# peteroh23/ModulationDetectionCNN

Measured on AMD Instinct MI355X. Metric: I/Q frames/sec (2x128, VT-CNN2, batch=2^20), higher is better.
Workload: dtype bf16; 1 GPU; vtcnn2-c11-bf16-n2^20; topology=vtcnn2, classes=11, frames_per_gpu=1048576, global_batch=1048576, parallelism=batch-shard x1 (no collective), outputs=softmax probabilities f32 + argmax int32, frames_per_forward_call=1048576, full=False

## Files before the change

### modulationdetectioncnn_amd/csrc/mdc_api.hip

```cpp
#include "mdc_internal.h"

#include <cstdlib>
#include <cstring>
#include <exception>
#include <mutex>
#include <new>

namespace mdc {

static thread_local char g_err[512] = "";

void set_error(const char* fmt, ...) {
    va_list ap;
    va_start(ap, fmt);
    vsnprintf(g_err, sizeof(g_err), fmt, ap);
    va_end(ap);
}

int upload(mdc_model* m, int idx, const void* host, size_t bytes) {
    if (m->d_pack[idx]) {
        (void)hipFree(m->d_pack[idx]);
        m->d_pack[idx] = nullptr;
    }
    MDC_HIP(hipMalloc(&m->d_pack[idx], bytes));
    MDC_HIP(hipMemcpy(m->d_pack[idx], host, bytes, hipMemcpyHostToDevice));
    m->pack_bytes[idx] = bytes;
    return MDC_OK;
}

ProfScope::ProfScope(const mdc_model* mm, int slot_, hipStream_t s_) : m(const_cast<mdc_model*>(mm)), slot(slot_), s(s_) {
    if (!m->profiling) return;
    if (hipEventCreate(&start) != hipSuccess) { start = nullptr; return; }
    (void)hipEventRecord(start, s);
}
ProfScope::~ProfScope() {
    if (!start) return;
    hipEvent_t stop = nullptr;
    if (hipEventCreate(&stop) != hipSuccess) { (void)hipEventDestroy(start); return; }
    (void)hipEventRecord(stop, s);
    try {
        std::lock_guard<std::mutex> g(m->prof_mu);
        std::vector<hipEvent_t>& ev = m->slots[slot].ev;
        ev.reserve(ev.size() + 2);
        ev.push_back(start);
        ev.push_back(stop);
    } catch (...) {
        (void)hipEventDestroy(start);
        (void)hipEventDestroy(stop);
    }
}

int iq_norm_check(const char* who, int64_t hop, float level, int flags) {
    if (hop < 1 || hop > (int64_t)1 << 24) { set_error("%s: hop must be in 1..2^24 sample pairs (got %lld)", who, (long long)hop); return MDC_EINVAL; }
    if (!(level > 0.f) || !(level <= 3.402823466e38f)) { set_error("%s: level must be finite and > 0", who); return MDC_EINVAL; }
    if ((flags & ~MDC_IQ_REMOVE_DC) != 0) { set_error("%s: unknown flag bits 0x%x", who, flags & ~MDC_IQ_REMOVE_DC); return MDC_EINVAL; }
    return MDC_OK;
}

}

using namespace mdc;

static int layer_layout(mdc_model* m) {
    const mdc_topology& t = m->topo;
    switch (t.kind) {
        case MDC_KIND_DEPLOYED:
            if (t.filters != 3 && t.filters != 10) { set_error("deployed: filters must be 3 or 10 (got %d)", t.filters); return MDC_ENOTSUP; }
            if (t.classes != 3) { set_error("deployed: classes must be 3 (got %d)", t.classes); return MDC_ENOTSUP; }
            m->nlayers = 2;
            m->nk[0] = 2 * (size_t)t.filters;            m->nb[0] = t.filters;
            m->nk[1] = 258 * (size_t)t.filters * t.classes; m->nb[1] = t.classes;
            m->slots = {{"mdc_deployed_fwd"}};
            return MDC_OK;
        case MDC_KIND_VTCNN2:
            if (t.classes < 2 || t.classes > 16) { set_error("vtcnn2: classes must be in 2..16 (got %d)", t.classes); return MDC_ENOTSUP; }
            m->nlayers = 4;
            m->nk[0] = (size_t)kC1 * 3;               m->nb[0] = kC1;
            m->nk[1] = (size_t)kC2 * kC1 * 2 * 3;     m->nb[1] = kC2;
            m->nk[2] = (size_t)kFeat * kHid;          m->nb[2] = kHid;
            m->nk[3] = (size_t)kHid * t.classes;      m->nb[3] = t.classes;
            m->slots = {{"mdc_vt_conv"}, {"mdc_vt_dense1"}, {"mdc_vt_head"}};
            return MDC_OK;
        case MDC_KIND_CNNPY:
            if (t.filters < 1 || t.filters > 10 || t.hidden < 1 || t.hidden > 16 || t.classes < 1 || t.classes > 16) {
                set_error("cnnpy: need filters 1..10, hidden 1..16, classes 1..16 (got %d,%d,%d)", t.filters, t.hidden, t.classes);
                return MDC_ENOTSUP;
            }
            m->nlayers = 3;
            m->nk[0] = 2 * 128 * (size_t)t.filters;        m->nb[0] = t.filters;
            m->nk[1] = 3 * (size_t)t.filters * t.hidden;    m->nb[1] = t.hidden;
            m->nk[2] = (size_t)t.hidden * t.classes;        m->nb[2] = t.classes;
            m->slots = {{"mdc_dense_chain"}};
            return MDC_OK;
        default:
            set_error("unknown topology kind %d", t.kind);
            return MDC_EINVAL;
    }
}

extern "C" {

int mdc_abi_version(void) { return MDC_ABI_VERSION; }

const char* mdc_last_error(void) { return g_err; }

int mdc_create(const mdc_topology* topo, int device, mdc_model** out) {
    return guarded("mdc_create", [&]() -> int {
        if (!topo || !out) { set_error("mdc_create: null argument"); return MDC_EINVAL; }
        *out = nullptr;
        if ((topo->reserved[0] & ~MDC_OPT_ALL) != 0) { set_error("mdc_create: unknown option bits 0x%x in reserved[0]", topo->reserved[0]); return MDC_EINVAL; }
        for (int i = 1; i < 4; ++i) if (topo->reserved[i] != 0) { set_error("mdc_create: reserved[1..3] must be 0"); return MDC_EINVAL; }
        if ((topo->reserved[0] & MDC_OPT_FP8_BF16_FEATURES) && topo->kind != MDC_KIND_VTCNN2) {
            set_error("mdc_create: MDC_OPT_FP8_BF16_FEATURES applies to MDC_KIND_VTCNN2 only");
            return MDC_EINVAL;
        }
        int ndev = 0;
        if (hipGetDeviceCount(&ndev) != hipSuccess || ndev == 0) { set_error("no HIP device available"); return MDC_ENODEV; }
        if (device < 0 || device >= ndev) { set_error("device %d out of range (have %d)", device, ndev); return MDC_ENODEV; }
        hipDeviceProp_t prop;
        MDC_HIP(hipGetDeviceProperties(&prop, device));
        if (std::strncmp(prop.gcnArchName, "gfx950", 6) != 0) {
            set_error("device %d is %s; libmdc.so carries gfx950 (MI355X) code only", device, prop.gcnArchName);
            return MDC_ENODEV;
        }
        mdc_model* m = new (std::nothrow) mdc_model();
        if (!m) { set_error("out of host memory"); return MDC_ENOMEM; }
        m->topo = *topo;
        m->device = device;
#ifdef MDC_ALTERNATES
        {
            auto flag = [](const char* name, int when) { const char* e = getenv(name); return e && atoi(e) == when; };
            if (flag("MDC_CONV_SCHED", 0)) m->alt |= kAltConvHipcc;
            if (flag("MDC_DENSE1_PHASED", 0)) m->alt |= kAltDense1Simple;
            if (flag("MDC_DEP_F32_MFMA", 1)) m->alt |= kAltDepF32Mfma;
            if (flag("MDC_D1_FUSED_HEAD", 0)) m->alt |= kAltSeparateHead;
            if (const char* e = getenv("MDC_DEP_RING")) m->alt_ring = atoi(e);
        }
#endif
        int rc = MDC_ENOMEM;
        try { rc = layer_layout(m); } catch (...) { delete m; throw; }
        if (rc != MDC_OK) { delete m; return rc; }
        *out = m;
        return MDC_OK;
    });
}

int mdc_num_layers(const mdc_model* m) {
    if (!m) { set_error("null model"); return MDC_EINVAL; }
    return m->nlayers;
}

int mdc_layer_sizes(const mdc_model* m, int layer, size_t* kernel_elems, size_t* bias_elems) {
    if (!m || layer < 0 || layer >= m->nlayers) { set_error("mdc_layer_sizes: bad layer %d", layer); return MDC_EINVAL; }
    if (kernel_elems) *kernel_elems = m->nk[layer];
    if (bias_elems) *bias_elems = m->nb[layer];
    return MDC_OK;
}

int mdc_set_weights(mdc_model* m, int layer, const float* kernel_host, size_t kernel_elems,
                    const float* bias_host, size_t bias_elems) {
    return guarded("mdc_set_weights", [&]() -> int {
        if (!m || !kernel_host || !bias_host) { set_error("mdc_set_weights: null argument"); return MDC_EINVAL; }
        if (m->finalized) { set_error("mdc_set_weights: model is finalized (immutable)"); return MDC_ESTATE; }
        if (layer < 0 || layer >= m->nlayers) { set_error("mdc_set_weights: layer %d out of range 0..%d", layer, m->nlayers - 1); return MDC_EINVAL; }
        if (kernel_elems != m->nk[layer] || bias_elems != m->nb[layer]) {
            set_error("mdc_set_weights: layer %d expects kernel %zu / bias %zu elements, got %zu / %zu",
                      layer, m->nk[layer], m->nb[layer], kernel_elems, bias_elems);
            return MDC_EINVAL;
        }
        m->have[layer] = false;
        m->hk[layer].assign(kernel_host, kernel_host + kernel_elems);
        m->hb[layer].assign(bias_host, bias_host + bias_elems);
        m->have[layer] = true;
        return MDC_OK;
    });
}

int mdc_finalize(mdc_model* m, int dtype) {
    return guarded("mdc_finalize", [&]() -> int {
        if (!m) { set_error("null model"); return MDC_EINVAL; }
        if (m->finalized) { set_error("mdc_finalize: already finalized"); return MDC_ESTATE; }
        for (int l = 0; l < m->nlayers; ++l)
            if (!m->have[l]) { set_error("mdc_finalize: layer %d has no weights", l); return MDC_ESTATE; }
        if (dtype != MDC_F32 && dtype != MDC_BF16 && dtype != MDC_FP8 && dtype != MDC_F16) { set_error("unknown dtype %d", dtype); return MDC_EINVAL; }
        if (dtype == MDC_F16 && m->topo.kind != MDC_KIND_DEPLOYED) { set_error("f16 is implemented for the deployed nets only"); return MDC_ENOTSUP; }
        if (dtype == MDC_FP8 && m->topo.kind == MDC_KIND_CNNPY) { set_error("fp8 is implemented for the vtcnn2 and deployed families only"); return MDC_ENOTSUP; }
        if ((m->topo.reserved[0] & MDC_OPT_FP8_BF16_FEATURES) && dtype != MDC_FP8) { set_error("mdc_finalize: MDC_OPT_FP8_BF16_FEATURES is an option of the MDC_FP8 mode"); return MDC_EINVAL; }
        if (dtype == MDC_BF16 && m->topo.kind == MDC_KIND_CNNPY) { set_error("bf16 is implemented for the vtcnn2 and deployed families only"); return MDC_ENOTSUP; }
        m->dtype = dtype;
        DeviceScope dev(m->device);
        if (!dev.ok) { set_error("mdc_finalize: cannot select device %d", m->device); return MDC_EIO; }
        int rc;
        switch (m->topo.kind) {
            case MDC_KIND_DEPLOYED:
                rc = deployed_pack(m);
                if (rc == MDC_OK) rc = deployed_q612_pack(m);
                if (rc == MDC_OK && dtype != MDC_F32) rc = deployed_bf16_pack(m);
                break;
            case MDC_KIND_VTCNN2:   rc = vtcnn2_pack(m); break;
            case MDC_KIND_CNNPY:    rc = cnnpy_pack(m); break;
            default: rc = MDC_EINVAL;
        }
        if (rc != MDC_OK) return rc;
        for (int l = 0; l < m->nlayers; ++l) {
            std::vector<float>().swap(m->hk[l]);
            std::vector<float>().swap(m->hb[l]);
        }
        m->finalized = true;
        return MDC_OK;
    });
}

size_t mdc_workspace_bytes(const mdc_model* m, int64_t n) {
    if (!m || n <= 0) return 0;
    if (m->topo.kind == MDC_KIND_VTCNN2) return vtcnn2_workspace_bytes(m, n);
    return 0;
}

int mdc_forward(const mdc_model* m, const void* x_dev, int64_t n, float* probs_dev, int32_t* labels_dev,
                float* tap_dev, int tap, void* workspace_dev, size_t workspace_bytes, void* hip_stream) {
    return guarded("mdc_forward", [&]() -> int {
        if (!m) { set_error("null model"); return MDC_EINVAL; }
        if (!m->finalized) { set_error("mdc_forward: model not finalized"); return MDC_ESTATE; }
        if (n < 0) { set_error("mdc_forward: negative frame count"); return MDC_EINVAL; }
        if (n == 0) return MDC_OK;
        if (!x_dev) { set_error("mdc_forward: null input"); return MDC_EINVAL; }
        if ((reinterpret_cast<uintptr_t>(x_dev) & 15) != 0) { set_error("mdc_forward: input must be 16-byte aligned"); return MDC_EINVAL; }
        if (tap < MDC_TAP_NONE || tap > MDC_TAP_HIDDEN) { set_error("mdc_forward: bad tap %d", tap); return MDC_EINVAL; }
        if ((tap != MDC_TAP_NONE) != (tap_dev != nullptr)) { set_error("mdc_forward: tap and tap_dev must be given together"); return MDC_EINVAL; }
        DeviceScope dev(m->device);
        if (!dev.ok) { set_error("mdc_forward: cannot select device %d", m->device); return MDC_EIO; }
        hipStream_t s = static_cast<hipStream_t>(hip_stream);
        const float* x = static_cast<const float*>(x_dev);
        switch (m->topo.kind) {
            case MDC_KIND_DEPLOYED: return deployed_forward(m, x, n, probs_dev, labels_dev, tap_dev, tap, s);
            case MDC_KIND_VTCNN2:   return vtcnn2_forward(m, x, n, probs_dev, labels_dev, tap_dev, tap, workspace_dev, workspace_bytes, s);
            case MDC_KIND_CNNPY:    return cnnpy_forward(m, x, n, probs_dev, labels_dev, tap_dev, tap, s);
            default: return MDC_EINVAL;
        }
    });
}

int mdc_forward_checked(const mdc_model* m, const void* x_dev, int64_t n, float* probs_dev, int32_t* labels_dev, void* workspace_dev,
                        size_t workspace_bytes, uint8_t* nonfinite_dev, int64_t* nonfinite_count_dev, int policy, void* hip_stream) {
    return guarded("mdc_forward_checked", [&]() -> int {
        if (policy != MDC_NONFINITE_REPORT && policy != MDC_NONFINITE_PROPAGATE) { set_error("mdc_forward_checked: unknown policy %d", policy); return MDC_EINVAL; }
        if (n < 0) { set_error("mdc_forward_checked: negative frame count"); return MDC_EINVAL; }
        if (n > 0 && !nonfinite_dev) { set_error("mdc_forward_checked: null nonfinite_dev (the per-frame flags are required)"); return MDC_EINVAL; }
        if (n > 0 && !x_dev) { set_error("mdc_forward_checked: null input"); return MDC_EINVAL; }
        if ((reinterpret_cast<uintptr_t>(x_dev) & 15) != 0) { set_error("mdc_forward_checked: input must be 16-byte aligned"); return MDC_EINVAL; }
        if (!m) { set_error("mdc_forward_checked: null model"); return MDC_EINVAL; }
        if (!m->finalized) { set_error("mdc_forward_checked: model not finalized"); return MDC_ESTATE; }
        if (n == 0) return MDC_OK;
        const bool poison = policy == MDC_NONFINITE_PROPAGATE;
        if (m->topo.kind == MDC_KIND_DEPLOYED) {
            DeviceScope dev(m->device);
            if (!dev.ok) { set_error("mdc_forward_checked: cannot select device %d", m->device); return MDC_EIO; }
            return deployed_forward_checked(m, static_cast<const float*>(x_dev), n, probs_dev, labels_dev, nonfinite_dev, nonfinite_count_dev,
                                            poison, static_cast<hipStream_t>(hip_stream));
        }
        int rc = mdc_forward(m, x_dev, n, probs_dev, labels_dev, nullptr, MDC_TAP_NONE, workspace_dev, workspace_bytes, hip_stream);
        if (rc != MDC_OK) return rc;
        DeviceScope dev(m->device);
        if (!dev.ok) { set_error("mdc_forward_checked: cannot select device %d", m->device); return MDC_EIO; }
        return nonfinite_launch(static_cast<const float*>(x_dev), n, nonfinite_dev, nonfinite_count_dev, probs_dev, labels_dev, m->topo.classes,
                                poison, static_cast<hipStream_t>(hip_stream));
    });
}

int mdc_forward_iq_u8(const mdc_model* m, const uint8_t* iq_dev, int64_t n, int64_t hop, float scale,
                      float* probs_dev, int32_t* labels_dev, void* workspace_dev, size_t workspace_bytes, void* hip_stream) {
    return guarded("mdc_forward_iq_u8", [&]() -> int {
        if (!m) { set_error("null model"); return MDC_EINVAL; }
        if (!m->finalized) { set_error("mdc_forward_iq_u8: model not finalized"); return MDC_ESTATE; }
        if (m->topo.kind == MDC_KIND_CNNPY) {
            set_error("mdc_forward_iq_u8: raw-IQ input exists for the deployed and vtcnn2 families; use mdc_iq_u8_to_frames + mdc_forward");
            return MDC_ENOTSUP;
        }
        if (n < 0) { set_error("mdc_forward_iq_u8: negative window count"); return MDC_EINVAL; }
        if (hop < 1 || hop > (int64_t)1 << 24) { set_error("mdc_forward_iq_u8: hop must be in 1..2^24 sample pairs (got %lld)", (long long)hop); return MDC_EINVAL; }
        if (n == 0) return MDC_OK;
        if (!iq_dev) { set_error("mdc_forward_iq_u8: null input"); return MDC_EINVAL; }
        if ((reinterpret_cast<uintptr_t>(iq_dev) & 1) != 0) { set_error("mdc_forward_iq_u8: input must start on a whole (I,Q) pair (2-byte aligned)"); return MDC_EINVAL; }
        DeviceScope dev(m->device);
        if (!dev.ok) { set_error("mdc_forward_iq_u8: cannot select device %d", m->device); return MDC_EIO; }
        hipStream_t s = static_cast<hipStream_t>(hip_stream);
        if (m->topo.kind == MDC_KIND_VTCNN2)
            return vtcnn2_forward_iq_u8(m, iq_dev, n, hop, scale, probs_dev, labels_dev, workspace_dev, workspace_bytes, s);
        return (m->dtype == MDC_F32) ? deployed_forward_iq_u8(m, iq_dev, n, hop, scale, probs_dev, labels_dev, s)
                                     : deployed_bf16_forward_iq_u8(m, iq_dev, n, hop, scale, probs_dev, labels_dev, s);
    });
}

int mdc_set_fp8_input_absmax(mdc_model* m, float absmax) {
    if (!m) { set_error("null model"); return MDC_EINVAL; }
    if (m->finalized) { set_error("mdc_set_fp8_input_absmax: call it before mdc_finalize"); return MDC_ESTATE; }
    if (!(absmax > 0.f) || !(absmax < 1e30f)) { set_error("mdc_set_fp8_input_absmax: need a positive finite value"); return MDC_EINVAL; }
    m->fp8_input_absmax = absmax;
    return MDC_OK;
}

int mdc_set_fp8_feature_absmax(mdc_model* m, float absmax) {
    if (!m) { set_error("null model"); return MDC_EINVAL; }
    if (m->finalized) { set_error("mdc_set_fp8_feature_absmax: call it before mdc_finalize"); return MDC_ESTATE; }
    if (m->topo.kind != MDC_KIND_VTCNN2) { set_error("mdc_set_fp8_feature_absmax: the E4M3 features exist for MDC_KIND_VTCNN2 only"); return MDC_EINVAL; }
    if (!(absmax > 0.f) || !(absmax < 1e30f)) { set_error("mdc_set_fp8_feature_absmax: need a positive finite value"); return MDC_EINVAL; }
    m->fp8_feature_absmax = absmax;
    return MDC_OK;
}

int mdc_forward_q612(const mdc_model* m, const void* x_dev, int x_is_q612, int64_t n, int32_t* dense_dev, int32_t* labels_dev,
                     void* hip_stream) {
    return guarded("mdc_forward_q612", [&]() -> int {
        if (!m) { set_error("null model"); return MDC_EINVAL; }
        if (!m->finalized) { set_error("mdc_forward_q612: model not finalized"); return MDC_ESTATE; }
        if (m->topo.kind != MDC_KIND_DEPLOYED) { set_error("mdc_forward_q612: the FPGA datapath exists for the deployed nets only"); return MDC_ENOTSUP; }
        if (n < 0) { set_error("mdc_forward_q612: negative frame count"); return MDC_EINVAL; }
        if (n == 0) return MDC_OK;
        if (!x_dev) { set_error("mdc_forward_q612: null input"); return MDC_EINVAL; }
        if ((reinterpret_cast<uintptr_t>(x_dev) & 15) != 0) { set_error("mdc_forward_q612: input must be 16-byte aligned"); return MDC_EINVAL; }
        DeviceScope dev(m->device);
        if (!dev.ok) { set_error("mdc_forward_q612: cannot select device %d", m->device); return MDC_EIO; }
        return deployed_q612_forward(m, x_dev, x_is_q612 != 0, n, dense_dev, labels_dev, static_cast<hipStream_t>(hip_stream));
    });
}

int mdc_confusion(const int32_t* truth_dev, const int32_t* pred_dev, int64_t n, int classes, int64_t* counts_dev, int64_t* bad_dev,
                  void* hip_stream) {
    if (n < 0) { set_error("mdc_confusion: negative count"); return MDC_EINVAL; }
    if (n > 0 && (!truth_dev || !pred_dev)) { set_error("mdc_confusion: null labels"); return MDC_EINVAL; }
    if (!counts_dev) { set_error("mdc_confusion: null counts"); return MDC_EINVAL; }
    return guarded("mdc_confusion", [&]() -> int {
        return confusion_launch(truth_dev, pred_dev, nullptr, n, classes, 1, counts_dev, bad_dev, static_cast<hipStream_t>(hip_stream)); });
}

int mdc_confusion_binned(const int32_t* truth_dev, const int32_t* pred_dev, const int32_t* bin_dev, int64_t n, int classes, int bins,
                         int64_t* counts_dev, int64_t* bad_dev, void* hip_stream) {
    if (n < 0) { set_error("mdc_confusion_binned: negative count"); return MDC_EINVAL; }
    if (n > 0 && (!truth_dev || !pred_dev || !bin_dev)) { set_error("mdc_confusion_binned: null labels"); return MDC_EINVAL; }
    if (!counts_dev) { set_error("mdc_confusion_binned: null counts"); return MDC_EINVAL; }
    if (bins < 1) { set_error("mdc_confusion_binned: bins must be >= 1 (got %d)", bins); return MDC_EINVAL; }
    return guarded("mdc_confusion_binned", [&]() -> int {
        return confusion_launch(truth_dev, pred_dev, bin_dev, n, classes, bins, counts_dev, bad_dev, static_cast<hipStream_t>(hip_stream)); });
}

int mdc_crossentropy(const float* probs_dev, const int32_t* truth_dev, int64_t n, int classes, double* loss_sum_dev, int64_t* bad_dev,
                     void* hip_stream) {
    if (n < 0) { set_error("mdc_crossentropy: negative count"); return MDC_EINVAL; }
    if (n > 0 && (!probs_dev || !truth_dev)) { set_error("mdc_crossentropy: null probabilities or labels"); return MDC_EINVAL; }
    if (!loss_sum_dev) { set_error("mdc_crossentropy: null loss accumulator"); return MDC_EINVAL; }
    return guarded("mdc_crossentropy", [&]() -> int {
        return crossentropy_launch(probs_dev, truth_dev, n, classes, loss_sum_dev, bad_dev, static_cast<hipStream_t>(hip_stream)); });
}

int mdc_iq_u8_to_frames(const uint8_t* iq_dev, int64_t n, float scale, float* x_dev, void* hip_stream) {
    if (n < 0) { set_error("mdc_iq_u8_to_frames: negative frame count"); return MDC_EINVAL; }
    if (n == 0) return MDC_OK;
    if (!iq_dev || !x_dev) { set_error("mdc_iq_u8_to_frames: null buffer"); return MDC_EINVAL; }
    if ((reinterpret_cast<uintptr_t>(iq_dev) & 3) != 0 || (reinterpret_cast<uintptr_t>(x_dev) & 7) != 0) {
        set_error("mdc_iq_u8_to_frames: iq must be 4-byte and frames 8-byte aligned");
        return MDC_EINVAL;
    }
    return guarded("mdc_iq_u8_to_frames", [&]() -> int { return iq_u8_launch(iq_dev, n, 128, scale, x_dev, static_cast<hipStream_t>(hip_stream)); });
}

int mdc_iq_u8_windows(const uint8_t* iq_dev, int64_t n, int64_t hop, float scale, float* x_dev, void* hip_stream) {
    if (n < 0) { set_error("mdc_iq_u8_windows: negative window count"); return MDC_EINVAL; }
    if (hop < 1 || hop > (int64_t)1 << 24) { set_error("mdc_iq_u8_windows: hop must be in 1..2^24 sample pairs (got %lld)", (long long)hop); return MDC_EINVAL; }
    if (n == 0) return MDC_OK;
    if (!iq_dev || !x_dev) { set_error("mdc_iq_u8_windows: null buffer"); return MDC_EINVAL; }
    if ((reinterpret_cast<uintptr_t>(x_dev) & 7) != 0) { set_error("mdc_iq_u8_windows: frames must be 8-byte aligned"); return MDC_EINVAL; }
    if ((reinterpret_cast<uintptr_t>(iq_dev) & 1) != 0) { set_error("mdc_iq_u8_windows: input must start on a whole (I,Q) pair (2-byte aligned)"); return MDC_EINVAL; }
    return guarded("mdc_iq_u8_windows", [&]() -> int { return iq_u8_launch(iq_dev, n, hop, scale, x_dev, static_cast<hipStream_t>(hip_stream)); });
}

int mdc_iq_u8_windows_norm(const uint8_t* iq_dev, int64_t n, int64_t hop, float level, int flags, float* x_dev,
                           mdc_iq_window_stats* stats_dev, void* hip_stream) {
    if (n < 0) { set_error("mdc_iq_u8_windows_norm: negative window count"); return MDC_EINVAL; }
    int rc = iq_norm_check("mdc_iq_u8_windows_norm", hop, level, flags);
    if (rc != MDC_OK) return rc;
    if (!x_dev && !stats_dev) { set_error("mdc_iq_u8_windows_norm: x_dev and stats_dev are both null (nothing to compute)"); return MDC_EINVAL; }
    if ((reinterpret_cast<uintptr_t>(x_dev) & 7) != 0) { set_error("mdc_iq_u8_windows_norm: frames must be 8-byte aligned"); return MDC_EINVAL; }
    if ((reinterpret_cast<uintptr_t>(stats_dev) & 15) != 0) { set_error("mdc_iq_u8_windows_norm: statistics must be 16-byte aligned"); return MDC_EINVAL; }
    if (n > 0 && !iq_dev) { set_error("mdc_iq_u8_windows_norm: null input"); return MDC_EINVAL; }
    if ((reinterpret_cast<uintptr_t>(iq_dev) & 1) != 0) { set_error("mdc_iq_u8_windows_norm: input must start on a whole (I,Q) pair (2-byte aligned)"); return MDC_EINVAL; }
    return guarded("mdc_iq_u8_windows_norm", [&]() -> int {
        return iq_norm_launch(iq_dev, n, hop, level, flags, x_dev, stats_dev, static_cast<hipStream_t>(hip_stream)); });
}

int mdc_set_profiling(mdc_model* m, int on) {
    if (!m) { set_error("null model"); return MDC_EINVAL; }
    m->profiling = on != 0;
    return MDC_OK;
}

int mdc_profile_slots(const mdc_model* m) { return m ? (int)m->slots.size() : MDC_EINVAL; }

const char* mdc_profile_name(const mdc_model* m, int slot) {
    if (!m || slot < 0 || slot >= (int)m->slots.size()) return "";
    return m->slots[slot].name;
}

int mdc_profile_read(mdc_model* m, int slot, double* total_ms, int64_t* launches) {
    return guarded("mdc_profile_read", [&]() -> int {
        if (!m || slot < 0 || slot >= (int)m->slots.size()) { set_error("mdc_profile_read: bad slot"); return MDC_EINVAL; }
        ProfSlot& ps = m->slots[slot];
        std::vector<hipEvent_t> ev;
        {
            std::lock_guard<std::mutex> g(m->prof_mu);
            ev.swap(ps.ev);
        }
        double add_ms = 0;
        int64_t add_n = 0;
        int rc = MDC_OK;
        for (size_t i = 0; i + 1 < ev.size(); i += 2) {
            float ms = 0.f;
            if (hipEventSynchronize(ev[i + 1]) != hipSuccess || hipEventElapsedTime(&ms, ev[i], ev[i + 1]) != hipSuccess) {
                set_error("mdc_profile_read: event query failed");
                rc = MDC_EIO;
                break;
            }
            add_ms += ms;
            add_n += 1;
        }
        for (hipEvent_t e : ev) (void)hipEventDestroy(e);
        std::lock_guard<std::mutex> g(m->prof_mu);
        ps.total_ms += add_ms;
        ps.launches += add_n;
        if (total_ms) *total_ms = ps.total_ms;
        if (launches) *launches = ps.launches;
        return rc;
    });
}

int mdc_profile_reset(mdc_model* m) {
    if (!m) { set_error("null model"); return MDC_EINVAL; }
    std::lock_guard<std::mutex> g(m->prof_mu);
    for (ProfSlot& ps : m->slots) {
        for (hipEvent_t e : ps.ev) (void)hipEventDestroy(e);
        ps.ev.clear();
        ps.total_ms = 0;
        ps.launches = 0;
    }
    return MDC_OK;
}

int mdc_predict_host(mdc_model* m, const float* x_host, int64_t n, float* probs_host, int32_t* labels_host, int64_t chunk_frames) {
    return guarded("mdc_predict_host", [&]() -> int { return predict_host(m, x_host, n, probs_host, labels_host, chunk_frames); });
}

int mdc_predict_host_checked(mdc_model* m, const float* x_host, int64_t n, float* probs_host, int32_t* labels_host, uint8_t* nonfinite_host,
                             int64_t* nonfinite_count, int policy, int64_t chunk_frames) {
    return guarded("mdc_predict_host_checked", [&]() -> int {
        return predict_host_checked(m, x_host, n, probs_host, labels_host, nonfinite_host, nonfinite_count, policy, chunk_frames); });
}

int mdc_predict_host_iq_u8(mdc_model* m, const uint8_t* iq_host, int64_t n, int64_t hop, float scale, float* probs_host,
                           int32_t* labels_host, int64_t chunk_frames) {
    return guarded("mdc_predict_host_iq_u8", [&]() -> int { return predict_host_iq_u8(m, iq_host, n, hop, scale, probs_host, labels_host, chunk_frames); });
}

int mdc_predict_host_iq(mdc_model* m, const void* iq_host, int format, int64_t n, int64_t hop, float scale, float* probs_host,
                        int32_t* labels_host, int64_t chunk_frames) {
    return guarded("mdc_predict_host_iq", [&]() -> int { return predict_host_iq(m, iq_host, format, n, hop, scale, probs_host, labels_host, chunk_frames); });
}

int mdc_predict_host_iq_norm(mdc_model* m, const void* iq_host, int format, int64_t n, int64_t hop, float level, int flags, float* probs_host,
                             int32_t* labels_host, mdc_iq_window_stats64* stats64_host, int64_t chunk_frames) {
    return guarded("mdc_predict_host_iq_norm", [&]() -> int {
        return predict_host_iq_norm(m, iq_host, format, n, hop, level, flags, probs_host, labels_host, stats64_host, chunk_frames); });
}

int mdc_predict_host_iq_u8_norm(mdc_model* m, const uint8_t* iq_host, int64_t n, int64_t hop, float level, int flags, float* probs_host,
                                int32_t* labels_host, mdc_iq_window_stats* stats_host, int64_t chunk_frames) {
    return guarded("mdc_predict_host_iq_u8_norm", [&]() -> int {
        return predict_host_iq_u8_norm(m, iq_host, n, hop, level, flags, probs_host, labels_host, stats_host, chunk_frames); });
}

void mdc_destroy(mdc_model* m) {
    if (!m) return;
    {
        DeviceScope dev(m->device);
        host_ctx_free(m);
    }
    for (void*& p : m->d_pack) if (p) { (void)hipFree(p); p = nullptr; }
    for (ProfSlot& ps : m->slots) for (hipEvent_t e : ps.ev) (void)hipEventDestroy(e);
    delete m;
}

}
```

### modulationdetectioncnn_amd/csrc/mdc_internal.h

```cpp
#pragma once
#include <hip/hip_runtime.h>
#include <cstdarg>
#include <cstdint>
#include <cstdio>
#include <exception>
#include <mutex>
#include <new>
#include <string>
#include <type_traits>
#include <vector>

#include "mdc.h"

namespace mdc {

void set_error(const char* fmt, ...);

template <class Fn>
inline int guarded(const char* what, Fn&& fn) noexcept {
    try {
        return fn();
    } catch (const std::bad_alloc&) {
        set_error("%s: out of host memory", what);
        return MDC_ENOMEM;
    } catch (const std::exception& e) {
        set_error("%s: %s", what, e.what());
        return MDC_EIO;
    } catch (...) {
        set_error("%s: unexpected exception", what);
        return MDC_EIO;
    }
}

#define MDC_HIP(call)                                                                      \
    do {                                                                                   \
        hipError_t e_ = (call);                                                            \
        if (e_ != hipSuccess) {                                                            \
            mdc::set_error("%s failed: %s (%s:%d)", #call, hipGetErrorString(e_), __FILE__, __LINE__); \
            return MDC_EIO;                                                                \
        }                                                                                  \
    } while (0)

constexpr int kRows = 2;
constexpr int kSamples = 128;
constexpr int kFrameFloats = kRows * kSamples;

constexpr int kC1 = 256;
constexpr int kW1 = 130;
constexpr int kC2 = 80;
constexpr int kW2 = 132;
constexpr int kFeat = kC2 * kW2;
constexpr int kHid = 256;

__host__ __device__ constexpr int feat16_index(int w, int o) {
    return (w >> 1) * (2 * kC2) + (o < 64 ? (w & 1) * 64 + o : 128 + 2 * (o - 64) + (w & 1));
}

__host__ __device__ constexpr int feat8_index(int w, int o) {
    return (w >> 2) * (4 * kC2) + (o < 64 ? ((w >> 1) & 1) * 128 + 8 * (o >> 2) + 4 * (w & 1) + (o & 3) : 256 + 4 * (o - 64) + (w & 3));
}

__device__ __forceinline__ uint2 load8_unaligned(const unsigned char* p) {
    uint2 r;
    __builtin_memcpy(&r, p, 8);
    return r;
}

struct NfArgs {
    unsigned char* flags;
    unsigned long long* count;
    int poison;
};
template <bool CHECK> using HopOrNf = typename std::conditional<CHECK, NfArgs, long>::type;
__device__ __forceinline__ long hop_of(long h) { return h; }
__device__ __forceinline__ long hop_of(const NfArgs&) { return 256; }
__device__ __forceinline__ NfArgs nf_of(long) { return NfArgs{nullptr, nullptr, 0}; }
__device__ __forceinline__ NfArgs nf_of(const NfArgs& a) { return a; }
constexpr unsigned kNfInfBits = 0x7F800000u;
__device__ __forceinline__ unsigned nf_absbits_max4(const float4 v) {
    return max(max(__float_as_uint(v.x) & 0x7FFFFFFFu, __float_as_uint(v.y) & 0x7FFFFFFFu),
               max(__float_as_uint(v.z) & 0x7FFFFFFFu, __float_as_uint(v.w) & 0x7FFFFFFFu));
}

enum { kAltConvHipcc = 1,
       kAltDense1Simple = 2,
       kAltDepF32Mfma = 4,
       kAltSeparateHead = 8 };

struct ProfSlot {
    const char* name;
    std::vector<hipEvent_t> ev;
    double total_ms = 0;
    int64_t launches = 0;
};

}

struct mdc_model {
    mdc_topology topo{};
    int device = 0;
    int dtype = MDC_F32;
    bool finalized = false;
    int nlayers = 0;
    size_t nk[4]{}, nb[4]{};
    std::vector<float> hk[4], hb[4];
    bool have[4]{};

    void* d_pack[8]{};
    size_t pack_bytes[8]{};

    int alt = 0;
    int alt_ring = -1;
    float fp8_input_absmax = 0.02f;
    float fp8_feature_absmax = 0.f;
    int fp8_feat_scale_log2 = 0;
    bool fp8_e4m3_features = false;
    float fp8_feat_divisor = 1.f;
    int feat_scale_log2 = 0;

    bool profiling = false;
    std::vector<mdc::ProfSlot> slots;
    std::mutex prof_mu;

    void* host_ctx = nullptr;
    std::mutex host_mu;
};

namespace mdc {

struct ProfScope {
    mdc_model* m;
    int slot;
    hipStream_t s;
    hipEvent_t start = nullptr;
    ProfScope(const mdc_model* mm, int slot_, hipStream_t s_);
    ~ProfScope();
    ProfScope(const ProfScope&) = delete;
    ProfScope& operator=(const ProfScope&) = delete;
};

int upload(mdc_model* m, int idx, const void* host, size_t bytes);

struct DeviceScope {
    int prev = -1, want;
    bool ok = true;
    explicit DeviceScope(int device) : want(device) {
        if (hipGetDevice(&prev) != hipSuccess) prev = -1;
        if (prev != want && hipSetDevice(want) != hipSuccess) ok = false;
    }
    ~DeviceScope() { if (prev >= 0 && prev != want) (void)hipSetDevice(prev); }
    DeviceScope(const DeviceScope&) = delete;
    DeviceScope& operator=(const DeviceScope&) = delete;
};

int predict_host(mdc_model* m, const float* x_host, int64_t n, float* probs_host, int32_t* labels_host, int64_t chunk_frames);
int predict_host_checked(mdc_model* m, const float* x_host, int64_t n, float* probs_host, int32_t* labels_host, uint8_t* nonfinite_host,
                         int64_t* nonfinite_count, int policy, int64_t chunk_frames);
int predict_host_iq_u8(mdc_model* m, const uint8_t* iq_host, int64_t n, int64_t hop, float scale, float* probs_host, int32_t* labels_host,
                       int64_t chunk_frames);
int predict_host_iq_u8_norm(mdc_model* m, const uint8_t* iq_host, int64_t n, int64_t hop, float level, int flags, float* probs_host,
                            int32_t* labels_host, mdc_iq_window_stats* stats_host, int64_t chunk_frames);
int predict_host_iq(mdc_model* m, const void* iq_host, int format, int64_t n, int64_t hop, float scale, float* probs_host, int32_t* labels_host,
                    int64_t chunk_frames);
int predict_host_iq_norm(mdc_model* m, const void* iq_host, int format, int64_t n, int64_t hop, float level, int flags, float* probs_host,
                         int32_t* labels_host, mdc_iq_window_stats64* stats_host, int64_t chunk_frames);
void host_ctx_free(mdc_model* m);

int deployed_pack(mdc_model* m);
int deployed_f32m_pack(mdc_model* m);
int deployed_f32m_forward(const mdc_model* m, const float* x, int64_t n, float* probs, int32_t* labels, float* tap_dense, hipStream_t s);
int deployed_f32m_forward_iq_u8(const mdc_model* m, const uint8_t* iq, int64_t n, long hop2, float scale, float* probs, int32_t* labels, hipStream_t s);
int deployed_bf16_pack(mdc_model* m);
int deployed_bf16_forward(const mdc_model* m, const float* x, int64_t n, float* probs, int32_t* labels, hipStream_t s);
int deployed_bf16_forward_iq_u8(const mdc_model* m, const uint8_t* iq, int64_t n, int64_t hop, float scale, float* probs, int32_t* labels, hipStream_t s);
int deployed_q612_pack(mdc_model* m);
int deployed_q612_forward(const mdc_model* m, const void* x, int x_is_q, int64_t n, int32_t* dense, int32_t* labels, hipStream_t s);
int vtcnn2_fp8_pack(mdc_model* m);
int vtcnn2_fp8_conv(const mdc_model* m, const float* x, int64_t n, void* feat, hipStream_t s, long hop2 = 0, float scale = 0.f);
int confusion_launch(const int32_t* truth, const int32_t* pred, const int32_t* bin, int64_t n, int classes, int bins, int64_t* counts,
                     int64_t* bad, hipStream_t s);
int crossentropy_launch(const float* probs, const int32_t* truth, int64_t n, int classes, double* loss_sum, int64_t* bad, hipStream_t s);
int iq_u8_launch(const uint8_t* iq, int64_t n, int64_t hop, float scale, float* x, hipStream_t s);
int iq_norm_check(const char* who, int64_t hop, float level, int flags);
int iq_norm_launch(const uint8_t* iq, int64_t n, int64_t hop, float level, int flags, float* x, mdc_iq_window_stats* stats, hipStream_t s);
constexpr long kIqGridCap = 16384;
int iq_pair_bytes(int format);
constexpr int64_t iq_span_count(int64_t pairs, int64_t span, int64_t step) { return pairs >= span ? (pairs - span) / step + 1 : 0; }
int iq_format_known(const char* who, int format);
int iq_pair_aligned(const char* who, const char* what, int format, const void* p);
int iq_aligned(const char* who, const char* what, const void* p, int bytes);
int iq_format_check(const char* who, int format, int64_t hop);
int iq_norm_wave_launch(const uint8_t* iq, int64_t n, int64_t hop, float level, int flags, float* x, mdc_iq_window_stats* stats, hipStream_t s);
int iq_spec_shape_check(const char* who, int64_t pairs, int nfft, int64_t hop, int avg);
int64_t iq_spec_rows(int64_t pairs, int nfft, int64_t hop, int avg);
int iq_spec_jobs_launch(const void* iq, int format, int order, int nfft, int64_t hop, int avg, const int16_t* window, float gain, float* power, int64_t rows,
                        const mdc_iq_line_job* jobs_dev, int64_t njobs, hipStream_t s);
template <class Fn>
inline int with_format(int format, Fn&& fn) {
    if (format == MDC_IQ_CU8) return fn(std::integral_constant<int, MDC_IQ_CU8>{});
    if (format == MDC_IQ_CI8) return fn(std::integral_constant<int, MDC_IQ_CI8>{});
    return fn(std::integral_constant<int, MDC_IQ_CI16>{});
}
inline int pow2_log2(int value, int lo, int hi) {
    for (int l = lo; l <= hi; ++l)
        if (value == 1 << l) return l;
    return -1;
}
template <int LO, int HI, class Fn>
inline int with_log2(int log2, Fn&& fn) {
    if constexpr (LO < HI) {
        if (log2 == LO) return fn(std::integral_constant<int, LO>{});
        return with_log2<LO + 1, HI>(log2, fn);
    } else {
        return fn(std::integral_constant<int, HI>{});
    }
}
int nonfinite_launch(const float* x, int64_t n, uint8_t* flags, int64_t* count, float* probs, int32_t* labels, int classes, bool poison,
                     hipStream_t s);
int deployed_forward(const mdc_model* m, const float* x, int64_t n, float* probs, int32_t* labels,
                     float* tap, int tap_kind, hipStream_t s);
int deployed_forward_iq_u8(const mdc_model* m, const uint8_t* iq, int64_t n, int64_t hop, float scale, float* probs, int32_t* labels, hipStream_t s);
int deployed_forward_checked(const mdc_model* m, const float* x, int64_t n, float* probs, int32_t* labels, uint8_t* flags, int64_t* count,
                             bool poison, hipStream_t s);
int deployed_bf16_forward_checked(const mdc_model* m, const float* x, int64_t n, float* probs, int32_t* labels, uint8_t* flags, int64_t* count,
                                  bool poison, hipStream_t s);

int cnnpy_pack(mdc_model* m);
int cnnpy_forward(const mdc_model* m, const float* x, int64_t n, float* probs, int32_t* labels,
                  float* tap, int tap_kind, hipStream_t s);

int vtcnn2_pack(mdc_model* m);
size_t vtcnn2_workspace_bytes(const mdc_model* m, int64_t n);
int vtcnn2_forward(const mdc_model* m, const float* x, int64_t n, float* probs, int32_t* labels,
                   float* tap, int tap_kind, void* ws, size_t ws_bytes, hipStream_t s);
int vtcnn2_forward_iq_u8(const mdc_model* m, const uint8_t* iq, int64_t n, int64_t hop, float scale, float* probs, int32_t* labels,
                         void* ws, size_t ws_bytes, hipStream_t s);

}
```

### modulationdetectioncnn_amd/csrc/vtcnn2.hip

```cpp
#include "dense_chain_common.h"

#include <algorithm>
#include <cmath>

namespace mdc {

namespace {

__device__ __forceinline__ void glds16(const void* g, void* lds_wave_base) {
    const unsigned l = (unsigned)(size_t)(__attribute__((address_space(3))) unsigned char*)lds_wave_base;
    asm volatile("global_load_lds_dwordx4 %0, off" ::"v"(g), "{m0}"(l) : "memory");
}
__device__ __forceinline__ void glds_drain_and_barrier() {
    asm volatile("s_waitcnt vmcnt(0)" ::: "memory");
    __syncthreads();
}

constexpr int kChunk = 16;
constexpr int kNChunk = kC1 / kChunk;
constexpr int kWChunkFloats = 2 * 3 * 5 * 4 * 64;
constexpr int kXld = 133;
constexpr int kXinFloats = 4 * 2 * 16 * kXld;
constexpr size_t kConvF32Lds = (2 * kWChunkFloats + kXinFloats) * sizeof(float);

template <bool U8, int KP, bool YSPLIT>
__global__ __launch_bounds__(256, 1) void vt_conv_f32_kernel(const float* __restrict__ x, long n,
                                                             const float* __restrict__ wpack,
                                                             const float* __restrict__ a1pack,
                                                             const float* __restrict__ b2,
                                                             float* __restrict__ feat,
                                                             long hop2, float scale) {
    extern __shared__ __attribute__((aligned(16))) float smem[];
    float* wbuf = smem;
    float* xin = smem + 2 * kWChunkFloats;
    const int tid = threadIdx.x, lane = tid & 63, q = tid >> 6;
    const int nl = lane & 15, g = lane >> 4;
    const long frame0 = (long)blockIdx.x * 64 + q * 16;

    float* xw = xin + q * (2 * 16 * kXld);
    {
        const int h = lane >> 5, s = (lane & 31) * 4;
#pragma unroll 4
        for (int i = 0; i < 16; ++i) {
            const long f = frame0 + i;
            float4 v = make_float4(0.f, 0.f, 0.f, 0.f);
            if constexpr (U8) {
                if (f < n) {
                    const uint2 r = load8_unaligned(reinterpret_cast<const unsigned char*>(x) + f * hop2 + (lane & 31) * 8);
                    const unsigned a = r.x >> (8 * h), b = r.y >> (8 * h);
                    v = make_float4(((float)(a & 0xFFu) - 127.5f) * scale, ((float)((a >> 16) & 0xFFu) - 127.5f) * scale,
                                    ((float)(b & 0xFFu) - 127.5f) * scale, ((float)((b >> 16) & 0xFFu) - 127.5f) * scale);
                }
            } else {
                if (f < n) v = reinterpret_cast<const float4*>(x + f * kFrameFloats)[lane];
            }
            float* d = xw + (h * 16 + i) * kXld + 2 + s;
            d[0] = v.x; d[1] = v.y; d[2] = v.z; d[3] = v.w;
        }
        for (int r = lane; r < 32 * 5; r += 64) {
            const int row = r / 5, k = r % 5;
            xw[row * kXld + (k < 2 ? k : 128 + k)] = 0.f;
        }
    }
    for (int p = q; p < kWChunkFloats / 256; p += 4) glds16(wpack + p * 256 + lane * 4, wbuf + p * 256);
    glds_drain_and_barrier();

    const float* xrow0 = xw + (0 * 16 + nl) * kXld + g;
    const float* xrow1 = xw + (1 * 16 + nl) * kXld + g;

    int it = 0;
    float a1n = a1pack[lane];
    constexpr int kNPB = kW2 / KP;
    static_assert(kNPB * KP == kW2, "KP must divide 132");
    for (int pb = YSPLIT ? (int)blockIdx.y : 0; pb < (YSPLIT ? (int)blockIdx.y + 1 : kNPB); ++pb) {
        const int w0 = pb * KP;
        f32x4 acc[KP][5];
#pragma unroll
        for (int a = 0; a < KP; ++a)
#pragma unroll
            for (int b = 0; b < 5; ++b) acc[a][b] = f32x4{0.f, 0.f, 0.f, 0.f};

        for (int cc = 0; cc < kNChunk; ++cc, ++it) {
            const float* wb = wbuf + (it & 1) * kWChunkFloats + lane;
            {
                const int nc = (cc + 1) & (kNChunk - 1);
                const float* src = wpack + (size_t)nc * kWChunkFloats;
                float* dst = wbuf + ((it + 1) & 1) * kWChunkFloats;
                for (int p = q; p < kWChunkFloats / 256; p += 4) glds16(src + p * 256 + lane * 4, dst + p * 256);
            }
            const float a1 = a1n;
            a1n = a1pack[((cc + 1) & (kNChunk - 1)) * 64 + lane];
#pragma unroll
            for (int u = 0; u < KP + 2; ++u) {
                const int wp = w0 + u;
                if (wp < 2 || wp > 131) continue;
                const int v = wp - 2;
#pragma unroll
                for (int h = 0; h < 2; ++h) {
                    const float xv = (h == 0 ? xrow0 : xrow1)[v];
                    const float b1f = (g == 3) ? 1.0f : xv;
                    f32x4 X = __builtin_amdgcn_mfma_f32_16x16x4f32(a1, b1f, f32x4{0.f, 0.f, 0.f, 0.f}, 0, 0, 0);
#pragma unroll
                    for (int r = 0; r < 4; ++r) X[r] = fmaxf(X[r], 0.f);
#pragma unroll
                    for (int j = 0; j < 3; ++j) {
                        const int wo = u - j;
                        if (wo < 0 || wo >= KP) continue;
#pragma unroll
                        for (int r = 0; r < 4; ++r)
#pragma unroll
                            for (int ot = 0; ot < 5; ++ot) {
                                const float a = wb[(((h * 3 + j) * 5 + ot) * 4 + r) * 64];
                                acc[wo][ot] = __builtin_amdgcn_mfma_f32_16x16x4f32(a, X[r], acc[wo][ot], 0, 0, 0);
                            }
                    }
                }
            }
            glds_drain_and_barrier();
        }
        const long f = frame0 + nl;
        if (f < n) {
#pragma unroll
            for (int a = 0; a < KP; ++a)
#pragma unroll
                for (int ot = 0; ot < 5; ++ot) {
                    const int o = ot * 16 + g * 4;
                    const float4 bb = *reinterpret_cast<const float4*>(b2 + o);
                    float4 r;
                    r.x = fmaxf(acc[a][ot][0] + bb.x, 0.f);
                    r.y = fmaxf(acc[a][ot][1] + bb.y, 0.f);
                    r.z = fmaxf(acc[a][ot][2] + bb.z, 0.f);
                    r.w = fmaxf(acc[a][ot][3] + bb.w, 0.f);
                    *reinterpret_cast<float4*>(feat + (f * kW2 + (w0 + a)) * kC2 + o) = r;
                }
        }
    }
}

constexpr int kDM = 128, kDK = 32;
constexpr int kDAld = 34, kDBld = 272;
constexpr int kDBBuf = kDK * kDBld;
template <int ROWS> constexpr size_t dense1_f32_lds() {
    const size_t img = (size_t)ROWS * kChainXld * sizeof(float), stg = 2 * ((size_t)ROWS * kDAld + kDBBuf) * sizeof(float);
    return img > stg ? img : stg;
}
constexpr size_t kDense1F32Lds = dense1_f32_lds<128>();

template <bool HEAD, int ROWS>
__global__ __launch_bounds__(512) void vt_dense1_f32_kernel(const float* __restrict__ feat, long n,
                                                            const float* __restrict__ w1p,
                                                            const float* __restrict__ c1,
                                                            float* __restrict__ hid,
                                                            const float* __restrict__ w2pack, int n_out,
                                                            float* __restrict__ probs, int* __restrict__ labels) {
    extern __shared__ __attribute__((aligned(16))) float dsm[];
    constexpr int kDABuf = ROWS * kDAld, RI = ROWS / 32;
    float* As = dsm;
    float* Bs = dsm + 2 * kDABuf;
    const int tid = threadIdx.x, lane = tid & 63, wv = tid >> 6;
    const int wr = wv >> 2, wc = wv & 3;
    const int fr = lane & 15, fq = lane >> 4;
    const long row0 = (long)blockIdx.x * ROWS;
    f32x4 acc[RI][4];
#pragma unroll
    for (int i = 0; i < RI; ++i)
#pragma unroll
        for (int j = 0; j < 4; ++j) acc[i][j] = f32x4{0.f, 0.f, 0.f, 0.f};

    constexpr bool kTwoA = ROWS == 128;
    const int ar0 = tid >> 3, ak4 = (tid & 7) * 4;
    const int bk0 = tid >> 6, bc4 = (tid & 63) * 4;
    const bool aok0 = row0 + ar0 < n, aok1 = kTwoA && row0 + ar0 + 64 < n;
    const float* ap0 = feat + (aok0 ? row0 + ar0 : 0) * (long)kFeat + ak4;
    const float* ap1 = feat + (aok1 ? row0 + ar0 + 64 : 0) * (long)kFeat + ak4;
    float4 ga0, ga1, gb0, gb1, gb2, gb3;
    const float* bp = w1p + (size_t)bk0 * kHid + bc4;
    auto fetch = [&](int k0) {
        ga0 = *reinterpret_cast<const float4*>(ap0 + k0);
        if (kTwoA) ga1 = *reinterpret_cast<const float4*>(ap1 + k0);
        const float* b = bp + (size_t)k0 * kHid;
        gb0 = *reinterpret_cast<const float4*>(b);
        gb1 = *reinterpret_cast<const float4*>(b + 8 * kHid);
        gb2 = *reinterpret_cast<const float4*>(b + 16 * kHid);
        gb3 = *reinterpret_cast<const float4*>(b + 24 * kHid);
    };
    auto stash = [&](int b) {
        float* a = As + b * kDABuf + ar0 * kDAld + ak4;
        const float4 v0 = aok0 ? ga0 : make_float4(0.f, 0.f, 0.f, 0.f), v1 = aok1 ? ga1 : make_float4(0.f, 0.f, 0.f, 0.f);
        *reinterpret_cast<float2*>(a) = make_float2(v0.x, v0.y);
        *reinterpret_cast<float2*>(a + 2) = make_float2(v0.z, v0.w);
        if (kTwoA) {
            *reinterpret_cast<float2*>(a + 64 * kDAld) = make_float2(v1.x, v1.y);
            *reinterpret_cast<float2*>(a + 64 * kDAld + 2) = make_float2(v1.z, v1.w);
        }
        float* d = Bs + b * kDBBuf + bk0 * kDBld + bc4;
        *reinterpret_cast<float4*>(d) = gb0;
        *reinterpret_cast<float4*>(d + 8 * kDBld) = gb1;
        *reinterpret_cast<float4*>(d + 16 * kDBld) = gb2;
        *reinterpret_cast<float4*>(d + 24 * kDBld) = gb3;
    };
    fetch(0);
    stash(0);
    __syncthreads();
    constexpr int kTiles = kFeat / kDK;
    for (int t = 0; t < kTiles; ++t) {
        const int b = t & 1;
        if (t + 1 < kTiles) fetch((t + 1) * kDK);
        __builtin_amdgcn_sched_barrier(0);
        const float* Ab = As + b * kDABuf + (wr * (ROWS / 2) + fr) * kDAld + fq;
        const float* Bb = Bs + b * kDBBuf + fq * kDBld + wc * 64 + fr;
#pragma unroll
        for (int kk = 0; kk < kDK; kk += 4) {
            float a[RI], bv[4];
#pragma unroll
            for (int i = 0; i < RI; ++i) a[i] = Ab[i * 16 * kDAld + kk];
#pragma unroll
            for (int j = 0; j < 4; ++j) bv[j] = Bb[kk * kDBld + j * 16];
#pragma unroll
            for (int i = 0; i < RI; ++i)
#pragma unroll
                for (int j = 0; j < 4; ++j)
                    acc[i][j] = __builtin_amdgcn_mfma_f32_16x16x4f32(a[i], bv[j], acc[i][j], 0, 0, 0);
        }
        __builtin_amdgcn_sched_barrier(0);
        if (t + 1 < kTiles) stash(b ^ 1);
        __syncthreads();
    }
    if constexpr (!HEAD) {
#pragma unroll
        for (int i = 0; i < RI; ++i)
#pragma unroll
            for (int j = 0; j < 4; ++j) {
                const int col = wc * 64 + j * 16 + fr;
                const float bias = c1[col];
#pragma unroll
                for (int r = 0; r < 4; ++r) {
                    const long row = row0 + wr * (ROWS / 2) + i * 16 + fq * 4 + r;
                    if (row < n) hid[row * kHid + col] = fmaxf(acc[i][j][r] + bias, 0.f);
                }
            }
    } else {
        float* xs = dsm;
#pragma unroll
        for (int j = 0; j < 4; ++j) {
            const int col = wc * 64 + j * 16 + fr;
            const float bias = c1[col];
#pragma unroll
            for (int i = 0; i < RI; ++i)
#pragma unroll
                for (int r = 0; r < 4; ++r) xs[(wr * (ROWS / 2) + i * 16 + fq * 4 + r) * kChainXld + col] = fmaxf(acc[i][j][r] + bias, 0.f);
        }
        float w2[64];
#pragma unroll
        for (int i = 0; i < 64; ++i) w2[i] = w2pack[i * 64 + lane];
        const float b2 = w2pack[64 * 64 + 16 * 64 + fr];
        __syncthreads();
        if (wv < ROWS / 16) {
            const f32x4 a2 = chain_k256(xs + (wv * 16 + fr) * kChainXld + fq, w2, f32x4{0.f, 0.f, 0.f, 0.f});
            f32x4 z;
#pragma unroll
            for (int r = 0; r < 4; ++r) z[r] = a2[r] + b2;
            chain_softmax_store(z, fr, fq, row0 + wv * 16, n, n_out, probs, labels, nullptr);
        }
    }
}

#ifdef MDC_ALTERNATES
constexpr int kDN = 128, kDld = 129;

__global__ __launch_bounds__(256) void vt_dense1_f32_tiles128_kernel(const float* __restrict__ feat, long n,
                                                                     const float* __restrict__ w1p,
                                                                     const float* __restrict__ c1,
                                                                     float* __restrict__ hid) {
    __shared__ float As[kDK][kDld];
    __shared__ float Bs[kDK][kDld + 3];
    const int tid = threadIdx.x, lane = tid & 63, wv = tid >> 6;
    const int wr = wv >> 1, wc = wv & 1;
    const int fr = lane & 15, fq = lane >> 4;
    const long row0 = (long)blockIdx.x * kDM;
    const int col0 = blockIdx.y * kDN;
    f32x4 acc[4][4];
#pragma unroll
    for (int i = 0; i < 4; ++i)
#pragma unroll
        for (int j = 0; j < 4; ++j) acc[i][j] = f32x4{0.f, 0.f, 0.f, 0.f};

    for (int k0 = 0; k0 < kFeat; k0 += kDK) {
#pragma unroll
        for (int i = 0; i < 4; ++i) {
            const int idx = tid + 256 * i;
            const int r = idx >> 3, k4 = (idx & 7) * 4;
            float4 v = make_float4(0.f, 0.f, 0.f, 0.f);
            if (row0 + r < n) v = *reinterpret_cast<const float4*>(feat + (row0 + r) * kFeat + k0 + k4);
            As[k4 + 0][r] = v.x; As[k4 + 1][r] = v.y; As[k4 + 2][r] = v.z; As[k4 + 3][r] = v.w;
        }
#pragma unroll
        for (int i = 0; i < 4; ++i) {
            const int idx = tid + 256 * i;
            const int k = idx >> 5, c4 = (idx & 31) * 4;
            const float4 v = *reinterpret_cast<const float4*>(w1p + (size_t)(k0 + k) * kHid + col0 + c4);
            *reinterpret_cast<float4*>(&Bs[k][c4]) = v;
        }
        __syncthreads();
#pragma unroll
        for (int kk = 0; kk < kDK; kk += 4) {
            float a[4], b[4];
#pragma unroll
            for (int i = 0; i < 4; ++i) a[i] = As[kk + fq][wr * 64 + i * 16 + fr];
#pragma unroll
            for (int j = 0; j < 4; ++j) b[j] = Bs[kk + fq][wc * 64 + j * 16 + fr];
#pragma unroll
            for (int i = 0; i < 4; ++i)
#pragma unroll
                for (int j = 0; j < 4; ++j)
                    acc[i][j] = __builtin_amdgcn_mfma_f32_16x16x4f32(a[i], b[j], acc[i][j], 0, 0, 0);
        }
        __syncthreads();
    }
#pragma unroll
    for (int i = 0; i < 4; ++i)
#pragma unroll
        for (int j = 0; j < 4; ++j) {
            const int col = col0 + wc * 64 + j * 16 + fr;
            const float bias = c1[col];
#pragma unroll
            for (int r = 0; r < 4; ++r) {
                const long row = row0 + wr * 64 + i * 16 + fq * 4 + r;
                if (row < n) hid[row * kHid + col] = fmaxf(acc[i][j][r] + bias, 0.f);
            }
        }
}
#endif

__global__ __launch_bounds__(64) void vt_dense1_f32_small_kernel(const float* __restrict__ feat, long n,
                                                                 const float* __restrict__ w1p,
                                                                 const float* __restrict__ c1, float* __restrict__ hid) {
    const int lane = threadIdx.x, fr = lane & 15, fq = lane >> 4;
    const long row0 = (long)blockIdx.x * 16;
    const int col0 = blockIdx.y * 16;
    long ar = row0 + fr;
    if (ar >= n) ar = n - 1;
    const float* ap = feat + ar * (long)kFeat + fq;
    const float* bp = w1p + (size_t)fq * kHid + col0 + fr;
    f32x4 acc = f32x4{0.f, 0.f, 0.f, 0.f};
    constexpr int kU = 24;
    constexpr int kBlocks = kFeat / (4 * kU);
    static_assert(kBlocks * 4 * kU == kFeat, "block size must divide K / 4");
    float a[2][kU], b[2][kU];
    auto fetch = [&](int blk, float (&aa)[kU], float (&bb)[kU]) {
        const int k0 = blk * 4 * kU;
#pragma unroll
        for (int u = 0; u < kU; ++u) {
            aa[u] = ap[k0 + 4 * u];
            bb[u] = bp[(size_t)(k0 + 4 * u) * kHid];
        }
    };
    fetch(0, a[0], b[0]);
    for (int blk = 0; blk < kBlocks; blk += 2) {
        if (blk + 1 < kBlocks) fetch(blk + 1, a[1], b[1]);
#pragma unroll
        for (int u = 0; u < kU; ++u) acc = __builtin_amdgcn_mfma_f32_16x16x4f32(a[0][u], b[0][u], acc, 0, 0, 0);
        if (blk + 1 < kBlocks) {
            if (blk + 2 < kBlocks) fetch(blk + 2, a[0], b[0]);
#pragma unroll
            for (int u = 0; u < kU; ++u) acc = __builtin_amdgcn_mfma_f32_16x16x4f32(a[1][u], b[1][u], acc, 0, 0, 0);
        }
    }
    const int col = col0 + fr;
    const float bias = c1[col];
#pragma unroll
    for (int r = 0; r < 4; ++r) {
        const long row = row0 + fq * 4 + r;
        if (row < n) hid[row * kHid + col] = fmaxf(acc[r] + bias, 0.f);
    }
}

template <typename T>
__global__ void vt_unpermute_kernel(const T* __restrict__ feat, long n, float* __restrict__ out, float unscale) {
    const long i = (long)blockIdx.x * blockDim.x + threadIdx.x;
    if (i >= n * kFeat) return;
    const long f = i / kFeat;
    const int r = (int)(i % kFeat);
    const int o = r / kW2, w = r % kW2;
    if constexpr (sizeof(T) == 2) {
        const T v = feat[f * kFeat + feat16_index(w, o)];
        out[i] = __uint_as_float(((unsigned)v) << 16) * unscale;
    } else {
        out[i] = feat[(f * kW2 + w) * kC2 + o];
    }
}

__global__ void vt_unpermute8_kernel(const unsigned char* __restrict__ feat, long n, float* __restrict__ out, float unscale) {
    const long i = (long)blockIdx.x * blockDim.x + threadIdx.x;
    if (i >= n * kFeat) return;
    const long f = i / kFeat;
    const int r = (int)(i % kFeat);
    const int o = r / kW2, w = r % kW2;
    const unsigned v = feat[f * kFeat + feat8_index(w, o)];
    const int e = (int)((v >> 3) & 15u), mant = (int)(v & 7u);
    float mag = e == 0 ? ldexpf((float)mant, -9) : ldexpf(1.f + (float)mant * 0.125f, e - 7);
    if ((v & 0x7Fu) == 0x7Fu) mag = __uint_as_float(0x7FC00000u);
    out[i] = ((v & 0x80u) ? -mag : mag) * unscale;
}

}

void chain_pack_layer(std::vector<float>& dst, const float* w, int k_in, int n_out, int ksteps, int tiles);
int chain_launch(int t1, int nl, const float* x, long n, const float* wpack, int n_out, int relu1, int relu2,
                 float* probs, int* labels, float* tap_logits, float* tap_h1, float* tap_h2, int n1, int n2, hipStream_t s);

int vtcnn2_bf16_pack(mdc_model* m);
int vtcnn2_bf16_conv(const mdc_model* m, const float* x, int64_t n, void* feat, hipStream_t s, long hop2 = 0, float scale = 0.f);
int vtcnn2_bf16_dense1(const mdc_model* m, const void* feat, int64_t n, float* hid, hipStream_t s,
                       bool fuse_head, float* probs, int32_t* labels, bool* fused);

int vtcnn2_pack(mdc_model* m) {
    const float* k1 = m->hk[0].data();
    const float* b1 = m->hb[0].data();
    const float* k2 = m->hk[1].data();
    int rc;
    if ((rc = upload(m, 2, m->hb[1].data(), kC2 * sizeof(float)))) return rc;
    if ((rc = upload(m, 4, m->hb[2].data(), kHid * sizeof(float)))) return rc;
    {
        const int C = m->topo.classes;
        if (C > 16) { set_error("vtcnn2: the HIP head covers up to 16 classes (got %d)", C); return MDC_ENOTSUP; }
        std::vector<float> pk;
        chain_pack_layer(pk, m->hk[3].data(), kHid, C, 64, 1);
        pk.resize(pk.size() + 16 * 64, 0.f);
        std::vector<float> bias(96, 0.f);
        for (int c = 0; c < C; ++c) bias[c] = m->hb[3][c];
        pk.insert(pk.end(), bias.begin(), bias.end());
        if ((rc = upload(m, 5, pk.data(), pk.size() * sizeof(float)))) return rc;
    }
    if (m->dtype == MDC_BF16) return vtcnn2_bf16_pack(m);
    if (m->dtype == MDC_FP8) return vtcnn2_fp8_pack(m);

    std::vector<float> wp((size_t)kNChunk * kWChunkFloats);
    for (int cc = 0; cc < kNChunk; ++cc)
        for (int h = 0; h < 2; ++h)
            for (int j = 0; j < 3; ++j)
                for (int ot = 0; ot < 5; ++ot)
                    for (int r = 0; r < 4; ++r)
                        for (int lane = 0; lane < 64; ++lane) {
                            const int o = 16 * ot + (lane & 15), c = 16 * cc + 4 * (lane >> 4) + r;
                            wp[(size_t)cc * kWChunkFloats + ((((h * 3 + j) * 5 + ot) * 4 + r) * 64) + lane] =
                                k2[(((size_t)o * kC1 + c) * 2 + h) * 3 + j];
                        }
    if ((rc = upload(m, 0, wp.data(), wp.size() * sizeof(float)))) return rc;
    std::vector<float> a1((size_t)kNChunk * 64);
    for (int cc = 0; cc < kNChunk; ++cc)
        for (int lane = 0; lane < 64; ++lane) {
            const int c = 16 * cc + (lane & 15), g = lane >> 4;
            a1[cc * 64 + lane] = (g < 3) ? k1[c * 3 + g] : b1[c];
        }
    if ((rc = upload(m, 1, a1.data(), a1.size() * sizeof(float)))) return rc;
    const float* w1 = m->hk[2].data();
    std::vector<float> w1p((size_t)kFeat * kHid);
    for (int w = 0; w < kW2; ++w)
        for (int o = 0; o < kC2; ++o)
            std::copy(w1 + (size_t)(o * kW2 + w) * kHid, w1 + (size_t)(o * kW2 + w + 1) * kHid,
                      w1p.begin() + (size_t)(w * kC2 + o) * kHid);
    return upload(m, 3, w1p.data(), w1p.size() * sizeof(float));
}

static size_t feat_elem(const mdc_model* m) { return m->dtype == MDC_F32 ? 4 : (m->dtype == MDC_FP8 && m->fp8_e4m3_features) ? 1 : 2; }

size_t vtcnn2_workspace_bytes(const mdc_model* m, int64_t n) {
    const size_t np = ((size_t)n + 255) & ~(size_t)255;
    return np * kFeat * feat_elem(m) + np * kHid * sizeof(float);
}

static int vtcnn2_run(const mdc_model* m, const float* x, long hop2, float scale, int64_t n, float* probs, int32_t* labels,
                      float* tap, int tap_kind, void* ws, size_t ws_bytes, hipStream_t s) {
    const size_t need = vtcnn2_workspace_bytes(m, n);
    if (!ws || ws_bytes < need) { set_error("vtcnn2 forward of %lld frames needs %zu workspace bytes (got %zu)", (long long)n, need, ws_bytes); return MDC_EINVAL; }
    if ((reinterpret_cast<uintptr_t>(ws) & 255) != 0) { set_error("workspace must be 256-byte aligned"); return MDC_EINVAL; }
    const size_t fbytes = (((size_t)n + 255) & ~(size_t)255) * kFeat * feat_elem(m);
    void* feat = ws;
    float* hid = reinterpret_cast<float*>(static_cast<char*>(ws) + fbytes);
    const int C = m->topo.classes;
    int rc;
    bool head_done = false;
    if (m->dtype == MDC_BF16 || m->dtype == MDC_FP8) {
        { ProfScope ps(m, 0, s); if ((rc = m->dtype == MDC_FP8 ? vtcnn2_fp8_conv(m, x, n, feat, s, hop2, scale) : vtcnn2_bf16_conv(m, x, n, feat, s, hop2, scale))) return rc; }
        const bool fuse = tap_kind != MDC_TAP_DENSE && tap_kind != MDC_TAP_HIDDEN;
        { ProfScope ps(m, 1, s); if ((rc = vtcnn2_bf16_dense1(m, feat, n, hid, s, fuse, probs, labels, &head_done))) return rc; }
    } else {
        {
            ProfScope ps(m, 0, s);
            const unsigned groups = (unsigned)((n + 63) / 64);
            constexpr long t1 = 128, t3 = 2048, t11 = 8192;
#define MDC_LAUNCH_CONV_F32(U, KP, YS) do { \
                MDC_HIP(hipFuncSetAttribute(reinterpret_cast<const void*>(vt_conv_f32_kernel<U, KP, YS>), hipFuncAttributeMaxDynamicSharedMemorySize, (int)kConvF32Lds)); \
                hipLaunchKernelGGL((vt_conv_f32_kernel<U, KP, YS>), dim3(groups, YS ? kW2 / KP : 1), dim3(256), kConvF32Lds, s, x, (long)n, \
                                   static_cast<const float*>(m->d_pack[0]), static_cast<const float*>(m->d_pack[1]), \
                                   static_cast<const float*>(m->d_pack[2]), static_cast<float*>(feat), hop2 > 0 ? hop2 : 256L, scale); } while (0)
            if (hop2 > 0) {
                if (n <= t1) MDC_LAUNCH_CONV_F32(true, 1, true);
                else if (n <= t3) MDC_LAUNCH_CONV_F32(true, 3, true);
                else if (n <= t11) MDC_LAUNCH_CONV_F32(true, 11, true);
                else MDC_LAUNCH_CONV_F32(true, 11, false);
            } else {
                if (n <= t1) MDC_LAUNCH_CONV_F32(false, 1, true);
                else if (n <= t3) MDC_LAUNCH_CONV_F32(false, 3, true);
                else if (n <= t11) MDC_LAUNCH_CONV_F32(false, 11, true);
                else MDC_LAUNCH_CONV_F32(false, 11, false);
            }
#undef MDC_LAUNCH_CONV_F32
            MDC_HIP(hipGetLastError());
        }
        {
            ProfScope ps(m, 1, s);
            const float* featf = static_cast<const float*>(feat);
            const float* w1p = static_cast<const float*>(m->d_pack[3]);
            const float* c1 = static_cast<const float*>(m->d_pack[4]);
            const float* w2pack = static_cast<const float*>(m->d_pack[5]);
            bool done = false;
#ifdef MDC_ALTERNATES
            if (n > 2048 && (m->alt & kAltDense1Simple)) {
                hipLaunchKernelGGL(vt_dense1_f32_tiles128_kernel, dim3((unsigned)((n + kDM - 1) / kDM), kHid / kDN), dim3(256), 0, s, featf, (long)n, w1p, c1, hid);
                done = true;
            }
#endif
            if (done) {
            } else if (n <= 2048) {
                hipLaunchKernelGGL(vt_dense1_f32_small_kernel, dim3((unsigned)((n + 15) / 16), kHid / 16), dim3(64), 0, s, featf, (long)n, w1p, c1, hid);
            } else {
                bool fuse = tap_kind != MDC_TAP_DENSE && tap_kind != MDC_TAP_HIDDEN;
#ifdef MDC_ALTERNATES
                if (m->alt & kAltSeparateHead) fuse = false;
#endif
#define MDC_LAUNCH_D1F32(H, R) do { \
                    MDC_HIP(hipFuncSetAttribute(reinterpret_cast<const void*>(vt_dense1_f32_kernel<H, R>), hipFuncAttributeMaxDynamicSharedMemorySize, (int)dense1_f32_lds<R>())); \
                    hipLaunchKernelGGL((vt_dense1_f32_kernel<H, R>), dim3((unsigned)((n + R - 1) / R)), dim3(512), dense1_f32_lds<R>(), s, featf, (long)n, w1p, c1, hid, \
                                       w2pack, C, probs, labels); } while (0)
                const bool half = n <= 16384;
                if (fuse) {
                    if (half) MDC_LAUNCH_D1F32(true, 64); else MDC_LAUNCH_D1F32(true, 128);
                    head_done = true;
                } else {
                    if (half) MDC_LAUNCH_D1F32(false, 64); else MDC_LAUNCH_D1F32(false, 128);
                }
#undef MDC_LAUNCH_D1F32
            }
            MDC_HIP(hipGetLastError());
        }
    }
    if (!head_done) {
        ProfScope ps(m, 2, s);
        if ((rc = chain_launch(1, 1, hid, (long)n, static_cast<const float*>(m->d_pack[5]), C, 0, 0, probs, labels,
                               tap_kind == MDC_TAP_DENSE ? tap : nullptr, nullptr, nullptr, 0, 0, s)))
            return rc;
    }
    if (tap_kind == MDC_TAP_CONV || tap_kind == MDC_TAP_FLAT) {
        const long total = (long)n * kFeat;
        const float unscale = std::ldexp(1.f, -m->feat_scale_log2);
        if (feat_elem(m) == 1)
            hipLaunchKernelGGL(vt_unpermute8_kernel, dim3((unsigned)((total + 255) / 256)), dim3(256), 0, s, static_cast<const unsigned char*>(feat), (long)n, tap, unscale);
        else if (m->dtype != MDC_F32)
            hipLaunchKernelGGL(vt_unpermute_kernel<unsigned short>, dim3((unsigned)((total + 255) / 256)), dim3(256), 0, s, static_cast<const unsigned short*>(feat), (long)n, tap, unscale);
        else
            hipLaunchKernelGGL(vt_unpermute_kernel<float>, dim3((unsigned)((total + 255) / 256)), dim3(256), 0, s, static_cast<const float*>(feat), (long)n, tap, unscale);
        MDC_HIP(hipGetLastError());
    } else if (tap_kind == MDC_TAP_HIDDEN) {
        MDC_HIP(hipMemcpyAsync(tap, hid, (size_t)n * kHid * sizeof(float), hipMemcpyDeviceToDevice, s));
    }
    return MDC_OK;
}

int vtcnn2_forward(const mdc_model* m, const float* x, int64_t n, float* probs, int32_t* labels,
                   float* tap, int tap_kind, void* ws, size_t ws_bytes, hipStream_t s) {
    return vtcnn2_run(m, x, 0, 0.f, n, probs, labels, tap, tap_kind, ws, ws_bytes, s);
}

int vtcnn2_forward_iq_u8(const mdc_model* m, const uint8_t* iq, int64_t n, int64_t hop, float scale, float* probs, int32_t* labels,
                         void* ws, size_t ws_bytes, hipStream_t s) {
    return vtcnn2_run(m, reinterpret_cast<const float*>(iq), 2 * (long)hop, scale, n, probs, labels, nullptr, MDC_TAP_NONE, ws, ws_bytes, s);
}

}
```

### modulationdetectioncnn_amd/csrc/vtcnn2_bf16.hip

```cpp
#include "vtcnn2_bf16_common.h"
#include "vtcnn2_sched_common.h"

#include <cmath>

#include <cstdlib>
#include <cstring>
#include <type_traits>

namespace mdc {

namespace {

#ifdef MDC_ALTERNATES
__global__ __launch_bounds__(256, 1) void vt_conv_bf16_kernel(const float* __restrict__ x, long n,
                                                              const u32x4* __restrict__ wq,
                                                              const u32x2* __restrict__ a1q,
                                                              const float* __restrict__ b2,
                                                              unsigned short* __restrict__ feat) {
    extern __shared__ __attribute__((aligned(16))) unsigned char smem[];
    unsigned* img = reinterpret_cast<unsigned*>(smem);
    float* part = reinterpret_cast<float*>(smem + (size_t)2 * kImgWords * 4);
    const int tid = threadIdx.x, lane = tid & 63;
    const int q = __builtin_amdgcn_readfirstlane(tid >> 6);
    const int nl = lane & 15, g = lane >> 4;

    bf16x8 W[2][3][2][5];
#pragma unroll
    for (int h = 0; h < 2; ++h)
#pragma unroll
        for (int j = 0; j < 3; ++j)
#pragma unroll
            for (int cp = 0; cp < 2; ++cp)
#pragma unroll
                for (int ot = 0; ot < 5; ++ot)
                    W[h][j][cp][ot] = __builtin_bit_cast(bf16x8, wq[(q * kWFrags + ((h * 3 + j) * 2 + cp) * 5 + ot) * 64 + lane]);
    s16x4 A1[4];
#pragma unroll
    for (int ct = 0; ct < 4; ++ct) A1[ct] = __builtin_bit_cast(s16x4, a1q[(q * 4 + ct) * 64 + lane]);
    float* bias_lds = part + 2 * kPartFloats;
    if (tid < kC2) bias_lds[tid] = b2[tid];
    const float* bq_lds = bias_lds + 16 * q + 4 * g;
    const float* b4_lds = bias_lds + 64 + 4 * g + q;

    for (int i = tid; i < 2 * kImgWords; i += 256) img[i] = ((i & 63) >= 48) ? 0x3F803F80u : 0u;
    __syncthreads();

    const long ngroups = (n + 15) >> 4;
    long grp = blockIdx.x;
    if (grp < ngroups)
        for (int k = 0; k < 4; ++k) stage_quarter(k, x, n, grp * 16, img, tid);
    __syncthreads();

    int buf = 0;
    for (; grp < ngroups; grp += gridDim.x, buf ^= 1) {
        const unsigned* im = img + buf * kImgWords + lane;
        const long frame0 = grp * 16;
        const long fme = frame0 + nl;
        unsigned short* fbase = feat + fme * (long)(kW2 * kC2) + 4 * g;
        const long gnext = grp + gridDim.x;

        f32x4 acc[3][5];
#pragma unroll
        for (int a = 0; a < 3; ++a)
#pragma unroll
            for (int b = 0; b < 5; ++b) acc[a][b] = f32x4{0.f, 0.f, 0.f, 0.f};
        bf16x8 Bf[2][2][2];
        f32x4 X[4][2];
        f32x4 rp[4];
        float rc[4];
        using I0 = std::integral_constant<int, 0>;
        using I1 = std::integral_constant<int, 1>;
        using I2 = std::integral_constant<int, 2>;

        unsigned bw[2][3];
        auto conv1_load = [&](int v, auto par_tag, auto h_tag) {
            constexpr int PAR = decltype(par_tag)::value, h = decltype(h_tag)::value;
            const unsigned* pi = im + (h * kPairs + (v >> 1)) * 64;
            bw[h][0] = pi[0];
            bw[h][1] = pi[64];
            if (PAR == 1) bw[h][2] = pi[128];
        };
        auto conv1 = [&](auto par_tag, auto h_tag) {
            constexpr int PAR = decltype(par_tag)::value, h = decltype(h_tag)::value;
            u32x2 b;
            if (PAR == 0) b = u32x2{bw[h][0], bw[h][1]};
            else b = u32x2{__builtin_amdgcn_alignbit(bw[h][1], bw[h][0], 16),
                           __builtin_amdgcn_alignbit(bw[h][2], bw[h][1], 16)};
#pragma unroll
            for (int ct = 0; ct < 4; ++ct) {
                f32x4& xd = X[ct][h];
                const s16x4& a1 = A1[ct];
                if (ct == 0) asm volatile("s_nop 1\n\tv_mfma_f32_16x16x16_bf16 %0, %1, %2, 0" : "=&v"(xd) : "v"(a1), "v"(b));
                else asm volatile("v_mfma_f32_16x16x16_bf16 %0, %1, %2, 0" : "=&v"(xd) : "v"(a1), "v"(b));
            }
        };
        auto x_fence = [&](auto h_tag) {
            constexpr int h = decltype(h_tag)::value;
            f32x4 &x0 = X[0][h], &x1 = X[1][h], &x2 = X[2][h], &x3 = X[3][h];
            asm volatile("s_nop 7\n\ts_nop 7" : "+v"(x0), "+v"(x1), "+v"(x2), "+v"(x3));
        };
        auto pack = [&](auto sp_tag, auto h_tag, auto cp_tag) {
            constexpr int sp = decltype(sp_tag)::value, h = decltype(h_tag)::value, cp = decltype(cp_tag)::value;
            const f32x4 t0 = X[2 * cp][h], t1 = X[2 * cp + 1][h];
            const u32x4 pk = u32x4{pack2relu(t0[0], t0[1]), pack2relu(t0[2], t0[3]), pack2relu(t1[0], t1[1]), pack2relu(t1[2], t1[3])};
            Bf[sp][h][cp] = __builtin_bit_cast(bf16x8, pk);
        };
        auto tap = [&](auto sp_tag, auto j_tag, auto h_tag, auto cp_tag, f32x4 (&a)[5], bool fresh) {
            constexpr int sp = decltype(sp_tag)::value, j = decltype(j_tag)::value, h = decltype(h_tag)::value, cp = decltype(cp_tag)::value;
#pragma unroll
            for (int ot = 0; ot < 5; ++ot) {
                const f32x4 c = fresh ? f32x4{0.f, 0.f, 0.f, 0.f} : a[ot];
                a[ot] = __builtin_amdgcn_mfma_f32_16x16x32_bf16(W[h][j][cp][ot], Bf[sp][h][cp], c, 0, 0, 0);
            }
        };
        auto part_write = [&](auto pb_tag, const f32x4 (&a)[5]) {
            constexpr int PB = decltype(pb_tag)::value;
            float* pw = part + PB * kPartFloats;
#pragma unroll
            for (int ot = 0; ot < 5; ++ot) *reinterpret_cast<f32x4*>(pw + ((q * 5 + ot) * 64 + lane) * 4) = a[ot];
        };
        auto red_load = [&](auto pb_tag) {
            constexpr int PB = decltype(pb_tag)::value;
            __syncthreads();
            const float* pw = part + PB * kPartFloats;
#pragma unroll
            for (int k = 0; k < 4; ++k) {
                rp[k] = *reinterpret_cast<const f32x4*>(pw + ((k * 5 + q) * 64 + lane) * 4);
                rc[k] = pw[((k * 5 + 4) * 64 + lane) * 4 + q];
            }
        };
        auto red_finish = [&](int w) {
            const f32x4 s = (rp[0] + rp[1]) + (rp[2] + rp[3]);
            u32x2 o;
            const f32x4 bq = *reinterpret_cast<const f32x4*>(bq_lds);
            o[0] = pack2relu(s[0] + bq[0], s[1] + bq[1]);
            o[1] = pack2relu(s[2] + bq[2], s[3] + bq[3]);
            const float t = ((rc[0] + rc[1]) + (rc[2] + rc[3])) + *b4_lds;
            const unsigned short t16 = (unsigned short)pack2relu(t, 0.f);
            unsigned short* frow = fbase - 4 * g;
            *reinterpret_cast<u32x2*>(frow + feat16_index(w, 16 * q + 4 * g)) = o;
            frow[feat16_index(w, 64 + 4 * g + q)] = t16;
        };
#define MDC_SB() __builtin_amdgcn_sched_barrier(0)
        auto step = [&](int v, auto par_next, auto first_tag, auto last_tag, f32x4 (&a0)[5], f32x4 (&a1)[5], f32x4 (&a2)[5]) {
            constexpr bool FIRST = decltype(first_tag)::value != 0, LAST = decltype(last_tag)::value != 0;
            using PB = std::integral_constant<int, 1 - decltype(par_next)::value>;
            if (!FIRST) { x_fence(I1{}); pack(PB{}, I1{}, I0{}); pack(PB{}, I1{}, I1{}); }
            if (!LAST) conv1_load(v + 1, par_next, I0{});
            tap(PB{}, I2{}, I0{}, I0{}, a2, false); tap(PB{}, I2{}, I0{}, I1{}, a2, false);
            tap(PB{}, I2{}, I1{}, I0{}, a2, false); tap(PB{}, I2{}, I1{}, I1{}, a2, false);
            part_write(PB{}, a2);
            if (!LAST) { conv1(par_next, I0{}); conv1_load(v + 1, par_next, I1{}); }
            tap(PB{}, I1{}, I0{}, I0{}, a1, false); tap(PB{}, I1{}, I0{}, I1{}, a1, false);
            tap(PB{}, I1{}, I1{}, I0{}, a1, false);
            if (!LAST) { x_fence(I0{}); pack(par_next, I0{}, I0{}); pack(par_next, I0{}, I1{}); }
            tap(PB{}, I1{}, I1{}, I1{}, a1, false);
            MDC_SB();
            if (!FIRST) red_finish(v - 1);
            red_load(PB{});
            asm volatile("" ::"a"(a2[0]), "a"(a2[1]), "a"(a2[2]), "a"(a2[3]), "a"(a2[4]));
            tap(PB{}, I0{}, I0{}, I0{}, a0, true);  tap(PB{}, I0{}, I0{}, I1{}, a0, false);
            tap(PB{}, I0{}, I1{}, I0{}, a0, false);
            if (!LAST) conv1(par_next, I1{});
            tap(PB{}, I0{}, I1{}, I1{}, a0, false);
            MDC_SB();
        };
        using P0 = std::integral_constant<int, 0>;
        using P1 = std::integral_constant<int, 1>;

        conv1_load(0, P0{}, I0{}); conv1_load(0, P0{}, I1{});
        conv1(P0{}, I0{}); conv1(P0{}, I1{});
        x_fence(I0{}); x_fence(I1{});
        pack(P0{}, I0{}, I0{}); pack(P0{}, I0{}, I1{}); pack(P0{}, I1{}, I0{}); pack(P0{}, I1{}, I1{});
        step(0, P1{}, I1{}, I0{}, acc[2], acc[1], acc[0]);
        int v = 1;
        for (int it = 0; it < 21; ++it, v += 6) {
            if (it >= 12 && it < 16 && gnext < ngroups)
                stage_quarter(it - 12, x, n, gnext * 16, img + (buf ^ 1) * kImgWords, tid);
            step(v + 0, P0{}, I0{}, I0{}, acc[0], acc[2], acc[1]);
            step(v + 1, P1{}, I0{}, I0{}, acc[1], acc[0], acc[2]);
            step(v + 2, P0{}, I0{}, I0{}, acc[2], acc[1], acc[0]);
            step(v + 3, P1{}, I0{}, I0{}, acc[0], acc[2], acc[1]);
            step(v + 4, P0{}, I0{}, I0{}, acc[1], acc[0], acc[2]);
            step(v + 5, P1{}, I0{}, I0{}, acc[2], acc[1], acc[0]);
        }
        step(127, P0{}, I0{}, I0{}, acc[0], acc[2], acc[1]);
        step(128, P1{}, I0{}, I0{}, acc[1], acc[0], acc[2]);
        step(129, P0{}, I0{}, I1{}, acc[2], acc[1], acc[0]);
        red_finish(129);
        part_write(I0{}, acc[1]); red_load(I0{});
        asm volatile("" ::"a"(acc[1][0]), "a"(acc[1][1]), "a"(acc[1][2]), "a"(acc[1][3]), "a"(acc[1][4]));
        red_finish(130);
        part_write(I1{}, acc[2]); red_load(I1{});
        asm volatile("" ::"a"(acc[2][0]), "a"(acc[2][1]), "a"(acc[2][2]), "a"(acc[2][3]), "a"(acc[2][4]));
        red_finish(131);
#undef MDC_SB
        __syncthreads();
    }
}


#endif

}

int vtcnn2_bf16_pack(mdc_model* m) {
    const float* k1 = m->hk[0].data();
    const float* b1 = m->hb[0].data();
    const float* k2 = m->hk[1].data();
    int rc;
#ifdef MDC_ALTERNATES
    std::vector<unsigned short> wq((size_t)4 * kWFrags * 64 * 8);
    for (int q = 0; q < 4; ++q)
        for (int h = 0; h < 2; ++h)
            for (int j = 0; j < 3; ++j)
                for (int cp = 0; cp < 2; ++cp)
                    for (int ot = 0; ot < 5; ++ot)
                        for (int lane = 0; lane < 64; ++lane)
                            for (int jj = 0; jj < 8; ++jj) {
                                const int o = 16 * ot + (lane & 15), g = lane >> 4;
                                const int ch = 64 * q + 32 * cp + (jj < 4 ? 4 * g + jj : 16 + 4 * g + (jj - 4));
                                const size_t idx = ((((size_t)q * kWFrags + ((h * 3 + j) * 2 + cp) * 5 + ot) * 64) + lane) * 8 + jj;
                                wq[idx] = f2bf(k2[(((size_t)o * kC1 + ch) * 2 + h) * 3 + j]);
                            }
    if ((rc = upload(m, 0, wq.data(), wq.size() * 2))) return rc;
    std::vector<unsigned short> a1((size_t)4 * 4 * 64 * 4, 0);
    for (int q = 0; q < 4; ++q)
        for (int ct = 0; ct < 4; ++ct)
            for (int lane = 0; lane < 64; ++lane) {
                const int ch = 64 * q + 16 * ct + (lane & 15), kg = lane >> 4;
                unsigned short* d = &a1[(((size_t)q * 4 + ct) * 64 + lane) * 4];
                const float sc = std::ldexp(1.f, -kFeatShift);
                if (kg == 3) {
                    const unsigned short hi = f2bf(b1[ch] * sc);
                    d[0] = hi;
                    d[1] = f2bf(b1[ch] * sc - bf2f(hi));
                } else {
                    for (int t = 0; t < 3; ++t) {
                        const float kv = k1[ch * 3 + t] * sc;
                        const unsigned short hi = f2bf(kv);
                        d[t] = (kg == 2) ? f2bf(kv - bf2f(hi)) : hi;
                    }
                }
            }
    if ((rc = upload(m, 1, a1.data(), a1.size() * 2))) return rc;
    (void)k1; (void)b1; (void)k2;
#else
    (void)k1; (void)b1; (void)k2;
#endif
    {
        std::vector<float> b2s(m->hb[1]);
        for (float& v : b2s) v = std::ldexp(v, -kFeatShift);
        if ((rc = upload(m, 2, b2s.data(), b2s.size() * sizeof(float)))) return rc;
    }
    m->feat_scale_log2 = -kFeatShift;
    const float* w1 = m->hk[2].data();
    std::vector<unsigned short> w1t((size_t)kHid * kFeat);
    for (int w = 0; w < kW2; ++w)
        for (int o = 0; o < kC2; ++o) {
            const float* src = w1 + (size_t)(o * kW2 + w) * kHid;
            const int kk = feat16_index(w, o);
            for (int nn = 0; nn < kHid; ++nn) w1t[((size_t)(kk >> 6) * kHid + nn) * 64 + (kk & 63)] = f2bf(std::ldexp(src[nn], kFeatShift));
        }
    if ((rc = upload(m, 3, w1t.data(), w1t.size() * 2))) return rc;
    return vtcnn2_bf16_pack_sched(m);
}

int vtcnn2_bf16_conv(const mdc_model* m, const float* x, int64_t n, void* feat, hipStream_t s, long hop2, float scale) {
#ifdef MDC_ALTERNATES
    if ((m->alt & kAltConvHipcc) && hop2 <= 0) {
        const long ngroups = (n + 15) / 16;
        const unsigned grid = (unsigned)(ngroups < 256 ? ngroups : 256);
        MDC_HIP(hipFuncSetAttribute(reinterpret_cast<const void*>(vt_conv_bf16_kernel), hipFuncAttributeMaxDynamicSharedMemorySize, (int)kConvBf16Lds));
        hipLaunchKernelGGL(vt_conv_bf16_kernel, dim3(grid), dim3(256), kConvBf16Lds, s, x, (long)n,
                           static_cast<const u32x4*>(m->d_pack[0]), static_cast<const u32x2*>(m->d_pack[1]),
                           static_cast<const float*>(m->d_pack[2]), static_cast<unsigned short*>(feat));
        MDC_HIP(hipGetLastError());
        return MDC_OK;
    }
#endif
    return vtcnn2_bf16_conv_sched(m, x, n, feat, s, hop2, scale);
}

}
```

### modulationdetectioncnn_amd/csrc/vtcnn2_bf16_common.h

```cpp
#pragma once
#include "mdc_internal.h"

#include <cstring>

namespace mdc {

using f32x4 = __attribute__((ext_vector_type(4))) float;
using f32x2 = __attribute__((ext_vector_type(2))) float;
using bf16x8 = __attribute__((ext_vector_type(8))) __bf16;
using bf16x2 = __attribute__((ext_vector_type(2))) __bf16;
using s16x4 = __attribute__((ext_vector_type(4))) short;
using s16x2 = __attribute__((ext_vector_type(2))) short;
using u32x4 = __attribute__((ext_vector_type(4))) unsigned;
using u32x2 = __attribute__((ext_vector_type(2))) unsigned;

namespace {

constexpr int kPairs = 67;
constexpr int kImgWords = 2 * kPairs * 64;
constexpr int kPartFloats = 4 * 5 * 64 * 4;
constexpr size_t kConvBf16Lds = (size_t)2 * kImgWords * 4 + (size_t)2 * kPartFloats * 4 + 512;
constexpr int kWFrags = 2 * 3 * 2 * 5;

__device__ __forceinline__ unsigned pack2(float a, float b) {
    return __builtin_bit_cast(unsigned, __builtin_convertvector(f32x2{a, b}, bf16x2));
}
__device__ __forceinline__ unsigned pack2relu(float a, float b) {
    s16x2 s = __builtin_bit_cast(s16x2, __builtin_convertvector(f32x2{a, b}, bf16x2));
    s = __builtin_elementwise_max(s, s16x2{0, 0});
    return __builtin_bit_cast(unsigned, s);
}
__device__ __forceinline__ float bf16_hi_as_f32(float a) {
    return __uint_as_float(pack2(a, 0.f) << 16);
}

template <bool U8> struct StageRaw { using type = float4; };
template <> struct StageRaw<true> { using type = uint2; };
template <bool U8 = false>
__device__ __forceinline__ typename StageRaw<U8>::type stage_load(int k, const float* __restrict__ x, long n, long frame0, int tid, long hop2 = 256) {
    const int idx = tid + 256 * k;
    const long f = frame0 + (idx >> 6);
    if constexpr (U8) return load8_unaligned(reinterpret_cast<const unsigned char*>(x) + (f < n ? f : n - 1) * hop2 + (idx & 31) * 8);
    else return reinterpret_cast<const float4*>(x + (f < n ? f : n - 1) * kFrameFloats)[idx & 63];
}
template <bool U8 = false>
__device__ __forceinline__ float4 stage_decode(typename StageRaw<U8>::type r, int tid, float scale) {
    if constexpr (U8) {
        const unsigned sh = ((tid >> 5) & 1) * 8;
        const unsigned a = r.x >> sh, b = r.y >> sh;
        return make_float4(((float)(a & 0xFFu) - 127.5f) * scale, ((float)((a >> 16) & 0xFFu) - 127.5f) * scale,
                           ((float)(b & 0xFFu) - 127.5f) * scale, ((float)((b >> 16) & 0xFFu) - 127.5f) * scale);
    } else {
        return r;
    }
}
__device__ __forceinline__ void stage_write(int k, float4 v, long n, long frame0, unsigned* __restrict__ im, int tid) {
    const int idx = tid + 256 * k;
    const int i = idx >> 6, l = idx & 63;
    if (frame0 + i >= n) v = make_float4(0.f, 0.f, 0.f, 0.f);
    const int h = l >> 5, m = l & 31;
    const float xs[4] = {v.x, v.y, v.z, v.w};
#pragma unroll
    for (int e = 0; e < 2; ++e) {
        const float a = xs[2 * e], b = xs[2 * e + 1];
        const unsigned hi = pack2(a, b);
        const float ah = __uint_as_float(hi << 16), bh = __uint_as_float(hi & 0xFFFF0000u);
        const unsigned lo = pack2(a - ah, b - bh);
        unsigned* d = im + (h * kPairs + 2 * m + 1 + e) * 64 + i;
        d[0] = hi;
        d[16] = lo;
        d[32] = hi;
    }
}
template <bool U8 = false>
__device__ __forceinline__ void stage_quarter(int k, const float* __restrict__ x, long n, long frame0,
                                              unsigned* __restrict__ im, int tid, long hop2 = 256, float scale = 0.f) {
    stage_write(k, stage_decode<U8>(stage_load<U8>(k, x, n, frame0, tid, hop2), tid, scale), n, frame0, im, tid);
}

__device__ __forceinline__ void glds16(const void* gsrc, void* lds_wave_base) {
    __builtin_amdgcn_global_load_lds((const __attribute__((address_space(1))) void*)gsrc,
                                     (__attribute__((address_space(3))) void*)lds_wave_base, 16, 0, 0);
}

__device__ __forceinline__ void glds16_nt(const void* gsrc, void* lds_wave_base) {
    __builtin_amdgcn_global_load_lds((const __attribute__((address_space(1))) void*)gsrc,
                                     (__attribute__((address_space(3))) void*)lds_wave_base, 16, 0, 2);
}

__device__ __forceinline__ void glds16_async(const void* gsrc, void* lds_wave_base) {
    const unsigned l = (unsigned)(size_t)(__attribute__((address_space(3))) unsigned char*)lds_wave_base;
    asm volatile("global_load_lds_dwordx4 %0, off" ::"v"(gsrc), "{m0}"(l) : "memory");
}

inline unsigned short f2bf(float f) {
    unsigned u;
    std::memcpy(&u, &f, 4);
    if ((u & 0x7F800000u) == 0x7F800000u) return (unsigned short)(u >> 16);
    u += 0x7FFFu + ((u >> 16) & 1u);
    return (unsigned short)(u >> 16);
}
inline float bf2f(unsigned short h) {
    unsigned u = (unsigned)h << 16;
    float f;
    std::memcpy(&f, &u, 4);
    return f;
}

}

int vtcnn2_bf16_conv_sched(const mdc_model* m, const float* x, int64_t n, void* feat, hipStream_t s, long hop2 = 0, float scale = 0.f);
int vtcnn2_bf16_pack_sched(mdc_model* m);

}
```

### modulationdetectioncnn_amd/csrc/vtcnn2_bf16_dense1.hip

```cpp
#include "vtcnn2_bf16_common.h"
#include "dense_chain_common.h"

#include <cstdlib>

namespace mdc {

namespace {

constexpr int kBM = 256, kBN = 256, kBK = 64;
constexpr int kTileBytes = kBM * kBK * 2;
constexpr size_t kDenseBf16Lds = (size_t)4 * kTileBytes;
constexpr size_t kDenseHeadLds = (size_t)128 * kChainXld * 4;
static_assert(kDenseHeadLds >= kDenseBf16Lds, "the fused-head form allocates the larger of the two");
constexpr int kNT = kFeat / kBK;

__device__ __forceinline__ bf16x8 cvt_e4m3x8(u32x2 r) {
    const bf16x2 p0 = __builtin_amdgcn_cvt_scalef32_pk_bf16_fp8(r[0], 1.0f, false);
    const bf16x2 p1 = __builtin_amdgcn_cvt_scalef32_pk_bf16_fp8(r[0], 1.0f, true);
    const bf16x2 p2 = __builtin_amdgcn_cvt_scalef32_pk_bf16_fp8(r[1], 1.0f, false);
    const bf16x2 p3 = __builtin_amdgcn_cvt_scalef32_pk_bf16_fp8(r[1], 1.0f, true);
    return bf16x8{p0[0], p0[1], p1[0], p1[1], p2[0], p2[1], p3[0], p3[1]};
}


#if defined(MDC_ALTERNATES) || defined(MDC_ABLATIONS)
template <int ABL>
__global__ __launch_bounds__(512) void vt_dense1_bf16_kernel(const unsigned short* __restrict__ feat, long n,
                                                             const unsigned short* __restrict__ w1t,
                                                             const float* __restrict__ c1,
                                                             float* __restrict__ hid) {
    extern __shared__ __attribute__((aligned(16))) unsigned char smem[];
    const int tid = threadIdx.x, lane = tid & 63;
    const int wv = __builtin_amdgcn_readfirstlane(tid >> 6);
    const int wr = wv >> 2, wc = wv & 3;
    const int fr = lane & 15, fg = lane >> 4;
    const long row0 = (long)blockIdx.x * kBM;

    const int srow = lane >> 3, spos = lane & 7;
    const unsigned short* asrc[4];
    const unsigned short* bsrc[4];
#pragma unroll
    for (int p = 0; p < 4; ++p) {
        const int r = (wv * 4 + p) * 8 + srow;
        long gr = (ABL == 1 ? 0 : row0) + r;
        if (gr >= n) gr = n - 1;
        asrc[p] = feat + gr * (long)kFeat + ((spos ^ (r & 7)) * 8);
        bsrc[p] = w1t + r * kBK + ((spos ^ (r & 7)) * 8);
    }
    auto stage = [&](int t, int b) {
        if (ABL == 3 && t > 1) return;
        unsigned char* A = smem + (size_t)b * 2 * kTileBytes;
        unsigned char* B = A + kTileBytes;
#pragma unroll
        for (int p = 0; p < 4; ++p) {
            glds16(asrc[p] + t * kBK, A + (wv * 4 + p) * 1024);
            glds16(bsrc[p] + (long)t * (kBN * kBK), B + (wv * 4 + p) * 1024);
        }
    };

    f32x4 acc[8][4];
#pragma unroll
    for (int i = 0; i < 8; ++i)
#pragma unroll
        for (int j = 0; j < 4; ++j) acc[i][j] = f32x4{0.f, 0.f, 0.f, 0.f};

    auto compute = [&](int b) {
        const unsigned char* A = smem + (size_t)b * 2 * kTileBytes;
        const unsigned char* B = A + kTileBytes;
#pragma unroll
        for (int ks = 0; ks < 2; ++ks) {
            bf16x8 af[8], bfr[4];
#pragma unroll
            for (int i = 0; i < 8; ++i) {
                const int r = wr * 128 + i * 16 + fr;
                af[i] = *reinterpret_cast<const bf16x8*>(A + r * 128 + (((ks * 4 + fg) ^ (r & 7)) * 16));
            }
#pragma unroll
            for (int j = 0; j < 4; ++j) {
                const int r = wc * 64 + j * 16 + fr;
                bfr[j] = *reinterpret_cast<const bf16x8*>(B + r * 128 + (((ks * 4 + fg) ^ (r & 7)) * 16));
            }
            if (ABL == 2) {
#pragma unroll
                for (int i = 0; i < 8; ++i) asm volatile("" ::"v"(af[i]));
#pragma unroll
                for (int j = 0; j < 4; ++j) asm volatile("" ::"v"(bfr[j]));
                continue;
            }
#pragma unroll
            for (int i = 0; i < 8; ++i)
#pragma unroll
                for (int j = 0; j < 4; ++j)
                    acc[i][j] = __builtin_amdgcn_mfma_f32_16x16x32_bf16(af[i], bfr[j], acc[i][j], 0, 0, 0);
        }
    };

    stage(0, 0);
    __syncthreads();
    int cur = 0;
    for (int t = 0; t < kNT - 1; ++t) {
        stage(t + 1, cur ^ 1);
        compute(cur);
        __syncthreads();
        cur ^= 1;
    }
    compute(cur);

#pragma unroll
    for (int j = 0; j < 4; ++j) {
        const int col = wc * 64 + j * 16 + fr;
        const float bias = c1[col];
#pragma unroll
        for (int i = 0; i < 8; ++i)
#pragma unroll
            for (int r = 0; r < 4; ++r) {
                const long row = row0 + wr * 128 + i * 16 + fg * 4 + r;
                if (row < n) hid[row * kHid + col] = fmaxf(acc[i][j][r] + bias, 0.f);
            }
    }
}


#endif

template <bool HEAD>
__device__ __forceinline__ void d1_epilogue(f32x4 (&acc)[8][4], unsigned char* smem, long row0, long n, int lane, int wv,
                                            const float* __restrict__ c1, float* __restrict__ hid, const float* __restrict__ w2pack,
                                            int n_out, float* __restrict__ probs, int* __restrict__ labels) {
    const int wr = wv >> 2, wc = wv & 3, fr = lane & 15, fg = lane >> 4;
    if constexpr (!HEAD) {
#pragma unroll
        for (int j = 0; j < 4; ++j) {
            const int col = wc * 64 + j * 16 + fr;
            const float bias = c1[col];
#pragma unroll
            for (int i = 0; i < 8; ++i)
#pragma unroll
                for (int r = 0; r < 4; ++r) {
                    const long row = row0 + wr * 128 + i * 16 + fg * 4 + r;
                    if (row < n) hid[row * kHid + col] = fmaxf(acc[i][j][r] + bias, 0.f);
                }
        }
    } else {
        float* xs = reinterpret_cast<float*>(smem);
        float w2[64];
#pragma unroll
        for (int i = 0; i < 64; ++i) w2[i] = w2pack[i * 64 + lane];
        const float b2 = w2pack[64 * 64 + 16 * 64 + fr];
        float bias1[4];
#pragma unroll
        for (int j = 0; j < 4; ++j) bias1[j] = c1[wc * 64 + j * 16 + fr];
#pragma unroll
        for (int half = 0; half < 2; ++half) {
            __syncthreads();
            if (wr == half) {
#pragma unroll
                for (int j = 0; j < 4; ++j)
#pragma unroll
                    for (int i = 0; i < 8; ++i)
#pragma unroll
                        for (int r = 0; r < 4; ++r)
                            xs[(i * 16 + fg * 4 + r) * kChainXld + wc * 64 + j * 16 + fr] = fmaxf(acc[i][j][r] + bias1[j], 0.f);
            }
            __syncthreads();
            const f32x4 a2 = chain_k256(xs + (wv * 16 + fr) * kChainXld + fg, w2, f32x4{0.f, 0.f, 0.f, 0.f});
            f32x4 z;
#pragma unroll
            for (int r = 0; r < 4; ++r) z[r] = a2[r] + b2;
            chain_softmax_store(z, fr, fg, row0 + half * 128 + wv * 16, n, n_out, probs, labels, nullptr);
        }
    }
}

constexpr int kUnitBytes = 128 * 128;

template <int ABL, bool HEAD = false, bool F8 = false>
__global__ __launch_bounds__(512) void vt_dense1_bf16_phased_kernel(const unsigned short* __restrict__ feat, long n,
                                                                    const unsigned short* __restrict__ w1t,
                                                                    const float* __restrict__ c1, float* __restrict__ hid,
                                                                    const float* __restrict__ w2pack = nullptr, int n_out = 0,
                                                                    float* __restrict__ probs = nullptr, int* __restrict__ labels = nullptr) {
    extern __shared__ __attribute__((aligned(16))) unsigned char smem[];
    const int tid = threadIdx.x, lane = tid & 63;
    const int wv = __builtin_amdgcn_readfirstlane(tid >> 6);
    const int wr = wv >> 2, wc = wv & 3;
    const int fr = lane & 15, fg = lane >> 4;
    const long row0 = (long)blockIdx.x * kBM;

    const int srow = lane >> 3, spos = lane & 7;
    const unsigned short* src[4][2];
#pragma unroll
    for (int j = 0; j < 2; ++j) {
        const int u = (wv * 2 + j) * 8 + srow;
        const int sw = (spos ^ (u & 7)) * 8;
        const int arow_lo = 128 * (u >> 6) + (u & 63);
        const int brow_lo = 64 * (u >> 5) + (u & 31);
        long g0 = (ABL == 1 ? 0 : row0) + arow_lo, g3 = (ABL == 1 ? 0 : row0) + arow_lo + 64;
        if (g0 >= n) g0 = n - 1;
        if (g3 >= n) g3 = n - 1;
        src[0][j] = feat + g0 * (long)kFeat + sw;
        src[3][j] = feat + g3 * (long)kFeat + sw;
        src[1][j] = w1t + brow_lo * kBK + sw;
        src[2][j] = w1t + (brow_lo + 32) * kBK + sw;
    }
    const unsigned char* src8[2] = {nullptr, nullptr};
    if constexpr (F8) {
        const int u = wv * 16 + (lane >> 2);
        const int sw = ((lane & 3) ^ ((u >> 2) & 3)) * 16;
        const int arow_lo = 128 * (u >> 6) + (u & 63);
        long g0 = row0 + arow_lo, g3 = row0 + arow_lo + 64;
        if (g0 >= n) g0 = n - 1;
        if (g3 >= n) g3 = n - 1;
        const unsigned char* f8 = reinterpret_cast<const unsigned char*>(feat);
        src8[0] = f8 + g0 * (long)kFeat + sw;
        src8[1] = f8 + g3 * (long)kFeat + sw;
    }
    auto stage_unit = [&](int t, int unit, int b) {
        if (ABL == 2 && (unit == 1 || unit == 2) && (t & 1)) return;
        unsigned char* dst = smem + ((size_t)b * 4 + unit) * kUnitBytes + (wv * 2) * 1024;
        if constexpr (F8) {
            if (unit == 0 || unit == 3) {
                glds16(src8[unit == 3] + (long)t * kBK, smem + ((size_t)b * 4 + unit) * kUnitBytes + wv * 1024);
                return;
            }
        }
        if (unit == 0 || unit == 3) {
            glds16_nt(src[unit][0] + (long)t * kBK, dst);
            glds16_nt(src[unit][1] + (long)t * kBK, dst + 1024);
        } else {
            glds16(src[unit][0] + (long)t * (kBN * kBK), dst);
            glds16(src[unit][1] + (long)t * (kBN * kBK), dst + 1024);
        }
    };

    auto frag = [&](const unsigned char* unit_base, int u, int ks) {
        return *reinterpret_cast<const bf16x8*>(unit_base + u * 128 + (((ks * 4 + fg) ^ (u & 7)) * 16));
    };

    f32x4 acc[8][4];
#pragma unroll
    for (int i = 0; i < 8; ++i)
#pragma unroll
        for (int j = 0; j < 4; ++j) acc[i][j] = f32x4{0.f, 0.f, 0.f, 0.f};
    bf16x8 a0[4][2], a1[4][2], b0[2][2], b1[2][2];
    u32x2 ra[4][2];

    unsigned ra_lane[2] = {0u, 0u};
    if constexpr (F8) {
        ra_lane[0] = (unsigned)((64 * wr + fr) * 64 + ((((fg >> 1) ^ ((fr >> 2) & 3)) * 16) + (fg & 1) * 8));
        ra_lane[1] = ra_lane[0] ^ 32u;
    }
    auto read_a = [&](bf16x8 (&a)[4][2], int unit, int b) {
        if (ABL == 3 && b == 1) return;
        const unsigned char* base = smem + ((size_t)b * 4 + unit) * kUnitBytes;
        if constexpr (F8) {
            const unsigned bl = (unsigned)(size_t)(__attribute__((address_space(3))) unsigned char*)const_cast<unsigned char*>(base);
            const unsigned ad0 = bl + ra_lane[0], ad1 = bl + ra_lane[1];
#pragma unroll
            for (int i = 0; i < 4; ++i) {
                asm volatile("ds_read_b64 %0, %1 offset:%2" : "=v"(ra[i][0]) : "v"(ad0), "i"(i * 1024) : "memory");
                asm volatile("ds_read_b64 %0, %1 offset:%2" : "=v"(ra[i][1]) : "v"(ad1), "i"(i * 1024) : "memory");
            }
        } else {
#pragma unroll
            for (int i = 0; i < 4; ++i)
#pragma unroll
                for (int ks = 0; ks < 2; ++ks) a[i][ks] = frag(base, 64 * wr + 16 * i + fr, ks);
        }
    };
    auto cvt_a = [&](bf16x8 (&a)[4][2]) {
        if constexpr (F8) {
#pragma unroll
            for (int i = 0; i < 4; ++i)
#pragma unroll
                for (int ks = 0; ks < 2; ++ks) a[i][ks] = cvt_e4m3x8(ra[i][ks]);
        }
    };
    auto read_b = [&](bf16x8 (&bq)[2][2], int unit, int b) {
        if (ABL == 3 && b == 1) return;
        const unsigned char* base = smem + ((size_t)b * 4 + unit) * kUnitBytes;
#pragma unroll
        for (int j = 0; j < 2; ++j)
#pragma unroll
            for (int ks = 0; ks < 2; ++ks) bq[j][ks] = frag(base, 32 * wc + 16 * j + fr, ks);
    };
    auto quadrant = [&](const bf16x8 (&a)[4][2], const bf16x8 (&bq)[2][2], int i0, int j0) {
#ifndef D1_NOPRIO
        __builtin_amdgcn_s_setprio(1);
#endif
#pragma unroll
        for (int ks = 0; ks < 2; ++ks)
#pragma unroll
            for (int i = 0; i < 4; ++i)
#pragma unroll
                for (int j = 0; j < 2; ++j)
                    acc[i0 + i][j0 + j] = __builtin_amdgcn_mfma_f32_16x16x32_bf16(a[i][ks], bq[j][ks], acc[i0 + i][j0 + j], 0, 0, 0);
#ifndef D1_NOPRIO
        __builtin_amdgcn_s_setprio(0);
#endif
    };
    auto quadrant_cv = [&](bf16x8 (&a)[4][2], const bf16x8 (&bq)[2][2], int i0, int j0, bf16x8 (&dst)[4][2], auto own) {
        constexpr bool OWN = decltype(own)::value;
        __builtin_amdgcn_s_setprio(1);
        if constexpr (OWN) a[0][0] = cvt_e4m3x8(ra[0][0]);
#pragma unroll
        for (int f = 0; f < 8; ++f) {
            const int ks = f >> 2, i = f & 3;
            if constexpr (OWN) { if (f + 1 < 8) a[(f + 1) & 3][(f + 1) >> 2] = cvt_e4m3x8(ra[(f + 1) & 3][(f + 1) >> 2]); }
            else dst[i][ks] = cvt_e4m3x8(ra[i][ks]);
#pragma unroll
            for (int j = 0; j < 2; ++j)
                acc[i0 + i][j0 + j] = __builtin_amdgcn_mfma_f32_16x16x32_bf16(a[i][ks], bq[j][ks], acc[i0 + i][j0 + j], 0, 0, 0);
        }
        if constexpr (OWN) __builtin_amdgcn_sched_group_barrier(0x002, 4, 0);
#pragma unroll
        for (int f = 0; f < 16; ++f) {
            __builtin_amdgcn_sched_group_barrier(0x008, 1, 0);
            __builtin_amdgcn_sched_group_barrier(0x002, 2, 0);
        }
        __builtin_amdgcn_s_setprio(0);
    };
#define D1_WAIT_BARRIER(N) do { asm volatile("s_waitcnt vmcnt(" #N ")" ::: "memory"); __builtin_amdgcn_s_barrier(); } while (0)
#define D1_LGKM() asm volatile("s_waitcnt lgkmcnt(0)" ::: "memory")
#define D1_LGKM_RA() asm volatile("s_waitcnt lgkmcnt(0)" : "+v"(ra[0][0]), "+v"(ra[0][1]), "+v"(ra[1][0]), "+v"(ra[1][1]), \
                                  "+v"(ra[2][0]), "+v"(ra[2][1]), "+v"(ra[3][0]), "+v"(ra[3][1]) :: "memory")

#pragma unroll
    for (int u = 0; u < 4; ++u) stage_unit(0, u, 0);
    D1_WAIT_BARRIER(0);
    read_a(a0, 0, 0);
    if constexpr (F8) { D1_LGKM_RA(); cvt_a(a0); }
#ifndef D1_NOSTAGGER
    if (wr == 1) __builtin_amdgcn_s_barrier();
#endif

    for (int t = 0; t < kNT; ++t) {
        const int b = t & 1;
        const bool more = t + 1 < kNT;
        if (more) stage_unit(t + 1, 0, b ^ 1);
        __builtin_amdgcn_sched_barrier(0);
        read_b(b0, 1, b);
        if constexpr (F8) { if (more) D1_WAIT_BARRIER(2); else D1_WAIT_BARRIER(1); }
        else { if (more) D1_WAIT_BARRIER(4); else D1_WAIT_BARRIER(2); }
        D1_LGKM();
        quadrant(a0, b0, 0, 0);
        __builtin_amdgcn_s_barrier();
        if (more) stage_unit(t + 1, 1, b ^ 1);
        __builtin_amdgcn_sched_barrier(0);
        read_b(b1, 2, b);
        if constexpr (F8) { if (more) D1_WAIT_BARRIER(3); else D1_WAIT_BARRIER(0); }
        else { if (more) D1_WAIT_BARRIER(4); else D1_WAIT_BARRIER(0); }
        D1_LGKM();
        quadrant(a0, b1, 0, 2);
        __builtin_amdgcn_s_barrier();
        if (more) stage_unit(t + 1, 2, b ^ 1);
        __builtin_amdgcn_sched_barrier(0);
        read_a(a1, 3, b);
        if (more) D1_WAIT_BARRIER(4); else __builtin_amdgcn_s_barrier();
        if constexpr (F8) { D1_LGKM_RA(); quadrant_cv(a1, b1, 4, 2, a1, std::true_type{}); }
        else { D1_LGKM(); quadrant(a1, b1, 4, 2); }
        __builtin_amdgcn_s_barrier();
        if (more) stage_unit(t + 1, 3, b ^ 1);
        __builtin_amdgcn_sched_barrier(0);
        if (more) read_a(a0, 0, b ^ 1);
        if constexpr (F8) { if (more) D1_WAIT_BARRIER(3); else __builtin_amdgcn_s_barrier(); }
        else { if (more) D1_WAIT_BARRIER(4); else __builtin_amdgcn_s_barrier(); }
        if constexpr (F8) {
            if (more) { D1_LGKM_RA(); quadrant_cv(a1, b0, 4, 0, a0, std::false_type{}); }
            else { D1_LGKM(); quadrant(a1, b0, 4, 0); }
        } else {
            quadrant(a1, b0, 4, 0);
            D1_LGKM();
        }
        __builtin_amdgcn_s_barrier();
    }
#ifndef D1_NOSTAGGER
    if (wr == 0) __builtin_amdgcn_s_barrier();
#endif
#undef D1_WAIT_BARRIER
#undef D1_LGKM
#undef D1_LGKM_RA

    d1_epilogue<HEAD>(acc, smem, row0, n, lane, wv, c1, hid, w2pack, n_out, probs, labels);
}


template <bool F8>
__global__ __launch_bounds__(64) void vt_dense1_bf16_small_kernel(const unsigned short* __restrict__ feat, long n,
                                                                  const unsigned short* __restrict__ w1t,
                                                                  const float* __restrict__ c1, float* __restrict__ hid) {
    const int lane = threadIdx.x, fr = lane & 15, fg = lane >> 4;
    const long row0 = (long)blockIdx.x * 16;
    const int col0 = blockIdx.y * 16;
    long ar = row0 + fr;
    if (ar >= n) ar = n - 1;
    using AFrag = typename std::conditional<F8, u32x2, bf16x8>::type;
    const unsigned char* ap = reinterpret_cast<const unsigned char*>(feat) + (ar * (long)kFeat + fg * 8) * (F8 ? 1 : 2);
    const unsigned short* bp = w1t + (long)(col0 + fr) * kBK + fg * 8;
    f32x4 acc = f32x4{0.f, 0.f, 0.f, 0.f};
    constexpr int kU = 5, kBlocks = kNT / kU;
    static_assert(kNT % kU == 0 && kBlocks % 2 == 1, "blocks: an even count in the loop, the last one drained after it");
    AFrag a0[kU][2], a1[kU][2];
    bf16x8 b0[kU][2], b1[kU][2];
    auto load = [&](AFrag (&af)[kU][2], bf16x8 (&bfr)[kU][2], int blk) {
#pragma unroll
        for (int u = 0; u < kU; ++u)
#pragma unroll
            for (int ks = 0; ks < 2; ++ks) {
                af[u][ks] = *reinterpret_cast<const AFrag*>(ap + ((blk * kU + u) * kBK + ks * 32) * (F8 ? 1 : 2));
                bfr[u][ks] = *reinterpret_cast<const bf16x8*>(bp + (long)(blk * kU + u) * (kBN * kBK) + ks * 32);
            }
    };
    auto mma = [&](const AFrag (&af)[kU][2], const bf16x8 (&bfr)[kU][2]) {
#pragma unroll
        for (int u = 0; u < kU; ++u)
#pragma unroll
            for (int ks = 0; ks < 2; ++ks) {
                bf16x8 a;
                if constexpr (F8) a = cvt_e4m3x8(af[u][ks]); else a = af[u][ks];
                acc = __builtin_amdgcn_mfma_f32_16x16x32_bf16(a, bfr[u][ks], acc, 0, 0, 0);
            }
    };
    load(a0, b0, 0);
    for (int blk = 0; blk < kBlocks - 1; blk += 2) {
        load(a1, b1, blk + 1);
        mma(a0, b0);
        load(a0, b0, blk + 2);
        mma(a1, b1);
    }
    mma(a0, b0);
    const int col = col0 + fr;
    const float bias = c1[col];
#pragma unroll
    for (int r = 0; r < 4; ++r) {
        const long row = row0 + fg * 4 + r;
        if (row < n) hid[row * kHid + col] = fmaxf(acc[r] + bias, 0.f);
    }
}

constexpr int kRing = 24;
constexpr int kGrp = 4;
constexpr size_t kCoopLds = (size_t)kRing * 4096;

template <bool F8>
__global__ __launch_bounds__(256) void vt_dense1_bf16_coop_kernel(const unsigned short* __restrict__ feat, long n,
                                                                  const unsigned short* __restrict__ w1t,
                                                                  const float* __restrict__ c1, float* __restrict__ hid) {
    extern __shared__ __attribute__((aligned(16))) unsigned char smem[];
    const int tid = threadIdx.x, lane = tid & 63, fr = lane & 15, fg = lane >> 4;
    const int wv = __builtin_amdgcn_readfirstlane(tid >> 6);
    const long row0 = (long)blockIdx.x * 16;
    const int col0 = blockIdx.y * 16;
    long ar = row0 + fr;
    if (ar >= n) ar = n - 1;
    const unsigned char* src;
    long kstep;
    if (wv < 2) {
        if constexpr (F8) { src = reinterpret_cast<const unsigned char*>(feat) + ar * (long)kFeat + fg * 16; kstep = kBK; }
        else { src = reinterpret_cast<const unsigned char*>(feat + ar * (long)kFeat + fg * 8 + (wv & 1) * 32); kstep = 2L * kBK; }
    } else {
        src = reinterpret_cast<const unsigned char*>(w1t + (long)(col0 + fr) * kBK + fg * 8 + (wv & 1) * 32);
        kstep = 2L * kBN * kBK;
    }
    const bool copies = !(F8 && wv == 1);
    static_assert(kRing % kGrp == 0, "groups do not straddle the ring's end");
    constexpr int kAhead = kRing / kGrp - 1;
    constexpr int kGroups = kNT / kGrp, kTail = kNT - kGroups * kGrp;
    auto issue = [&](int g) {
#pragma unroll
        for (int j = 0; j < kGrp; ++j) {
            const int t = g * kGrp + j, tc = t < kNT ? t : kNT - 1;
            if (copies) glds16_async(src + tc * kstep, smem + (size_t)(t % kRing) * 4096 + wv * 1024);
        }
    };
    auto read = [&](bf16x8 (&f)[kGrp][4], int g) {
        const unsigned char* slot = smem + (size_t)((g * kGrp) % kRing) * 4096;
        const unsigned char* base = slot + lane * 16;
#pragma unroll
        for (int j = 0; j < kGrp; ++j)
#pragma unroll
            for (int q = 0; q < 4; ++q) {
                if constexpr (F8) {
                    if (q < 2) {
                        const u32x2 r = *reinterpret_cast<const u32x2*>(slot + j * 4096 + (fr + 16 * (2 * q + (fg >> 1))) * 16 + (fg & 1) * 8);
                        f[j][q] = __builtin_bit_cast(bf16x8, u32x4{r[0], r[1], 0u, 0u});
                        continue;
                    }
                }
                f[j][q] = *reinterpret_cast<const bf16x8*>(base + j * 4096 + q * 1024);
            }
    };
    f32x4 acc = f32x4{0.f, 0.f, 0.f, 0.f};
    auto afrag = [&](const bf16x8& raw) {
        if constexpr (F8) { const u32x4 r = __builtin_bit_cast(u32x4, raw); return cvt_e4m3x8(u32x2{r[0], r[1]}); }
        else return raw;
    };
    auto mma = [&](const bf16x8 (&f)[kGrp][4], int tiles) {
#pragma unroll
        for (int j = 0; j < kGrp; ++j)
            if (j < tiles) {
                acc = __builtin_amdgcn_mfma_f32_16x16x32_bf16(afrag(f[j][0]), f[j][2], acc, 0, 0, 0);
                acc = __builtin_amdgcn_mfma_f32_16x16x32_bf16(afrag(f[j][1]), f[j][3], acc, 0, 0, 0);
            }
    };
    bf16x8 f0[kGrp][4], f1[kGrp][4];
    for (int g = 0; g < kAhead; ++g) issue(g);
    asm volatile("s_waitcnt vmcnt(%0)\n\ts_barrier" ::"n"((kAhead - 1) * kGrp) : "memory");
    read(f0, 0);
    asm volatile("s_waitcnt lgkmcnt(0)" ::: "memory");
    auto step = [&](bf16x8 (&cur)[kGrp][4], bf16x8 (&nxt)[kGrp][4], int g) {
        issue(g + kAhead);
        asm volatile("s_waitcnt vmcnt(%0)\n\ts_barrier" ::"n"((kAhead - 1) * kGrp) : "memory");
        read(nxt, g + 1);
        mma(cur, kGrp);
        asm volatile("s_waitcnt lgkmcnt(0)" ::: "memory");
    };
    static_assert(kGroups % 2 == 1 && kTail >= 0 && kTail < kGrp, "pairs of steps, a last full group, then the tail tiles");
    for (int g = 0; g < kGroups - 1; g += 2) {
        step(f0, f1, g);
        step(f1, f0, g + 1);
    }
    step(f0, f1, kGroups - 1);
    mma(f1, kTail);
    asm volatile("s_waitcnt vmcnt(0)" ::: "memory");
    if (wv != 0) return;
    const int col = col0 + fr;
    const float bias = c1[col];
#pragma unroll
    for (int r = 0; r < 4; ++r) {
        const long row = row0 + fg * 4 + r;
        if (row < n) hid[row * kHid + col] = fmaxf(acc[r] + bias, 0.f);
    }
}

constexpr long kCoopBatch = 256;

constexpr long kSmallBatch = 2048;

}

int vtcnn2_bf16_dense1(const mdc_model* m, const void* feat, int64_t n, float* hid, hipStream_t s,
                       bool fuse_head, float* probs, int32_t* labels, bool* fused) {
    if (fused) *fused = false;
    const bool f8 = m->dtype == MDC_FP8 && m->fp8_e4m3_features;
    if (n <= kCoopBatch) {
#define MDC_LAUNCH_COOP(F) do { \
        MDC_HIP(hipFuncSetAttribute(reinterpret_cast<const void*>(vt_dense1_bf16_coop_kernel<F>), hipFuncAttributeMaxDynamicSharedMemorySize, (int)kCoopLds)); \
        hipLaunchKernelGGL(vt_dense1_bf16_coop_kernel<F>, dim3((unsigned)((n + 15) / 16), kHid / 16), dim3(256), kCoopLds, s, \
                           static_cast<const unsigned short*>(feat), (long)n, static_cast<const unsigned short*>(m->d_pack[3]), \
                           static_cast<const float*>(m->d_pack[4]), hid); } while (0)
        if (f8) MDC_LAUNCH_COOP(true); else MDC_LAUNCH_COOP(false);
#undef MDC_LAUNCH_COOP
        MDC_HIP(hipGetLastError());
        return MDC_OK;
    }
    if (n <= kSmallBatch) {
#define MDC_LAUNCH_SMALL(F) hipLaunchKernelGGL(vt_dense1_bf16_small_kernel<F>, dim3((unsigned)((n + 15) / 16), kHid / 16), dim3(64), 0, s, \
                           static_cast<const unsigned short*>(feat), (long)n, static_cast<const unsigned short*>(m->d_pack[3]), \
                           static_cast<const float*>(m->d_pack[4]), hid)
        if (f8) MDC_LAUNCH_SMALL(true); else MDC_LAUNCH_SMALL(false);
#undef MDC_LAUNCH_SMALL
        MDC_HIP(hipGetLastError());
        return MDC_OK;
    }
    const unsigned short* f = static_cast<const unsigned short*>(feat);
    const unsigned short* w1t = static_cast<const unsigned short*>(m->d_pack[3]);
    const float* c1 = static_cast<const float*>(m->d_pack[4]);
    const dim3 grid((unsigned)((n + kBM - 1) / kBM));
#if defined(MDC_ALTERNATES) || defined(MDC_ABLATIONS)
#define MDC_LAUNCH_D1(A) do { \
    MDC_HIP(hipFuncSetAttribute(reinterpret_cast<const void*>(vt_dense1_bf16_kernel<A>), hipFuncAttributeMaxDynamicSharedMemorySize, (int)kDenseBf16Lds)); \
    hipLaunchKernelGGL(vt_dense1_bf16_kernel<A>, grid, dim3(512), kDenseBf16Lds, s, f, (long)n, w1t, c1, hid); } while (0)
#endif
#ifdef MDC_ABLATIONS
    static const int abl = getenv("MDC_ABLATE_D1") ? atoi(getenv("MDC_ABLATE_D1")) : 0;
#define MDC_LAUNCH_PROBE(A) do { \
        MDC_HIP(hipFuncSetAttribute(reinterpret_cast<const void*>(vt_dense1_bf16_phased_kernel<A>), hipFuncAttributeMaxDynamicSharedMemorySize, (int)kDenseBf16Lds)); \
        hipLaunchKernelGGL(vt_dense1_bf16_phased_kernel<A>, grid, dim3(512), kDenseBf16Lds, s, f, (long)n, w1t, c1, hid); \
        MDC_HIP(hipGetLastError()); \
        return MDC_OK; } while (0)
    if (!f8 && abl == 10) MDC_LAUNCH_PROBE(0);
    if (!f8 && abl == 11) MDC_LAUNCH_PROBE(1);
    if (!f8 && abl == 12) MDC_LAUNCH_PROBE(2);
    if (!f8 && abl == 13) MDC_LAUNCH_PROBE(3);
#undef MDC_LAUNCH_PROBE
    if (abl >= 1 && abl <= 3) {
        switch (abl) { case 1: MDC_LAUNCH_D1(1); break; case 2: MDC_LAUNCH_D1(2); break; default: MDC_LAUNCH_D1(3); }
        MDC_HIP(hipGetLastError());
        return MDC_OK;
    }
#endif
#ifdef MDC_ALTERNATES
    if (!f8 && (m->alt & kAltDense1Simple)) {
        MDC_LAUNCH_D1(0);
        MDC_HIP(hipGetLastError());
        return MDC_OK;
    }
    if (m->alt & kAltSeparateHead) fuse_head = false;
#endif
#undef MDC_LAUNCH_D1
#define MDC_LAUNCH_PHASED(F) do { \
    if (fuse_head && (probs || labels)) { \
        MDC_HIP(hipFuncSetAttribute(reinterpret_cast<const void*>(vt_dense1_bf16_phased_kernel<0, true, F>), hipFuncAttributeMaxDynamicSharedMemorySize, (int)kDenseHeadLds)); \
        hipLaunchKernelGGL((vt_dense1_bf16_phased_kernel<0, true, F>), grid, dim3(512), kDenseHeadLds, s, f, (long)n, w1t, c1, hid, \
                           static_cast<const float*>(m->d_pack[5]), (int)m->topo.classes, probs, labels); \
        if (fused) *fused = true; \
    } else { \
        MDC_HIP(hipFuncSetAttribute(reinterpret_cast<const void*>(vt_dense1_bf16_phased_kernel<0, false, F>), hipFuncAttributeMaxDynamicSharedMemorySize, (int)kDenseBf16Lds)); \
        hipLaunchKernelGGL((vt_dense1_bf16_phased_kernel<0, false, F>), grid, dim3(512), kDenseBf16Lds, s, f, (long)n, w1t, c1, hid); \
    } } while (0)
    if (f8) MDC_LAUNCH_PHASED(true); else MDC_LAUNCH_PHASED(false);
#undef MDC_LAUNCH_PHASED
    MDC_HIP(hipGetLastError());
    return MDC_OK;
}

}
```

### modulationdetectioncnn_amd/csrc/vtcnn2_bf16_sched.hip

```cpp
#include "vtcnn2_bf16_common.h"
#include "vtcnn2_sched_common.h"

#include <cmath>
#include <cstdlib>
#include <type_traits>

namespace mdc {

namespace {

constexpr int kNV = 24;

struct SchedState {
    u32x4 Wv[kNV];
    u32x4 Wa[kWFrags - kNV];
    f32x4 bias[5];
    u32x4 A1[2];
    unsigned Bf[2][2][2][4];
    f32x16 X[2];
    f32x4 rp[4];
    float rc[4];
    float tprev;
    u32x4 L0[3];
    u32x4 L1;
    unsigned cb[4];
    unsigned wr_addr, rd_addr, rc_addr, im_addr;
    int gs;
};

template <int SP, int J, int I, bool PAD = false>
__device__ __forceinline__ void sch_tap(SchedState& st, f32x4 (&acc)[5]) {
    constexpr int CT = 1 - I / 10, BB = (I / 5) % 2, OT = I % 5;
    constexpr int IDX = ((CT * 3 + J) * 2 + BB) * 5 + OT;
    const u32x4 b = u32x4{st.Bf[SP][CT][BB][0], st.Bf[SP][CT][BB][1], st.Bf[SP][CT][BB][2], st.Bf[SP][CT][BB][3]};
    if constexpr (J == 0 && I < 5) {
        if constexpr (IDX < kNV) asm volatile("v_mfma_f32_16x16x32_bf16 %0, %1, %2, %3" : "=&a"(acc[OT]) : "v"(st.Wv[IDX]), "v"(b), "a"(st.bias[OT]));
        else asm volatile("v_mfma_f32_16x16x32_bf16 %0, %1, %2, %3" : "=&a"(acc[OT]) : "a"(st.Wa[IDX - kNV]), "v"(b), "a"(st.bias[OT]));
    } else if constexpr (PAD) {
        static_assert(IDX >= kNV, "padded form written for the AGPR-resident fragments only");
        asm volatile("s_nop 1\n\tv_mfma_f32_16x16x32_bf16 %0, %1, %2, %0" : "+a"(acc[OT]) : "a"(st.Wa[IDX - kNV]), "v"(b));
    } else {
        if constexpr (IDX < kNV) asm volatile("v_mfma_f32_16x16x32_bf16 %0, %1, %2, %0" : "+a"(acc[OT]) : "v"(st.Wv[IDX]), "v"(b));
        else asm volatile("v_mfma_f32_16x16x32_bf16 %0, %1, %2, %0" : "+a"(acc[OT]) : "a"(st.Wa[IDX - kNV]), "v"(b));
    }
}
template <int SP, int U>
__device__ __forceinline__ void sch_packop(SchedState& st) {
    constexpr int CT = U >> 3, j = U & 7;
    unsigned& d = st.Bf[SP][CT][j >> 2][j & 3];
    const float lo = st.X[CT][2 * j], hi = st.X[CT][2 * j + 1];
    asm volatile("v_cvt_pk_bf16_f32 %0, %1, %2 clamp" : "=v"(d) : "v"(lo), "v"(hi));
}
template <int V12, bool FIRST, bool LAST, int ABL, bool RANGE = false>
__device__ __forceinline__ void sch_step(SchedState& st, int v, int q, unsigned short* fbase, f32x4 (&acc)[3][5], int wlo = 0) {
    constexpr int PAR = V12 & 1, PN = 1 - PAR;
    constexpr int R1 = (V12 + 1) & 3, S0 = ((V12 + 1) >> 2) % 3, SN = (S0 + 1) % 3;
    constexpr bool kLoadEven = (V12 & 3) == 1 && !LAST, kLoadOdd = (V12 & 3) == 3 && !LAST;
    constexpr int LSLOT = ((V12 >> 2) + 1) % 3;
    constexpr bool kExch = ABL != 2 && ABL != 6, kFin = ABL != 3 && ABL != 6, kC1 = ABL != 5 && ABL != 6;
    f32x4 (&a2)[5] = acc[V12 % 3];
    f32x4 (&a1)[5] = acc[(V12 + 1) % 3];
    f32x4 (&a0)[5] = acc[(V12 + 2) % 3];
    const unsigned load_addr = st.im_addr + ((v >> 2) * 16 + (kLoadEven ? 16 : 24));
    FinTmp ft;
    FinOut fo;
    constexpr int OP = (V12 + 1) & 1;
#define FIN(K) do { if (!FIRST && kFin) sch_fin_clamp<K, OP>(st, ft, fo); } while (0)
#define PREP(I) do { if (!LAST && kC1 && ABL != 11) sch_prep<R1, S0, SN, I>(st); } while (0)
#define C1M(CT) do { if (!LAST && kC1) sch_conv1_mfma<R1, S0, CT>(st); } while (0)
#define ST(W) do { if (!FIRST && kFin && (W == 0 || OP == 1)) { if (ABL == 7) { if (W == 0) asm volatile("" ::"v"(fo.o0), "v"(fo.o1)); else asm volatile("" ::"v"(fo.tt)); } else if (!RANGE || v - 1 >= wlo) sch_store<W>(fo, fbase, v - 1, q, st.gs); } } while (0)
#define WR(OT) do { if (kExch && ABL != 8) sch_part_write<PAR, OT>(st, a2[OT]); } while (0)
#define PK(N) do { if (!LAST && kC1 && ABL != 10) sch_packop<PN, N>(st); } while (0)
#define RD(R) do { if (kExch && ABL != 9) sch_red_load1<PAR, R>(st); } while (0)
#define LD() do { if (kC1 && ABL != 11) { if (kLoadEven) sch_load_even<LSLOT>(st, load_addr); else if (kLoadOdd) sch_load_odd(st, load_addr); } } while (0)
#ifdef MDC_F8_PROBE_HALF_BARRIER
    constexpr bool kHalfBarrierSkip = (V12 & 1) == 1;
#else
    constexpr bool kHalfBarrierSkip = false;
#endif
#define HANDOFF() do { \
        if (ABL == 1 || kHalfBarrierSkip) asm volatile("s_waitcnt lgkmcnt(0)" ::: "memory"); \
        else if (kExch) asm volatile("s_waitcnt lgkmcnt(0)\n\ts_barrier" ::: "memory"); \
        asm volatile("" ::"a"(a2[0]), "a"(a2[1]), "a"(a2[2]), "a"(a2[3]), "a"(a2[4])); } while (0)
    sch_wait_lds(st);
    sch_tap<PAR, 2, 0, RANGE && (V12 == 1 || V12 == 2)>(st, a2); FIN(0);
    sch_tap<PAR, 2, 1>(st, a2); FIN(1);
    sch_tap<PAR, 2, 2>(st, a2); FIN(2);
    sch_tap<PAR, 2, 3>(st, a2); FIN(3);
    sch_tap<PAR, 2, 4>(st, a2); FIN(4);
    sch_tap<PAR, 2, 5>(st, a2); FIN(5);
    sch_tap<PAR, 2, 6>(st, a2); FIN(6);
    sch_tap<PAR, 2, 7>(st, a2); FIN(7);
    sch_tap<PAR, 2, 8>(st, a2); FIN(8);
    sch_tap<PAR, 2, 9>(st, a2); FIN(9);
    sch_tap<PAR, 2, 10>(st, a2); FIN(10);
    sch_tap<PAR, 2, 11>(st, a2); FIN(11);
    sch_tap<PAR, 2, 12>(st, a2); FIN(12);
    sch_tap<PAR, 2, 13>(st, a2); FIN(13);
    sch_tap<PAR, 2, 14>(st, a2); FIN(14);
    sch_tap<PAR, 2, 15>(st, a2); FIN(15);
    sch_tap<PAR, 2, 16>(st, a2); PREP(0);
    sch_tap<PAR, 2, 17>(st, a2); PREP(1);
    sch_tap<PAR, 2, 18>(st, a2); PREP(2);
    sch_tap<PAR, 2, 19>(st, a2); PREP(3);
    C1M(0); WR(0); FIN(16); FIN(17);
    C1M(1); WR(1);
    sch_tap<PAR, 1, 0>(st, a1); ST(0);
    sch_tap<PAR, 1, 1>(st, a1); WR(2);
    sch_tap<PAR, 1, 2>(st, a1); ST(1);
    sch_tap<PAR, 1, 3>(st, a1); PK(0);
    sch_tap<PAR, 1, 4>(st, a1); WR(3);
    sch_tap<PAR, 1, 5>(st, a1); PK(1);
    sch_tap<PAR, 1, 6>(st, a1); PK(2);
    sch_tap<PAR, 1, 7>(st, a1); WR(4);
    sch_tap<PAR, 1, 8>(st, a1); PK(3);
    sch_tap<PAR, 1, 9>(st, a1); PK(4);
    sch_tap<PAR, 1, 10>(st, a1); PK(5);
    sch_tap<PAR, 1, 11>(st, a1); PK(6);
    sch_tap<PAR, 1, 12>(st, a1); PK(7);
    sch_tap<PAR, 1, 13>(st, a1); PK(8);
    sch_tap<PAR, 1, 14>(st, a1); PK(9);
    sch_tap<PAR, 1, 15>(st, a1); PK(10);
    sch_tap<PAR, 1, 16>(st, a1); PK(11);
    sch_tap<PAR, 1, 17>(st, a1); PK(12);
    sch_tap<PAR, 1, 18>(st, a1); PK(13);
    sch_tap<PAR, 1, 19>(st, a1); PK(14);
    sch_tap<PAR, 0, 0>(st, a0); PK(15);
    sch_tap<PAR, 0, 1>(st, a0);
    sch_tap<PAR, 0, 2>(st, a0);
    sch_tap<PAR, 0, 3>(st, a0);
    sch_tap<PAR, 0, 4>(st, a0);
    sch_tap<PAR, 0, 5>(st, a0);
    sch_tap<PAR, 0, 6>(st, a0); HANDOFF();
    sch_tap<PAR, 0, 7>(st, a0); RD(0);
    sch_tap<PAR, 0, 8>(st, a0); RD(1);
    sch_tap<PAR, 0, 9>(st, a0); RD(2);
    sch_tap<PAR, 0, 10>(st, a0); RD(3);
    sch_tap<PAR, 0, 11>(st, a0); RD(4);
    sch_tap<PAR, 0, 12>(st, a0); RD(5);
    sch_tap<PAR, 0, 13>(st, a0); RD(6);
    sch_tap<PAR, 0, 14>(st, a0); RD(7);
    sch_tap<PAR, 0, 15>(st, a0); LD();
    sch_tap<PAR, 0, 16>(st, a0);
    sch_tap<PAR, 0, 17>(st, a0);
    sch_tap<PAR, 0, 18>(st, a0);
    sch_tap<PAR, 0, 19>(st, a0);
    if (ABL == 10 && !LAST) asm volatile("" ::"v"(st.X[0]), "v"(st.X[1]));
#undef FIN
#undef PREP
#undef C1M
#undef ST
#undef WR
#undef PK
#undef RD
#undef LD
#undef HANDOFF
}

template <int ABL, bool U8 = false, bool RANGE = false>
__global__ __launch_bounds__(256, 1) void vt_conv_bf16_sched_kernel(const float* __restrict__ x, long n,
                                                                    const u32x4* __restrict__ wq, const u32x4* __restrict__ a1q,
                                                                    const float* __restrict__ b2, unsigned short* __restrict__ feat,
                                                                    long hop2 = 256, float scale = 0.f) {
    extern __shared__ __attribute__((aligned(16))) unsigned char smem[];
    unsigned* img = reinterpret_cast<unsigned*>(smem);
    const int tid = threadIdx.x, lane = tid & 63;
    const int q = __builtin_amdgcn_readfirstlane(tid >> 6);
    const int nl = lane & 15, g = lane >> 4;

    SchedState st;
#pragma unroll
    for (int i = 0; i < kWFrags; ++i) {
        const u32x4 w = wq[(q * kWFrags + i) * 64 + lane];
        if (i < kNV) { st.Wv[i] = w; asm volatile("" : "+v"(st.Wv[i])); }
        else { st.Wa[i - kNV] = w; asm volatile("" : "+a"(st.Wa[i - kNV])); }
    }
    st.A1[0] = a1q[(q * 2 + 0) * 64 + lane];
    st.A1[1] = a1q[(q * 2 + 1) * 64 + lane];
#pragma unroll
    for (int ot = 0; ot < 5; ++ot) {
        const f32x4 b = *reinterpret_cast<const f32x4*>(b2 + 16 * ot + 4 * g);
        st.bias[ot] = q == 0 ? b : f32x4{0.f, 0.f, 0.f, 0.f};
        asm volatile("" : "+a"(st.bias[ot]));
    }
    const unsigned part_lds = (unsigned)(size_t)(__attribute__((address_space(3))) unsigned char*)(smem + (size_t)2 * kSImgWords * 4);
    const unsigned img_lds = (unsigned)(size_t)(__attribute__((address_space(3))) unsigned char*)smem;
    auto entry = [](int f, int gg) { return 8 * (4 * (f >> 3) + gg) + ((f & 7) ^ (gg >> 1)); };
    const int fs = lane >> 2, gs = lane & 3;
    st.gs = gs;
    st.wr_addr = part_lds + (q * 5 * 64 + entry(nl, g)) * 16;
    st.rd_addr = part_lds + (q * 64 + entry(fs, gs)) * 16;
    st.rc_addr = part_lds + (4 * 64 + entry(fs, q)) * 16 + gs * 4;
#pragma unroll
    for (int k = 0; k < 4; ++k) { st.rp[k] = f32x4{0.f, 0.f, 0.f, 0.f}; st.rc[k] = 0.f; }
#pragma unroll
    for (int s = 0; s < 3; ++s) st.L0[s] = u32x4{0u, 0u, 0u, 0u};
    st.L1 = u32x4{0u, 0u, 0u, 0u};
    st.cb[0] = st.cb[1] = st.cb[2] = st.cb[3] = 0u;
    st.tprev = 0.f;

    for (int i = tid; i < 2 * kSImgWords; i += 256) img[i] = ((((i / kS) & 63) >= 32) && ((i % kS) & 1)) ? 0x3F803F80u : 0u;
    __syncthreads();
    const long ngroups = (n + 15) >> 4;
    long grp = blockIdx.x;
    if (grp < ngroups)
        for (int k = 0; k < 4; ++k) sch_stage_write(k, stage_decode<U8>(stage_load<U8>(k, x, n, grp * 16, tid, hop2), tid, scale), n, grp * 16, img, tid);
    __syncthreads();
    const int rng = RANGE ? (int)blockIdx.y : 0;
    const int S = 12 * rng;
    const int wlo = rng ? S + 2 : 0;

    int buf = 0;
    for (; grp < ngroups; grp += gridDim.x, buf ^= 1) {
        st.im_addr = img_lds + (buf * kSImgWords + lane * kS) * 4;
        unsigned short* fbase = feat + (grp * 16 + fs) * (long)(kW2 * kC2);
        const long gnext = RANGE ? ngroups : grp + gridDim.x;
        f32x4 acc[3][5];
        {
            const u32x4 zero = u32x4{0u, 0u, 0u, 0u};
#pragma unroll
            for (int b = 0; b < 5; ++b) {
                asm volatile("s_nop 1\n\tv_mfma_f32_16x16x32_bf16 %0, %1, %1, %2" : "=&a"(acc[0][b]) : "v"(zero), "a"(st.bias[b]));
                asm volatile("v_mfma_f32_16x16x32_bf16 %0, %1, %1, %2" : "=&a"(acc[1][b]) : "v"(zero), "a"(st.bias[b]));
            }
        }

        sch_load_even<0>(st, st.im_addr + (S >> 2) * 16);
        sch_load_odd(st, st.im_addr + (S >> 2) * 16 + 8);
        sch_wait_lds(st);
        sch_conv1_mfma<0, 0, 0>(st); sch_conv1_mfma<0, 0, 1>(st);
        asm volatile("s_nop 7\n\ts_nop 7\n\ts_nop 7\n\ts_nop 7\n\ts_nop 7\n\ts_nop 7\n\ts_nop 7\n\ts_nop 7" : "+v"(st.X[0]), "+v"(st.X[1]));
        [&]<int... N>(std::integer_sequence<int, N...>) { (sch_packop<0, N>(st), ...); }(std::make_integer_sequence<int, 16>{});
        asm volatile("s_nop 1");

        sch_step<0, true, false, ABL, RANGE>(st, S, q, fbase, acc, wlo);
        const int iters = RANGE ? (rng < 10 ? 1 : 0) : 10;
        int v = S + 1;
        typename StageRaw<U8>::type sv{};
        for (int it = 0; it < iters; ++it, v += 12) {
            if constexpr (!RANGE) {
                if (it >= 6 && gnext < ngroups) sch_stage_write(it - 6, stage_decode<U8>(sv, tid, scale), n, gnext * 16, img + (buf ^ 1) * kSImgWords, tid);
                if (it >= 5 && it < 9 && gnext < ngroups) sv = stage_load<U8>(it - 5, x, n, gnext * 16, tid, hop2);
            }
            sch_step<1, false, false, ABL, RANGE>(st, v + 0, q, fbase, acc, wlo);
            sch_step<2, false, false, ABL, RANGE>(st, v + 1, q, fbase, acc, wlo);
            sch_step<3, false, false, ABL, RANGE>(st, v + 2, q, fbase, acc, wlo);
            sch_step<4, false, false, ABL, RANGE>(st, v + 3, q, fbase, acc, wlo);
            sch_step<5, false, false, ABL, RANGE>(st, v + 4, q, fbase, acc, wlo);
            sch_step<6, false, false, ABL, RANGE>(st, v + 5, q, fbase, acc, wlo);
            sch_step<7, false, false, ABL, RANGE>(st, v + 6, q, fbase, acc, wlo);
            sch_step<8, false, false, ABL, RANGE>(st, v + 7, q, fbase, acc, wlo);
            sch_step<9, false, false, ABL, RANGE>(st, v + 8, q, fbase, acc, wlo);
            sch_step<10, false, false, ABL, RANGE>(st, v + 9, q, fbase, acc, wlo);
            sch_step<11, false, false, ABL, RANGE>(st, v + 10, q, fbase, acc, wlo);
            sch_step<0, false, false, ABL, RANGE>(st, v + 11, q, fbase, acc, wlo);
        }
        const int vt = RANGE ? v : 121;
        sch_step<1, false, false, ABL, RANGE>(st, vt, q, fbase, acc, wlo);
        if constexpr (RANGE) {
            if (rng < 10) {
                FinOut fo;
                sch_wait_lds(st);
                sch_fin_all_clamp<1>(st, fo);
                sch_store<0>(fo, fbase, vt, q, st.gs);
                sch_store<1>(fo, fbase, vt, q, st.gs);
                asm volatile("s_nop 7\n\ts_nop 7" ::"a"(acc[0][0]), "a"(acc[1][0]), "a"(acc[2][0]));
                __syncthreads();
                continue;
            }
        }
        sch_step<2, false, false, ABL, RANGE>(st, 122, q, fbase, acc, wlo);
        sch_step<3, false, false, ABL, RANGE>(st, 123, q, fbase, acc, wlo);
        sch_step<4, false, false, ABL, RANGE>(st, 124, q, fbase, acc, wlo);
        sch_step<5, false, false, ABL, RANGE>(st, 125, q, fbase, acc, wlo);
        sch_step<6, false, false, ABL, RANGE>(st, 126, q, fbase, acc, wlo);
        sch_step<7, false, false, ABL, RANGE>(st, 127, q, fbase, acc, wlo);
        sch_step<8, false, false, ABL, RANGE>(st, 128, q, fbase, acc, wlo);
        sch_step<9, false, true, ABL, RANGE>(st, 129, q, fbase, acc, wlo);
        auto finish_store = [&](auto odd, int w) {
            FinOut fo;
            sch_wait_lds(st);
            sch_fin_all_clamp<decltype(odd)::value>(st, fo);
            sch_store<0>(fo, fbase, w, q, st.gs);
            if constexpr (decltype(odd)::value) sch_store<1>(fo, fbase, w, q, st.gs);
        };
        using Even = std::integral_constant<int, 0>;
        using Odd = std::integral_constant<int, 1>;
        finish_store(Odd{}, 129);
        asm volatile("s_nop 7\n\ts_nop 7");
        sch_part_write<0, 0>(st, acc[1][0]); sch_part_write<0, 1>(st, acc[1][1]); sch_part_write<0, 2>(st, acc[1][2]);
        sch_part_write<0, 3>(st, acc[1][3]); sch_part_write<0, 4>(st, acc[1][4]);
        asm volatile("s_waitcnt lgkmcnt(0)\n\ts_barrier" ::: "memory");
        sch_red_load<0>(st);
        asm volatile("" ::"a"(acc[1][0]), "a"(acc[1][1]), "a"(acc[1][2]), "a"(acc[1][3]), "a"(acc[1][4]));
        finish_store(Even{}, 130);
        sch_part_write<1, 0>(st, acc[2][0]); sch_part_write<1, 1>(st, acc[2][1]); sch_part_write<1, 2>(st, acc[2][2]);
        sch_part_write<1, 3>(st, acc[2][3]); sch_part_write<1, 4>(st, acc[2][4]);
        asm volatile("s_waitcnt lgkmcnt(0)\n\ts_barrier" ::: "memory");
        sch_red_load<1>(st);
        asm volatile("" ::"a"(acc[2][0]), "a"(acc[2][1]), "a"(acc[2][2]), "a"(acc[2][3]), "a"(acc[2][4]));
        finish_store(Odd{}, 131);
        __syncthreads();
    }
}

}

int vtcnn2_bf16_pack_sched(mdc_model* m) {
    const float* k1 = m->hk[0].data();
    const float* b1 = m->hb[0].data();
    const float* k2 = m->hk[1].data();
    int rc;
    std::vector<unsigned short> wq((size_t)4 * kWFrags * 64 * 8);
    for (int q = 0; q < 4; ++q)
        for (int ct = 0; ct < 2; ++ct)
            for (int j = 0; j < 3; ++j)
                for (int bb = 0; bb < 2; ++bb)
                    for (int ot = 0; ot < 5; ++ot)
                        for (int lane = 0; lane < 64; ++lane)
                            for (int jj = 0; jj < 8; ++jj) {
                                const int o = 16 * ot + (lane & 15), kg = lane >> 4, h = kg & 1, r = 8 * bb + jj;
                                const int ch = 64 * q + 32 * ct + 8 * (r >> 2) + 4 * (kg >> 1) + (r & 3);
                                const size_t idx = ((((size_t)q * kWFrags + ((ct * 3 + j) * 2 + bb) * 5 + ot) * 64) + lane) * 8 + jj;
                                wq[idx] = f2bf(k2[(((size_t)o * kC1 + ch) * 2 + h) * 3 + j]);
                            }
    if ((rc = upload(m, 6, wq.data(), wq.size() * 2))) return rc;
    std::vector<unsigned short> a1((size_t)4 * 2 * 64 * 8, 0);
    for (int q = 0; q < 4; ++q)
        for (int ct = 0; ct < 2; ++ct)
            for (int lane = 0; lane < 64; ++lane) {
                const int ch = 64 * q + 32 * ct + (lane & 31), khalf = lane >> 5;
                unsigned short* d = &a1[(((size_t)q * 2 + ct) * 64 + lane) * 8];
                const float sc = std::ldexp(1.f, -kFeatShift);
                unsigned short th[3], tl[3];
                for (int t = 0; t < 3; ++t) {
                    th[t] = f2bf(k1[ch * 3 + t] * sc);
                    tl[t] = f2bf(k1[ch * 3 + t] * sc - bf2f(th[t]));
                }
                if (khalf == 0) {
                    d[0] = th[0]; d[1] = th[1]; d[2] = th[0]; d[3] = th[1]; d[4] = th[2]; d[6] = th[2];
                } else {
                    const unsigned short bh = f2bf(b1[ch] * sc);
                    d[0] = tl[0]; d[1] = tl[1]; d[2] = bh; d[3] = f2bf(b1[ch] * sc - bf2f(bh)); d[4] = tl[2];
                }
            }
    return upload(m, 7, a1.data(), a1.size() * 2);
}

int vtcnn2_bf16_conv_sched(const mdc_model* m, const float* x, int64_t n, void* feat, hipStream_t s, long hop2, float scale) {
    const long ngroups = (n + 15) / 16;
    const unsigned grid = (unsigned)(ngroups < 256 ? ngroups : 256);
#define MDC_LAUNCH_SCHED_V(U, R, GRID) do { \
    MDC_HIP(hipFuncSetAttribute(reinterpret_cast<const void*>(vt_conv_bf16_sched_kernel<0, U, R>), hipFuncAttributeMaxDynamicSharedMemorySize, (int)kSchedLds)); \
    hipLaunchKernelGGL((vt_conv_bf16_sched_kernel<0, U, R>), GRID, dim3(256), kSchedLds, s, x, (long)n, \
                       static_cast<const u32x4*>(m->d_pack[6]), static_cast<const u32x4*>(m->d_pack[7]), \
                       static_cast<const float*>(m->d_pack[2]), static_cast<unsigned short*>(feat), hop2 > 0 ? hop2 : 256L, scale); \
    MDC_HIP(hipGetLastError()); return MDC_OK; } while (0)
    if (n <= kConvRangeFrames) {
        if (hop2 > 0) MDC_LAUNCH_SCHED_V(true, true, dim3((unsigned)ngroups, 11));
        else MDC_LAUNCH_SCHED_V(false, true, dim3((unsigned)ngroups, 11));
    }
    if (hop2 > 0) MDC_LAUNCH_SCHED_V(true, false, dim3(grid));
#undef MDC_LAUNCH_SCHED_V
#define MDC_LAUNCH_SCHED(A) do { \
    MDC_HIP(hipFuncSetAttribute(reinterpret_cast<const void*>(vt_conv_bf16_sched_kernel<A>), hipFuncAttributeMaxDynamicSharedMemorySize, (int)kSchedLds)); \
    hipLaunchKernelGGL(vt_conv_bf16_sched_kernel<A>, dim3(grid), dim3(256), kSchedLds, s, x, (long)n, \
                       static_cast<const u32x4*>(m->d_pack[6]), static_cast<const u32x4*>(m->d_pack[7]), \
                       static_cast<const float*>(m->d_pack[2]), static_cast<unsigned short*>(feat), 256L, 0.f); } while (0)
#ifdef MDC_ABLATIONS
    static const int abl = getenv("MDC_ABLATE_S") ? atoi(getenv("MDC_ABLATE_S")) : 0;
    switch (abl) { case 1: MDC_LAUNCH_SCHED(1); break; case 2: MDC_LAUNCH_SCHED(2); break; case 3: MDC_LAUNCH_SCHED(3); break;
                   case 5: MDC_LAUNCH_SCHED(5); break; case 6: MDC_LAUNCH_SCHED(6); break; case 7: MDC_LAUNCH_SCHED(7); break;
                   case 8: MDC_LAUNCH_SCHED(8); break; case 9: MDC_LAUNCH_SCHED(9); break; case 10: MDC_LAUNCH_SCHED(10); break;
                   case 11: MDC_LAUNCH_SCHED(11); break; default: MDC_LAUNCH_SCHED(0); }
#else
    MDC_LAUNCH_SCHED(0);
#endif
#undef MDC_LAUNCH_SCHED
    MDC_HIP(hipGetLastError());
    return MDC_OK;
}

}
```

### modulationdetectioncnn_amd/csrc/vtcnn2_sched_common.h

```cpp
#pragma once
#include "vtcnn2_bf16_common.h"

#include <type_traits>
#include <utility>

namespace mdc {

namespace {

constexpr int kS = 140;
constexpr int kSImgWords = 64 * kS;
constexpr long kConvRangeFrames = 1024;
constexpr size_t kSchedLds = (size_t)2 * kSImgWords * 4 + (size_t)2 * kPartFloats * 4;

using f32x16 = __attribute__((ext_vector_type(16))) float;

template <int SLOT, class S>
__device__ __forceinline__ void sch_load_even(S& st, unsigned entry_addr) {
    asm volatile("ds_read_b128 %0, %1" : "=v"(st.L0[SLOT]) : "v"(entry_addr) : "memory");
}
template <class S>
__device__ __forceinline__ void sch_load_odd(S& st, unsigned entry_addr) {
    asm volatile("ds_read2_b64 %0, %1 offset0:0 offset1:1" : "=v"(st.L1) : "v"(entry_addr) : "memory");
}
template <int R, int S0, int SN, int I, class S>
__device__ __forceinline__ void sch_prep(S& st) {
    if constexpr (R == 1 || R == 3) {
        const unsigned w0 = R == 1 ? st.L0[S0][0] : st.L1[0], w1 = R == 1 ? st.L0[S0][1] : st.L1[1];
        const unsigned w2 = R == 1 ? st.L0[S0][2] : st.L1[2], w3 = R == 1 ? st.L0[S0][3] : st.L1[3];
        const unsigned w4 = R == 1 ? st.L1[2] : st.L0[SN][2], w5 = R == 1 ? st.L1[3] : st.L0[SN][3];
        unsigned& d = st.cb[I];
        if constexpr (I == 0) asm volatile("v_alignbit_b32 %0, %1, %2, 16" : "=v"(d) : "v"(w2), "v"(w0));
        else if constexpr (I == 1) asm volatile("v_alignbit_b32 %0, %1, %2, 16" : "=v"(d) : "v"(w3), "v"(w1));
        else if constexpr (I == 2) asm volatile("v_alignbit_b32 %0, %1, %2, 16" : "=v"(d) : "v"(w4), "v"(w2));
        else asm volatile("v_alignbit_b32 %0, %1, %2, 16" : "=v"(d) : "v"(w5), "v"(w3));
    }
}
template <int R, int S0, int CT, class S>
__device__ __forceinline__ void sch_conv1_mfma(S& st) {
    const u32x4 b = R == 0 ? st.L0[S0] : R == 2 ? st.L1 : u32x4{st.cb[0], st.cb[1], st.cb[2], st.cb[3]};
    asm volatile("v_mfma_f32_32x32x16_bf16 %0, %1, %2, 0" : "=&v"(st.X[CT]) : "v"(st.A1[CT]), "v"(b));
}
template <int PB, int OT, class S>
__device__ __forceinline__ void sch_part_write(S& st, const f32x4& a) {
    asm volatile("ds_write_b128 %0, %1 offset:%2" ::"v"(st.wr_addr), "a"(a), "i"(PB * kPartFloats * 4 + OT * 1024) : "memory");
}
template <int PB, int R, class S>
__device__ __forceinline__ void sch_red_load1(S& st) {
    constexpr int K = R >> 1;
    if constexpr ((R & 1) == 0) asm volatile("ds_read_b128 %0, %1 offset:%2" : "=v"(st.rp[K]) : "v"(st.rd_addr), "i"(PB * kPartFloats * 4 + K * 5120) : "memory");
    else asm volatile("ds_read_b32 %0, %1 offset:%2" : "=v"(st.rc[K]) : "v"(st.rc_addr), "i"(PB * kPartFloats * 4 + K * 5120) : "memory");
}
template <int PB, class S>
__device__ __forceinline__ void sch_red_load(S& st) {
    sch_red_load1<PB, 0>(st); sch_red_load1<PB, 1>(st); sch_red_load1<PB, 2>(st); sch_red_load1<PB, 3>(st);
    sch_red_load1<PB, 4>(st); sch_red_load1<PB, 5>(st); sch_red_load1<PB, 6>(st); sch_red_load1<PB, 7>(st);
}
template <class S>
__device__ __forceinline__ void sch_wait_lds(S& st) {
    asm volatile("s_waitcnt lgkmcnt(0)"
                 : "+v"(st.rp[0]), "+v"(st.rp[1]), "+v"(st.rp[2]), "+v"(st.rp[3]), "+v"(st.rc[0]), "+v"(st.rc[1]), "+v"(st.rc[2]),
                   "+v"(st.rc[3]), "+v"(st.L0[0]), "+v"(st.L0[1]), "+v"(st.L0[2]), "+v"(st.L1)
                 :: "memory");
}
struct FinOut { unsigned o0, o1, tt; };
struct FinTmp { float s[4], u[4], a, b, t; };
constexpr int kFeatShift = 32;

template <int K, int ODD, class S>
__device__ __forceinline__ void sch_fin_clamp(S& st, FinTmp& f, FinOut& out) {
    if constexpr (K < 4) asm volatile("v_add_f32 %0, %1, %2" : "=v"(f.s[K]) : "v"(st.rp[0][K]), "v"(st.rp[1][K]));
    else if constexpr (K < 8) asm volatile("v_add_f32 %0, %1, %2" : "=v"(f.u[K - 4]) : "v"(st.rp[2][K - 4]), "v"(st.rp[3][K - 4]));
    else if constexpr (K < 12) asm volatile("v_add_f32 %0, %0, %1" : "+v"(f.s[K - 8]) : "v"(f.u[K - 8]));
    else if constexpr (K == 12) asm volatile("v_cvt_pk_bf16_f32 %0, %1, %2 clamp" : "=v"(out.o0) : "v"(f.s[0]), "v"(f.s[1]));
    else if constexpr (K == 13) asm volatile("v_cvt_pk_bf16_f32 %0, %1, %2 clamp" : "=v"(out.o1) : "v"(f.s[2]), "v"(f.s[3]));
    else if constexpr (K == 14) asm volatile("v_add_f32 %0, %1, %2" : "=v"(f.a) : "v"(st.rc[0]), "v"(st.rc[1]));
    else if constexpr (K == 15) asm volatile("v_add_f32 %0, %1, %2" : "=v"(f.b) : "v"(st.rc[2]), "v"(st.rc[3]));
    else if constexpr (K == 16) {
        if constexpr (ODD) asm volatile("v_add_f32 %0, %1, %2" : "=v"(f.t) : "v"(f.a), "v"(f.b));
        else asm volatile("v_add_f32 %0, %1, %2" : "=v"(st.tprev) : "v"(f.a), "v"(f.b));
    } else if constexpr (ODD) asm volatile("v_cvt_pk_bf16_f32 %0, %1, %2 clamp" : "=v"(out.tt) : "v"(st.tprev), "v"(f.t));
}
template <int ODD, class S>
__device__ __forceinline__ void sch_fin_all_clamp(S& st, FinOut& out) {
    FinTmp f;
    [&]<int... K>(std::integer_sequence<int, K...>) { (sch_fin_clamp<K, ODD>(st, f, out), ...); }(std::make_integer_sequence<int, 18>{});
}

template <int WHICH>
__device__ __forceinline__ void sch_store(const FinOut& fo, unsigned short* frow, int w, int q, int gs) {
    unsigned short* pair = frow + (long)(w >> 1) * (2 * kC2);
    if constexpr (WHICH == 0) *reinterpret_cast<u32x2*>(pair + (w & 1) * 64 + 16 * q + 4 * gs) = u32x2{fo.o0, fo.o1};
    else *reinterpret_cast<unsigned*>(pair + 128 + 2 * (4 * q + gs)) = fo.tt;
}

__device__ __forceinline__ void sch_stage_write(int k, float4 v, long n, long frame0, unsigned* __restrict__ im, int tid) {
    const int idx = tid + 256 * k;
    const int i = idx >> 6, l = idx & 63;
    if (frame0 + i >= n) v = make_float4(0.f, 0.f, 0.f, 0.f);
    const int h = l >> 5, m = l & 31;
    const float xs[4] = {v.x, v.y, v.z, v.w};
#pragma unroll
    for (int e = 0; e < 2; ++e) {
        const float a = xs[2 * e], b = xs[2 * e + 1];
        const unsigned hi = pack2(a, b);
        const float ah = __uint_as_float(hi << 16), bh = __uint_as_float(hi & 0xFFFF0000u);
        const unsigned lo = pack2(a - ah, b - bh);
        unsigned* d = im + (i + 16 * h) * kS + 2 * (2 * m + 1 + e);
        *reinterpret_cast<u32x2*>(d) = u32x2{hi, lo};
        d[32 * kS] = hi;
    }
}


}

}
```

Before: 40.11 million frames/s.

## Store conv features in 256-frame K-tile blocked layout for dense1 loads

Adds a blocked feature layout in which each group of 256 frames is stored K-tile-major (64-element tiles contiguous across frames) instead of one row of 10560 elements per frame. The conv kernel's stores are rewritten to compute tile and offset through a new FeatDst helper, and the dense1 kernels take tile and row strides so their global-to-LDS loads read contiguous tiles. This is meant to give dense1's A-operand streaming better locality and DRAM page behaviour. In exchange the conv stores become more scattered, and the layout is used only for bf16 batches above 2048 frames without conv or flat taps.

After: 40.31 million frames/s, median of 6. No clear change (+0.5%).

```diff
diff --git a/modulationdetectioncnn_amd/csrc/mdc_api.hip b/modulationdetectioncnn_amd/csrc/mdc_api.hip
--- a/modulationdetectioncnn_amd/csrc/mdc_api.hip
+++ b/modulationdetectioncnn_amd/csrc/mdc_api.hip
@@ -134,6 +134,7 @@
             if (flag("MDC_DENSE1_PHASED", 0)) m->alt |= kAltDense1Simple;
             if (flag("MDC_DEP_F32_MFMA", 1)) m->alt |= kAltDepF32Mfma;
             if (flag("MDC_D1_FUSED_HEAD", 0)) m->alt |= kAltSeparateHead;
+            if (flag("MDC_FEAT_BLOCKED", 0)) m->alt |= kAltFeatRows;
             if (const char* e = getenv("MDC_DEP_RING")) m->alt_ring = atoi(e);
         }
 #endif
diff --git a/modulationdetectioncnn_amd/csrc/mdc_internal.h b/modulationdetectioncnn_amd/csrc/mdc_internal.h
--- a/modulationdetectioncnn_amd/csrc/mdc_internal.h
+++ b/modulationdetectioncnn_amd/csrc/mdc_internal.h
@@ -56,6 +56,20 @@
     return (w >> 1) * (2 * kC2) + (o < 64 ? (w & 1) * 64 + o : 128 + 2 * (o - 64) + (w & 1));
 }
 
+constexpr int kFeatTile = 64;
+constexpr long kFeatBlockElems = 256L * kFeat;
+constexpr int kFeatTiles = kFeat / kFeatTile;
+constexpr int kFeatTileBlocked = 256 * kFeatTile;
+static_assert((long)kFeatTiles * kFeatTileBlocked == kFeatBlockElems, "a block of 256 frames is 165 K-tile units");
+constexpr long kFeatBlockedAbove = 2048;
+struct FeatStrides { int tile, row; };
+constexpr FeatStrides kFeatRows{kFeatTile, kFeat}, kFeatBlocked{kFeatTileBlocked, kFeatTile};
+__host__ __device__ constexpr long feat16_row_base(long f, int row_stride) { return (f >> 8) * kFeatBlockElems + (f & 255) * row_stride; }
+__host__ __device__ constexpr long feat16_offset(long f, int e, int tile_stride, int row_stride) {
+    return feat16_row_base(f, row_stride) + (long)(e >> 6) * tile_stride + (e & 63);
+}
+static_assert(feat16_offset(777, 5555, kFeatRows.tile, kFeatRows.row) == 777L * kFeat + 5555, "frame rows are the formula at strides (64, 10560)");
+
 __host__ __device__ constexpr int feat8_index(int w, int o) {
     return (w >> 2) * (4 * kC2) + (o < 64 ? ((w >> 1) & 1) * 128 + 8 * (o >> 2) + 4 * (w & 1) + (o & 3) : 256 + 4 * (o - 64) + (w & 3));
 }
@@ -85,7 +99,8 @@
 enum { kAltConvHipcc = 1,
        kAltDense1Simple = 2,
        kAltDepF32Mfma = 4,
-       kAltSeparateHead = 8 };
+       kAltSeparateHead = 8,
+       kAltFeatRows = 16 };
 
 struct ProfSlot {
     const char* name;
diff --git a/modulationdetectioncnn_amd/csrc/vtcnn2.hip b/modulationdetectioncnn_amd/csrc/vtcnn2.hip
--- a/modulationdetectioncnn_amd/csrc/vtcnn2.hip
+++ b/modulationdetectioncnn_amd/csrc/vtcnn2.hip
@@ -410,9 +410,9 @@
                  float* probs, int* labels, float* tap_logits, float* tap_h1, float* tap_h2, int n1, int n2, hipStream_t s);
 
 int vtcnn2_bf16_pack(mdc_model* m);
-int vtcnn2_bf16_conv(const mdc_model* m, const float* x, int64_t n, void* feat, hipStream_t s, long hop2 = 0, float scale = 0.f);
+int vtcnn2_bf16_conv(const mdc_model* m, const float* x, int64_t n, void* feat, hipStream_t s, long hop2, float scale, bool blocked);
 int vtcnn2_bf16_dense1(const mdc_model* m, const void* feat, int64_t n, float* hid, hipStream_t s,
-                       bool fuse_head, float* probs, int32_t* labels, bool* fused);
+                       bool fuse_head, float* probs, int32_t* labels, bool* fused, bool blocked);
 
 int vtcnn2_pack(mdc_model* m) {
     const float* k1 = m->hk[0].data();
@@ -480,11 +480,13 @@
     float* hid = reinterpret_cast<float*>(static_cast<char*>(ws) + fbytes);
     const int C = m->topo.classes;
     int rc;
+    const bool blocked = m->dtype == MDC_BF16 && n > kFeatBlockedAbove && tap_kind != MDC_TAP_CONV && tap_kind != MDC_TAP_FLAT &&
+                         !(m->alt & (kAltFeatRows | kAltConvHipcc));
     bool head_done = false;
     if (m->dtype == MDC_BF16 || m->dtype == MDC_FP8) {
-        { ProfScope ps(m, 0, s); if ((rc = m->dtype == MDC_FP8 ? vtcnn2_fp8_conv(m, x, n, feat, s, hop2, scale) : vtcnn2_bf16_conv(m, x, n, feat, s, hop2, scale))) return rc; }
+        { ProfScope ps(m, 0, s); if ((rc = m->dtype == MDC_FP8 ? vtcnn2_fp8_conv(m, x, n, feat, s, hop2, scale) : vtcnn2_bf16_conv(m, x, n, feat, s, hop2, scale, blocked))) return rc; }
         const bool fuse = tap_kind != MDC_TAP_DENSE && tap_kind != MDC_TAP_HIDDEN;
-        { ProfScope ps(m, 1, s); if ((rc = vtcnn2_bf16_dense1(m, feat, n, hid, s, fuse, probs, labels, &head_done))) return rc; }
+        { ProfScope ps(m, 1, s); if ((rc = vtcnn2_bf16_dense1(m, feat, n, hid, s, fuse, probs, labels, &head_done, blocked))) return rc; }
     } else {
         {
             ProfScope ps(m, 0, s);
diff --git a/modulationdetectioncnn_amd/csrc/vtcnn2_bf16.hip b/modulationdetectioncnn_amd/csrc/vtcnn2_bf16.hip
--- a/modulationdetectioncnn_amd/csrc/vtcnn2_bf16.hip
+++ b/modulationdetectioncnn_amd/csrc/vtcnn2_bf16.hip
@@ -266,9 +266,10 @@
     return vtcnn2_bf16_pack_sched(m);
 }
 
-int vtcnn2_bf16_conv(const mdc_model* m, const float* x, int64_t n, void* feat, hipStream_t s, long hop2, float scale) {
+int vtcnn2_bf16_conv(const mdc_model* m, const float* x, int64_t n, void* feat, hipStream_t s, long hop2, float scale, bool blocked) {
 #ifdef MDC_ALTERNATES
     if ((m->alt & kAltConvHipcc) && hop2 <= 0) {
+        if (blocked) { set_error("vtcnn2 bf16 conv: the hipcc-scheduled kernel writes frame rows only"); return MDC_EINVAL; }
         const long ngroups = (n + 15) / 16;
         const unsigned grid = (unsigned)(ngroups < 256 ? ngroups : 256);
         MDC_HIP(hipFuncSetAttribute(reinterpret_cast<const void*>(vt_conv_bf16_kernel), hipFuncAttributeMaxDynamicSharedMemorySize, (int)kConvBf16Lds));
@@ -279,7 +280,7 @@
         return MDC_OK;
     }
 #endif
-    return vtcnn2_bf16_conv_sched(m, x, n, feat, s, hop2, scale);
-}
-
-}
+    return vtcnn2_bf16_conv_sched(m, x, n, feat, s, hop2, scale, blocked);
+}
+
+}
diff --git a/modulationdetectioncnn_amd/csrc/vtcnn2_bf16_common.h b/modulationdetectioncnn_amd/csrc/vtcnn2_bf16_common.h
--- a/modulationdetectioncnn_amd/csrc/vtcnn2_bf16_common.h
+++ b/modulationdetectioncnn_amd/csrc/vtcnn2_bf16_common.h
@@ -109,7 +109,7 @@
 
 }
 
-int vtcnn2_bf16_conv_sched(const mdc_model* m, const float* x, int64_t n, void* feat, hipStream_t s, long hop2 = 0, float scale = 0.f);
+int vtcnn2_bf16_conv_sched(const mdc_model* m, const float* x, int64_t n, void* feat, hipStream_t s, long hop2 = 0, float scale = 0.f, bool blocked = false);
 int vtcnn2_bf16_pack_sched(mdc_model* m);
 
 }
diff --git a/modulationdetectioncnn_amd/csrc/vtcnn2_bf16_dense1.hip b/modulationdetectioncnn_amd/csrc/vtcnn2_bf16_dense1.hip
--- a/modulationdetectioncnn_amd/csrc/vtcnn2_bf16_dense1.hip
+++ b/modulationdetectioncnn_amd/csrc/vtcnn2_bf16_dense1.hip
@@ -28,7 +28,8 @@
 __global__ __launch_bounds__(512) void vt_dense1_bf16_kernel(const unsigned short* __restrict__ feat, long n,
                                                              const unsigned short* __restrict__ w1t,
                                                              const float* __restrict__ c1,
-                                                             float* __restrict__ hid) {
+                                                             float* __restrict__ hid,
+                                                             int kts = kFeatRows.tile, int rs = kFeatRows.row) {
     extern __shared__ __attribute__((aligned(16))) unsigned char smem[];
     const int tid = threadIdx.x, lane = tid & 63;
     const int wv = __builtin_amdgcn_readfirstlane(tid >> 6);
@@ -44,7 +45,7 @@
         const int r = (wv * 4 + p) * 8 + srow;
         long gr = (ABL == 1 ? 0 : row0) + r;
         if (gr >= n) gr = n - 1;
-        asrc[p] = feat + gr * (long)kFeat + ((spos ^ (r & 7)) * 8);
+        asrc[p] = feat + feat16_row_base(gr, rs) + ((spos ^ (r & 7)) * 8);
         bsrc[p] = w1t + r * kBK + ((spos ^ (r & 7)) * 8);
     }
     auto stage = [&](int t, int b) {
@@ -53,7 +54,7 @@
         unsigned char* B = A + kTileBytes;
 #pragma unroll
         for (int p = 0; p < 4; ++p) {
-            glds16(asrc[p] + t * kBK, A + (wv * 4 + p) * 1024);
+            glds16(asrc[p] + (long)t * kts, A + (wv * 4 + p) * 1024);
             glds16(bsrc[p] + (long)t * (kBN * kBK), B + (wv * 4 + p) * 1024);
         }
     };
@@ -179,7 +180,8 @@
                                                                     const unsigned short* __restrict__ w1t,
                                                                     const float* __restrict__ c1, float* __restrict__ hid,
                                                                     const float* __restrict__ w2pack = nullptr, int n_out = 0,
-                                                                    float* __restrict__ probs = nullptr, int* __restrict__ labels = nullptr) {
+                                                                    float* __restrict__ probs = nullptr, int* __restrict__ labels = nullptr,
+                                                                    int kts = kFeatRows.tile, int rs = kFeatRows.row) {
     extern __shared__ __attribute__((aligned(16))) unsigned char smem[];
     const int tid = threadIdx.x, lane = tid & 63;
     const int wv = __builtin_amdgcn_readfirstlane(tid >> 6);
@@ -198,8 +200,8 @@
         long g0 = (ABL == 1 ? 0 : row0) + arow_lo, g3 = (ABL == 1 ? 0 : row0) + arow_lo + 64;
         if (g0 >= n) g0 = n - 1;
         if (g3 >= n) g3 = n - 1;
-        src[0][j] = feat + g0 * (long)kFeat + sw;
-        src[3][j] = feat + g3 * (long)kFeat + sw;
+        src[0][j] = feat + feat16_row_base(g0, rs) + sw;
+        src[3][j] = feat + feat16_row_base(g3, rs) + sw;
         src[1][j] = w1t + brow_lo * kBK + sw;
         src[2][j] = w1t + (brow_lo + 32) * kBK + sw;
     }
@@ -225,8 +227,8 @@
             }
         }
         if (unit == 0 || unit == 3) {
-            glds16_nt(src[unit][0] + (long)t * kBK, dst);
-            glds16_nt(src[unit][1] + (long)t * kBK, dst + 1024);
+            glds16_nt(src[unit][0] + (long)t * kts, dst);
+            glds16_nt(src[unit][1] + (long)t * kts, dst + 1024);
         } else {
             glds16(src[unit][0] + (long)t * (kBN * kBK), dst);
             glds16(src[unit][1] + (long)t * (kBN * kBK), dst + 1024);
@@ -540,9 +542,12 @@
 }
 
 int vtcnn2_bf16_dense1(const mdc_model* m, const void* feat, int64_t n, float* hid, hipStream_t s,
-                       bool fuse_head, float* probs, int32_t* labels, bool* fused) {
+                       bool fuse_head, float* probs, int32_t* labels, bool* fused, bool blocked) {
     if (fused) *fused = false;
     const bool f8 = m->dtype == MDC_FP8 && m->fp8_e4m3_features;
+    static_assert(kFeatBlockedAbove >= kSmallBatch && kFeatTile == kBK && kFeatTiles == kNT, "blocked features: tiled kernels only, their K-tiles");
+    if (blocked && (f8 || n <= kFeatBlockedAbove)) { set_error("vtcnn2 dense1: blocked features are bf16, more than %ld frames", kFeatBlockedAbove); return MDC_EINVAL; }
+    const FeatStrides fl = blocked ? kFeatBlocked : kFeatRows;
     if (n <= kCoopBatch) {
 #define MDC_LAUNCH_COOP(F) do { \
         MDC_HIP(hipFuncSetAttribute(reinterpret_cast<const void*>(vt_dense1_bf16_coop_kernel<F>), hipFuncAttributeMaxDynamicSharedMemorySize, (int)kCoopLds)); \
@@ -570,13 +575,14 @@
 #if defined(MDC_ALTERNATES) || defined(MDC_ABLATIONS)
 #define MDC_LAUNCH_D1(A) do { \
     MDC_HIP(hipFuncSetAttribute(reinterpret_cast<const void*>(vt_dense1_bf16_kernel<A>), hipFuncAttributeMaxDynamicSharedMemorySize, (int)kDenseBf16Lds)); \
-    hipLaunchKernelGGL(vt_dense1_bf16_kernel<A>, grid, dim3(512), kDenseBf16Lds, s, f, (long)n, w1t, c1, hid); } while (0)
+    hipLaunchKernelGGL(vt_dense1_bf16_kernel<A>, grid, dim3(512), kDenseBf16Lds, s, f, (long)n, w1t, c1, hid, fl.tile, fl.row); } while (0)
 #endif
 #ifdef MDC_ABLATIONS
     static const int abl = getenv("MDC_ABLATE_D1") ? atoi(getenv("MDC_ABLATE_D1")) : 0;
 #define MDC_LAUNCH_PROBE(A) do { \
         MDC_HIP(hipFuncSetAttribute(reinterpret_cast<const void*>(vt_dense1_bf16_phased_kernel<A>), hipFuncAttributeMaxDynamicSharedMemorySize, (int)kDenseBf16Lds)); \
-        hipLaunchKernelGGL(vt_dense1_bf16_phased_kernel<A>, grid, dim3(512), kDenseBf16Lds, s, f, (long)n, w1t, c1, hid); \
+        hipLaunchKernelGGL(vt_dense1_bf16_phased_kernel<A>, grid, dim3(512), kDenseBf16Lds, s, f, (long)n, w1t, c1, hid, \
+                           static_cast<const float*>(nullptr), 0, static_cast<float*>(nullptr), static_cast<int*>(nullptr), fl.tile, fl.row); \
         MDC_HIP(hipGetLastError()); \
         return MDC_OK; } while (0)
     if (!f8 && abl == 10) MDC_LAUNCH_PROBE(0);
@@ -603,11 +609,12 @@
     if (fuse_head && (probs || labels)) { \
         MDC_HIP(hipFuncSetAttribute(reinterpret_cast<const void*>(vt_dense1_bf16_phased_kernel<0, true, F>), hipFuncAttributeMaxDynamicSharedMemorySize, (int)kDenseHeadLds)); \
         hipLaunchKernelGGL((vt_dense1_bf16_phased_kernel<0, true, F>), grid, dim3(512), kDenseHeadLds, s, f, (long)n, w1t, c1, hid, \
-                           static_cast<const float*>(m->d_pack[5]), (int)m->topo.classes, probs, labels); \
+                           static_cast<const float*>(m->d_pack[5]), (int)m->topo.classes, probs, labels, fl.tile, fl.row); \
         if (fused) *fused = true; \
     } else { \
         MDC_HIP(hipFuncSetAttribute(reinterpret_cast<const void*>(vt_dense1_bf16_phased_kernel<0, false, F>), hipFuncAttributeMaxDynamicSharedMemorySize, (int)kDenseBf16Lds)); \
-        hipLaunchKernelGGL((vt_dense1_bf16_phased_kernel<0, false, F>), grid, dim3(512), kDenseBf16Lds, s, f, (long)n, w1t, c1, hid); \
+        hipLaunchKernelGGL((vt_dense1_bf16_phased_kernel<0, false, F>), grid, dim3(512), kDenseBf16Lds, s, f, (long)n, w1t, c1, hid, \
+                           static_cast<const float*>(nullptr), 0, static_cast<float*>(nullptr), static_cast<int*>(nullptr), fl.tile, fl.row); \
     } } while (0)
     if (f8) MDC_LAUNCH_PHASED(true); else MDC_LAUNCH_PHASED(false);
 #undef MDC_LAUNCH_PHASED
diff --git a/modulationdetectioncnn_amd/csrc/vtcnn2_bf16_sched.hip b/modulationdetectioncnn_amd/csrc/vtcnn2_bf16_sched.hip
--- a/modulationdetectioncnn_amd/csrc/vtcnn2_bf16_sched.hip
+++ b/modulationdetectioncnn_amd/csrc/vtcnn2_bf16_sched.hip
@@ -25,7 +25,6 @@
     u32x4 L1;
     unsigned cb[4];
     unsigned wr_addr, rd_addr, rc_addr, im_addr;
-    int gs;
 };
 
 template <int SP, int J, int I, bool PAD = false>
@@ -52,7 +51,7 @@
     asm volatile("v_cvt_pk_bf16_f32 %0, %1, %2 clamp" : "=v"(d) : "v"(lo), "v"(hi));
 }
 template <int V12, bool FIRST, bool LAST, int ABL, bool RANGE = false>
-__device__ __forceinline__ void sch_step(SchedState& st, int v, int q, unsigned short* fbase, f32x4 (&acc)[3][5], int wlo = 0) {
+__device__ __forceinline__ void sch_step(SchedState& st, int v, int q, FeatDst& fd, f32x4 (&acc)[3][5], int wlo = 0) {
     constexpr int PAR = V12 & 1, PN = 1 - PAR;
     constexpr int R1 = (V12 + 1) & 3, S0 = ((V12 + 1) >> 2) % 3, SN = (S0 + 1) % 3;
     constexpr bool kLoadEven = (V12 & 3) == 1 && !LAST, kLoadOdd = (V12 & 3) == 3 && !LAST;
@@ -65,10 +64,11 @@
     FinTmp ft;
     FinOut fo;
     constexpr int OP = (V12 + 1) & 1;
+    constexpr int KW = (V12 + 11) % 12;
 #define FIN(K) do { if (!FIRST && kFin) sch_fin_clamp<K, OP>(st, ft, fo); } while (0)
 #define PREP(I) do { if (!LAST && kC1 && ABL != 11) sch_prep<R1, S0, SN, I>(st); } while (0)
 #define C1M(CT) do { if (!LAST && kC1) sch_conv1_mfma<R1, S0, CT>(st); } while (0)
-#define ST(W) do { if (!FIRST && kFin && (W == 0 || OP == 1)) { if (ABL == 7) { if (W == 0) asm volatile("" ::"v"(fo.o0), "v"(fo.o1)); else asm volatile("" ::"v"(fo.tt)); } else if (!RANGE || v - 1 >= wlo) sch_store<W>(fo, fbase, v - 1, q, st.gs); } } while (0)
+#define ST(W) do { if (!FIRST && kFin && (W == 0 || OP == 1)) { if (ABL == 7) { if (W == 0) asm volatile("" ::"v"(fo.o0), "v"(fo.o1)); else asm volatile("" ::"v"(fo.tt)); } else if (!RANGE || v - 1 >= wlo) sch_store_tiled<W, KW>(fo, fd); } } while (0)
 #define WR(OT) do { if (kExch && ABL != 8) sch_part_write<PAR, OT>(st, a2[OT]); } while (0)
 #define PK(N) do { if (!LAST && kC1 && ABL != 10) sch_packop<PN, N>(st); } while (0)
 #define RD(R) do { if (kExch && ABL != 9) sch_red_load1<PAR, R>(st); } while (0)
@@ -161,7 +161,8 @@
 __global__ __launch_bounds__(256, 1) void vt_conv_bf16_sched_kernel(const float* __restrict__ x, long n,
                                                                     const u32x4* __restrict__ wq, const u32x4* __restrict__ a1q,
                                                                     const float* __restrict__ b2, unsigned short* __restrict__ feat,
-                                                                    long hop2 = 256, float scale = 0.f) {
+                                                                    long hop2 = 256, float scale = 0.f,
+                                                                    int kts = kFeatRows.tile, int rs = kFeatRows.row) {
     extern __shared__ __attribute__((aligned(16))) unsigned char smem[];
     unsigned* img = reinterpret_cast<unsigned*>(smem);
     const int tid = threadIdx.x, lane = tid & 63;
@@ -187,7 +188,6 @@
     const unsigned img_lds = (unsigned)(size_t)(__attribute__((address_space(3))) unsigned char*)smem;
     auto entry = [](int f, int gg) { return 8 * (4 * (f >> 3) + gg) + ((f & 7) ^ (gg >> 1)); };
     const int fs = lane >> 2, gs = lane & 3;
-    st.gs = gs;
     st.wr_addr = part_lds + (q * 5 * 64 + entry(nl, g)) * 16;
     st.rd_addr = part_lds + (q * 64 + entry(fs, gs)) * 16;
     st.rc_addr = part_lds + (4 * 64 + entry(fs, q)) * 16 + gs * 4;
@@ -209,11 +209,13 @@
     const int rng = RANGE ? (int)blockIdx.y : 0;
     const int S = 12 * rng;
     const int wlo = rng ? S + 2 : 0;
+    FeatDst fd = sch_feat_dst(q, fs, gs, kts, rs);
 
     int buf = 0;
     for (; grp < ngroups; grp += gridDim.x, buf ^= 1) {
         st.im_addr = img_lds + (buf * kSImgWords + lane * kS) * 4;
-        unsigned short* fbase = feat + (grp * 16 + fs) * (long)(kW2 * kC2);
+        unsigned short* const gbase = feat + feat16_row_base(grp * 16, rs);
+        fd.tb = gbase + (long)rng * 15 * kts;
         const long gnext = RANGE ? ngroups : grp + gridDim.x;
         f32x4 acc[3][5];
         {
@@ -233,73 +235,74 @@
         [&]<int... N>(std::integer_sequence<int, N...>) { (sch_packop<0, N>(st), ...); }(std::make_integer_sequence<int, 16>{});
         asm volatile("s_nop 1");
 
-        sch_step<0, true, false, ABL, RANGE>(st, S, q, fbase, acc, wlo);
+        sch_step<0, true, false, ABL, RANGE>(st, S, q, fd, acc, wlo);
         const int iters = RANGE ? (rng < 10 ? 1 : 0) : 10;
         int v = S + 1;
         typename StageRaw<U8>::type sv{};
         for (int it = 0; it < iters; ++it, v += 12) {
+            fd.tb = gbase + (long)(rng + it) * 15 * kts;
             if constexpr (!RANGE) {
                 if (it >= 6 && gnext < ngroups) sch_stage_write(it - 6, stage_decode<U8>(sv, tid, scale), n, gnext * 16, img + (buf ^ 1) * kSImgWords, tid);
                 if (it >= 5 && it < 9 && gnext < ngroups) sv = stage_load<U8>(it - 5, x, n, gnext * 16, tid, hop2);
             }
-            sch_step<1, false, false, ABL, RANGE>(st, v + 0, q, fbase, acc, wlo);
-            sch_step<2, false, false, ABL, RANGE>(st, v + 1, q, fbase, acc, wlo);
-            sch_step<3, false, false, ABL, RANGE>(st, v + 2, q, fbase, acc, wlo);
-            sch_step<4, false, false, ABL, RANGE>(st, v + 3, q, fbase, acc, wlo);
-            sch_step<5, false, false, ABL, RANGE>(st, v + 4, q, fbase, acc, wlo);
-            sch_step<6, false, false, ABL, RANGE>(st, v + 5, q, fbase, acc, wlo);
-            sch_step<7, false, false, ABL, RANGE>(st, v + 6, q, fbase, acc, wlo);
-            sch_step<8, false, false, ABL, RANGE>(st, v + 7, q, fbase, acc, wlo);
-            sch_step<9, false, false, ABL, RANGE>(st, v + 8, q, fbase, acc, wlo);
-            sch_step<10, false, false, ABL, RANGE>(st, v + 9, q, fbase, acc, wlo);
-            sch_step<11, false, false, ABL, RANGE>(st, v + 10, q, fbase, acc, wlo);
-            sch_step<0, false, false, ABL, RANGE>(st, v + 11, q, fbase, acc, wlo);
+            sch_step<1, false, false, ABL, RANGE>(st, v + 0, q, fd, acc, wlo);
+            sch_step<2, false, false, ABL, RANGE>(st, v + 1, q, fd, acc, wlo);
+            sch_step<3, false, false, ABL, RANGE>(st, v + 2, q, fd, acc, wlo);
+            sch_step<4, false, false, ABL, RANGE>(st, v + 3, q, fd, acc, wlo);
+            sch_step<5, false, false, ABL, RANGE>(st, v + 4, q, fd, acc, wlo);
+            sch_step<6, false, false, ABL, RANGE>(st, v + 5, q, fd, acc, wlo);
+            sch_step<7, false, false, ABL, RANGE>(st, v + 6, q, fd, acc, wlo);
+            sch_step<8, false, false, ABL, RANGE>(st, v + 7, q, fd, acc, wlo);
+            sch_step<9, false, false, ABL, RANGE>(st, v + 8, q, fd, acc, wlo);
+            sch_step<10, false, false, ABL, RANGE>(st, v + 9, q, fd, acc, wlo);
+            sch_step<11, false, false, ABL, RANGE>(st, v + 10, q, fd, acc, wlo);
+            sch_step<0, false, false, ABL, RANGE>(st, v + 11, q, fd, acc, wlo);
         }
         const int vt = RANGE ? v : 121;
-        sch_step<1, false, false, ABL, RANGE>(st, vt, q, fbase, acc, wlo);
+        fd.tb = gbase + (long)((vt - 1) / 12) * 15 * kts;
+        sch_step<1, false, false, ABL, RANGE>(st, vt, q, fd, acc, wlo);
         if constexpr (RANGE) {
             if (rng < 10) {
                 FinOut fo;
                 sch_wait_lds(st);
                 sch_fin_all_clamp<1>(st, fo);
-                sch_store<0>(fo, fbase, vt, q, st.gs);
-                sch_store<1>(fo, fbase, vt, q, st.gs);
+                sch_store_tiled<0, 1>(fo, fd);
+                sch_store_tiled<1, 1>(fo, fd);
                 asm volatile("s_nop 7\n\ts_nop 7" ::"a"(acc[0][0]), "a"(acc[1][0]), "a"(acc[2][0]));
                 __syncthreads();
                 continue;
             }
         }
-        sch_step<2, false, false, ABL, RANGE>(st, 122, q, fbase, acc, wlo);
-        sch_step<3, false, false, ABL, RANGE>(st, 123, q, fbase, acc, wlo);
-        sch_step<4, false, false, ABL, RANGE>(st, 124, q, fbase, acc, wlo);
-        sch_step<5, false, false, ABL, RANGE>(st, 125, q, fbase, acc, wlo);
-        sch_step<6, false, false, ABL, RANGE>(st, 126, q, fbase, acc, wlo);
-        sch_step<7, false, false, ABL, RANGE>(st, 127, q, fbase, acc, wlo);
-        sch_step<8, false, false, ABL, RANGE>(st, 128, q, fbase, acc, wlo);
-        sch_step<9, false, true, ABL, RANGE>(st, 129, q, fbase, acc, wlo);
-        auto finish_store = [&](auto odd, int w) {
+        sch_step<2, false, false, ABL, RANGE>(st, 122, q, fd, acc, wlo);
+        sch_step<3, false, false, ABL, RANGE>(st, 123, q, fd, acc, wlo);
+        sch_step<4, false, false, ABL, RANGE>(st, 124, q, fd, acc, wlo);
+        sch_step<5, false, false, ABL, RANGE>(st, 125, q, fd, acc, wlo);
+        sch_step<6, false, false, ABL, RANGE>(st, 126, q, fd, acc, wlo);
+        sch_step<7, false, false, ABL, RANGE>(st, 127, q, fd, acc, wlo);
+        sch_step<8, false, false, ABL, RANGE>(st, 128, q, fd, acc, wlo);
+        sch_step<9, false, true, ABL, RANGE>(st, 129, q, fd, acc, wlo);
+        auto finish_store = [&](auto wtag) {
+            constexpr int w = decltype(wtag)::value;
             FinOut fo;
             sch_wait_lds(st);
-            sch_fin_all_clamp<decltype(odd)::value>(st, fo);
-            sch_store<0>(fo, fbase, w, q, st.gs);
-            if constexpr (decltype(odd)::value) sch_store<1>(fo, fbase, w, q, st.gs);
+            sch_fin_all_clamp<w & 1>(st, fo);
+            sch_store_tiled<0, w % 12>(fo, fd);
+            if constexpr (w & 1) sch_store_tiled<1, w % 12>(fo, fd);
         };
-        using Even = std::integral_constant<int, 0>;
-        using Odd = std::integral_constant<int, 1>;
-        finish_store(Odd{}, 129);
+        finish_store(std::integral_constant<int, 129>{});
         asm volatile("s_nop 7\n\ts_nop 7");
         sch_part_write<0, 0>(st, acc[1][0]); sch_part_write<0, 1>(st, acc[1][1]); sch_part_write<0, 2>(st, acc[1][2]);
         sch_part_write<0, 3>(st, acc[1][3]); sch_part_write<0, 4>(st, acc[1][4]);
         asm volatile("s_waitcnt lgkmcnt(0)\n\ts_barrier" ::: "memory");
         sch_red_load<0>(st);
         asm volatile("" ::"a"(acc[1][0]), "a"(acc[1][1]), "a"(acc[1][2]), "a"(acc[1][3]), "a"(acc[1][4]));
-        finish_store(Even{}, 130);
+        finish_store(std::integral_constant<int, 130>{});
         sch_part_write<1, 0>(st, acc[2][0]); sch_part_write<1, 1>(st, acc[2][1]); sch_part_write<1, 2>(st, acc[2][2]);
         sch_part_write<1, 3>(st, acc[2][3]); sch_part_write<1, 4>(st, acc[2][4]);
         asm volatile("s_waitcnt lgkmcnt(0)\n\ts_barrier" ::: "memory");
         sch_red_load<1>(st);
         asm volatile("" ::"a"(acc[2][0]), "a"(acc[2][1]), "a"(acc[2][2]), "a"(acc[2][3]), "a"(acc[2][4]));
-        finish_store(Odd{}, 131);
+        finish_store(std::integral_constant<int, 131>{});
         __syncthreads();
     }
 }
@@ -347,14 +350,17 @@
     return upload(m, 7, a1.data(), a1.size() * 2);
 }
 
-int vtcnn2_bf16_conv_sched(const mdc_model* m, const float* x, int64_t n, void* feat, hipStream_t s, long hop2, float scale) {
+int vtcnn2_bf16_conv_sched(const mdc_model* m, const float* x, int64_t n, void* feat, hipStream_t s, long hop2, float scale, bool blocked) {
+    static_assert(kFeatBlockedAbove >= kConvRangeFrames, "blocked features come from the batch form only");
+    if (blocked && n <= kFeatBlockedAbove) { set_error("vtcnn2 bf16 conv: blocked features need more than %ld frames (got %lld)", kFeatBlockedAbove, (long long)n); return MDC_EINVAL; }
+    const FeatStrides fl = blocked ? kFeatBlocked : kFeatRows;
     const long ngroups = (n + 15) / 16;
     const unsigned grid = (unsigned)(ngroups < 256 ? ngroups : 256);
 #define MDC_LAUNCH_SCHED_V(U, R, GRID) do { \
     MDC_HIP(hipFuncSetAttribute(reinterpret_cast<const void*>(vt_conv_bf16_sched_kernel<0, U, R>), hipFuncAttributeMaxDynamicSharedMemorySize, (int)kSchedLds)); \
     hipLaunchKernelGGL((vt_conv_bf16_sched_kernel<0, U, R>), GRID, dim3(256), kSchedLds, s, x, (long)n, \
                        static_cast<const u32x4*>(m->d_pack[6]), static_cast<const u32x4*>(m->d_pack[7]), \
-                       static_cast<const float*>(m->d_pack[2]), static_cast<unsigned short*>(feat), hop2 > 0 ? hop2 : 256L, scale); \
+                       static_cast<const float*>(m->d_pack[2]), static_cast<unsigned short*>(feat), hop2 > 0 ? hop2 : 256L, scale, fl.tile, fl.row); \
     MDC_HIP(hipGetLastError()); return MDC_OK; } while (0)
     if (n <= kConvRangeFrames) {
         if (hop2 > 0) MDC_LAUNCH_SCHED_V(true, true, dim3((unsigned)ngroups, 11));
@@ -366,7 +372,7 @@
     MDC_HIP(hipFuncSetAttribute(reinterpret_cast<const void*>(vt_conv_bf16_sched_kernel<A>), hipFuncAttributeMaxDynamicSharedMemorySize, (int)kSchedLds)); \
     hipLaunchKernelGGL(vt_conv_bf16_sched_kernel<A>, dim3(grid), dim3(256), kSchedLds, s, x, (long)n, \
                        static_cast<const u32x4*>(m->d_pack[6]), static_cast<const u32x4*>(m->d_pack[7]), \
-                       static_cast<const float*>(m->d_pack[2]), static_cast<unsigned short*>(feat), 256L, 0.f); } while (0)
+                       static_cast<const float*>(m->d_pack[2]), static_cast<unsigned short*>(feat), 256L, 0.f, fl.tile, fl.row); } while (0)
 #ifdef MDC_ABLATIONS
     static const int abl = getenv("MDC_ABLATE_S") ? atoi(getenv("MDC_ABLATE_S")) : 0;
     switch (abl) { case 1: MDC_LAUNCH_SCHED(1); break; case 2: MDC_LAUNCH_SCHED(2); break; case 3: MDC_LAUNCH_SCHED(3); break;
diff --git a/modulationdetectioncnn_amd/csrc/vtcnn2_sched_common.h b/modulationdetectioncnn_amd/csrc/vtcnn2_sched_common.h
--- a/modulationdetectioncnn_amd/csrc/vtcnn2_sched_common.h
+++ b/modulationdetectioncnn_amd/csrc/vtcnn2_sched_common.h
@@ -94,6 +94,57 @@
     else *reinterpret_cast<unsigned*>(pair + 128 + 2 * (4 * q + gs)) = fo.tt;
 }
 
+struct FeatDst {
+    unsigned short* tb;
+    int kts;
+    int we, wo;
+    int wt;
+    unsigned lo0, lo1;
+};
+__device__ __forceinline__ FeatDst sch_feat_dst(int q, int fs, int gs, int kts, int rs) {
+    FeatDst d;
+    d.tb = nullptr;
+    d.kts = kts;
+    d.we = 16 * q;
+    d.wo = q < 2 ? 32 + 16 * q : kts + 16 * q - 32;
+    d.wt = 8 * q;
+    d.lo0 = (unsigned)(fs * rs + 4 * gs) * 2u;
+    d.lo1 = (unsigned)(fs * rs + 2 * gs) * 2u;
+    return d;
+}
+constexpr int sch_tile_of(int which, int K, int q, int kts) {
+    const int pk = K >> 1;
+    if (which == 0) return (2 * pk + (K & 1) + (pk >> 1)) * kts + ((pk & 1) ? (q < 2 ? 32 + 16 * q : kts + 16 * q - 32) : 16 * q);
+    return (2 * pk + 2 + (pk >> 1)) * kts + (pk & 1) * 32 + 8 * q;
+}
+constexpr bool sch_tiles_match() {
+    for (int kts : {kFeatRows.tile, kFeatBlocked.tile})
+        for (int w = 0; w < kW2; ++w)
+            for (int q = 0; q < 4; ++q) {
+                const int e0 = feat16_index(w, 16 * q), e1 = feat16_index(w & ~1, 64 + 4 * q);
+                if (feat16_index(w, 16 * q + 15) != e0 + 15 || (e0 >> 6) != ((e0 + 15) >> 6)) return false;
+                if (feat16_index(w | 1, 64 + 4 * q + 3) != e1 + 7 || (e1 >> 6) != ((e1 + 7) >> 6)) return false;
+                if ((w / 12) * 15 * kts + sch_tile_of(0, w % 12, q, kts) != (e0 >> 6) * kts + (e0 & 63)) return false;
+                if ((w / 12) * 15 * kts + sch_tile_of(1, w % 12, q, kts) != (e1 >> 6) * kts + (e1 & 63)) return false;
+            }
+    return true;
+}
+static_assert(sch_tiles_match(), "sch_store_tiled's split of a store's K-tile and offset is feat16_index's");
+template <int WHICH, int K>
+__device__ __forceinline__ void sch_store_tiled(const FinOut& fo, FeatDst& d) {
+    constexpr int pk = K >> 1;
+    char* tb = reinterpret_cast<char*>(d.tb);
+    unsigned& lo = WHICH == 0 ? d.lo0 : d.lo1;
+    asm volatile("" : "+v"(lo));
+    if constexpr (WHICH == 0) {
+        const int off = (2 * pk + (K & 1) + (pk >> 1)) * d.kts + ((pk & 1) ? d.wo : d.we);
+        *reinterpret_cast<u32x2*>(tb + 2L * off + lo) = u32x2{fo.o0, fo.o1};
+    } else {
+        const int off = (2 * pk + 2 + (pk >> 1)) * d.kts + (pk & 1) * 32 + d.wt;
+        *reinterpret_cast<unsigned*>(tb + 2L * off + lo) = fo.tt;
+    }
+}
+
 __device__ __forceinline__ void sch_stage_write(int k, float4 v, long n, long frame0, unsigned* __restrict__ im, int tid) {
     const int idx = tid + 256 * k;
     const int i = idx >> 6, l = idx & 63;
```
